# swook/EVE

Measured on AMD Instinct MI355X. Metric: train-step frames/sec, 128x128 eye patches T=30, higher is better.
Workload: dtype bf16; 1 GPU; BASELINE configs[1]: EyeNet training (configs/eye_net.json: ResNet-18-IN + GRU-128, angular + pupil L1 losses, clip 5.0, Adam wd 0.005), 128x128 patches, fwd+bwd+clip+Adam; global_batch=32, batch_per_gpu=32, seq_len=30, parallelism=dp1

## Files before the change

### eve_amd/_lib.py

```python
import ctypes
import os
from ctypes import POINTER, Structure, c_char_p, c_float, c_int, c_longlong, c_uint, c_void_p

from .build import LIB_PATH


class EveLibraryError(RuntimeError):
    pass


class ConvDesc(Structure):
    _fields_ = [(n, c_int) for n in ('dtype', 'N', 'IH', 'IW', 'Cin', 'OH', 'OW', 'Cout',
                                     'KH', 'KW', 'stride', 'pad')]


class DispatchConfig(Structure):
    _fields_ = [(n, c_int) for n in (
        'struct_bytes', 'conv_impl_v1', 'conv_tile_big', 'conv_halo', 'conv_ws64', 'conv_wg8', 'conv_wg8_min_tiles',
        'conv_wg8_s2_min_tiles', 'halo_persist', 'wgrad_target_wgs', 'wgrad_min_rows', 'wgrad_halo', 'wgrad_wg8',
        'wg64_th', 'wg64_nreg', 'wg64_fixed', 'in_split', 'in_min_threads', 'in_stats_one_pass', 'stem_split',
        'in_trunk_kernels', 'stem_fused_wgrad', 'stem_fwd_pairs', 'conv1x1_stream', 'conv3x3_stream', 'in_big_planes', 'cgru_seq_max_b',
        'cgru_scan', 'small_linear', 'tail_loss_node', 'bucket_elems', 'gate_wait_polls')] + [('wgrad_halo_min_m', c_longlong)]

    def as_dict(self):
        return {n: int(getattr(self, n)) for n, _ in self._fields_ if n != 'struct_bytes'}


class WgradProblem(Structure):
    _fields_ = [('dY', c_void_p), ('Y', c_void_p), ('X', c_void_p), ('X2', c_void_p), ('dW', c_void_p), ('db', c_void_p),
                ('M', c_int), ('N', c_int), ('K', c_int), ('K1', c_int), ('K2', c_int), ('act', c_int), ('rows_per_split', c_int),
                ('ldY', c_int), ('ldX', c_int), ('ldW', c_int), ('x_shift_T', c_int), ('reserved', c_int)]


WGRAD_BATCH_MAX = 12

class EyeGateParams(Structure):
    _fields_ = [('max_reproj_px', ctypes.c_double), ('pitch_lo', ctypes.c_double), ('pitch_hi', ctypes.c_double),
                ('yaw_lo', ctypes.c_double * 2), ('yaw_hi', ctypes.c_double * 2), ('close_ratio', ctypes.c_double),
                ('open_ratio', ctypes.c_double), ('baseline_rate', ctypes.c_double), ('baseline_rise', ctypes.c_double),
                ('min_inliers', c_int), ('min_inside', c_int), ('hold_frames', c_int), ('max_closed_frames', c_int)]


P = c_void_p
I = c_int
L = c_longlong
F = c_float

class PackItem(Structure):
    _fields_ = [('w_ohwi', c_void_p), ('dst_ohwi', c_void_p), ('dst_ihwo', c_void_p),
                ('Cout', c_int), ('taps', c_int), ('Cin', c_int), ('src_Cout', c_int), ('src_Cin', c_int)]


class VecTerm(Structure):
    _fields_ = [('pred', c_void_p), ('tgt', c_void_p), ('valid', c_void_p), ('dpred', c_void_p), ('D', c_int), ('kind', c_int)]


class EyeTailWeights(Structure):
    _fields_ = [(n, c_void_p) for n in ('fc_w', 'fc_b', 'c0_w', 'c0_b', 'c2_w', 'c2_b', 'ih_w', 'ih_b', 'hh_w', 'hh_b', 'g0_w', 'g0_b',
                                        'g2_w', 'p0_w', 'p0_b', 'p2_w', 'p2_b')]


class Surface(Structure):
    _fields_ = [('struct_bytes', c_int), ('kind', c_int), ('width', c_int), ('height', c_int), ('frame_stride', c_longlong),
                ('frame_bytes', c_longlong), ('offset', c_longlong * 3), ('pitch', c_int * 3), ('step', c_int * 3),
                ('xshift', c_int), ('yshift', c_int)]


VEC_TERMS_MAX = 32
PACK_BATCH_MAX = 48
ABI_VERSION = 10

SIGNATURES = {
    'eve_conv2d_fwd': [POINTER(ConvDesc), P, P, P, I, P, I, P, P],
    'eve_conv2d_fwd_stats': [POINTER(ConvDesc), P, P, P, I, P, P, F, POINTER(c_int), P],
    'eve_conv2d_dgrad': [POINTER(ConvDesc), P, P, P, P, ctypes.c_ulonglong, P],
    'eve_conv2d_dgrad_acc': [POINTER(ConvDesc), P, P, P, P],
    'eve_conv2d_wgrad': [POINTER(ConvDesc), P, P, P, I, P, P, ctypes.c_ulonglong, P],
    'eve_conv2d_wgrad_bias': [POINTER(ConvDesc), P, P, P, P, P, ctypes.c_ulonglong, P],
    'eve_get_dispatch_config': [POINTER(DispatchConfig)],
    'eve_get_default_dispatch_config': [POINTER(DispatchConfig)],
    'eve_set_dispatch_config': [POINTER(DispatchConfig)],
    'eve_stem_pack_input': [I, I, I, I, I, P, P, P],
    'eve_frames_u8_to_nchw': [L, I, I, I, P, F, F, I, P, P],
    'eve_frames_u8_to_stem': [I, L, I, I, I, P, F, F, P, P],
    'eve_stem7x7s2_fwd': [I, I, I, I, P, P, P, P],
    'eve_stem_fwd_fused': [I, I, I, I, P, P, F, P, P, P, P],
    'eve_stem_wgrad': [I, I, I, I, P, P, P, P],
    'eve_stem_bwd_dx': [I, I, I, I, P, P, P, P, P, P, P, P, P],
    'eve_stem_bwd_wgrad': [I, I, I, I, P, P, P, P, P, P, P, P, P, ctypes.c_ulonglong, P],
    'eve_stem_bwd_wgrad_workspace': [I, I, I],
    'eve_stem_dgrad_pack': [I, I, P, P, P],
    'eve_stem_dgrad': [I, I, I, I, I, P, P, P, P],
    'eve_bias_grad': [I, L, I, P, P, P],
    'eve_cgru_scan_fwd': [I, I, I, P, P, P, P, P, P, P, P, P, P, P, P],
    'eve_cgru_scan_bwd': [I, I, I, P, P, P, P, P, P, P, P, P, P, P, P],
    'eve_vector_terms': [POINTER(VecTerm), I, I, I, P, P],
    'eve_gate_signal': [P, P],
    'eve_gate_wait': [P, c_uint, P, P, P, c_uint, P],
    'eve_crnn_scan_fwd': [I, I, P, P, P, P, P, P, P],
    'eve_crnn_scan_bwd': [I, I, P, P, P, P, P, P, P],
    'eve_clstm_scan_fwd': [I, I, P, P, P, P, P, P, P, P],
    'eve_cgru_scan_fwd_c': [I, I, I, I, P, P, P, P, P, P, P, P, P, P, P, P],
    'eve_cgru_scan_bwd_c': [I, I, I, I, P, P, P, P, P, P, P, P, P, P, P, P],
    'eve_crnn_scan_fwd_c': [I, I, I, P, P, P, P, P, P, P],
    'eve_crnn_scan_bwd_c': [I, I, I, P, P, P, P, P, P, P],
    'eve_clstm_scan_fwd_c': [I, I, I, P, P, P, P, P, P, P, P],
    'eve_clstm_scan_fwd_train_c': [I, I, I, P, P, P, P, P, P, P, P, P, P, P],
    'eve_clstm_scan_bwd_c': [I, I, I, P, P, P, P, P, P, P, P, P, P, P],
    'eve_rnn_scan_fwd': [I, I, I, P, P, P, P, P, P],
    'eve_rnn_scan_bwd': [I, I, I, P, P, P, P, P, P],
    'eve_lstm_scan_fwd': [I, I, I, P, P, P, P, P, P, P, P, P],
    'eve_lstm_scan_bwd': [I, I, I, P, P, P, P, P, P, P, P, P, P, P],
    'eve_pack_weights_batch': [I, I, P, P],
    'eve_eye_losses': [I, I, P, P, P, P, P, P, F, F, P, P, P, P],
    'eve_gaze_to_pog': [L, P, P, P, P, P, P, P, F, F, P, P, P, P, P],
    'eve_gaze_to_pog_bwd': [L, P, P, P, P, P, P],
    'eve_combined_gaze': [L, P, P, P, P, P, P],
    'eve_make_heatmaps': [L, I, I, P, P, F, F, F, P, P],
    'eve_make_heatmaps_bwd': [L, I, I, P, F, F, F, P, P, P],
    'eve_soft_argmax_fwd': [L, I, I, P, F, F, P, P, P],
    'eve_soft_argmax_bwd': [L, I, I, P, P, P, F, F, P, P],
    'eve_linear_fwd': [I, I, I, P, P, P, I, P, P],
    'eve_linear_dgrad': [I, I, I, P, P, I, P, P, P],
    'eve_linear_wgrad': [I, I, I, P, P, I, P, P, P, P],
    'eve_linear_fwd_ex': [I, I, I, P, I, P, P, I, I, P, I, P],
    'eve_linear_dgrad_ex': [I, I, I, P, I, P, I, P, P, I, I, P],
    'eve_tail_head_pose': [I, P, P, P, I, I, P],
    'eve_tail_outputs_fwd': [I, P, P, P, P, P],
    'eve_tail_outputs_bwd': [I, P, P, P, P, P, F, F, P, P, P],
    'eve_linear_wgrad_batch': [POINTER(WgradProblem), I, P],
    'eve_instnorm_stats': [I, I, I, I, P, F, P, P],
    'eve_instnorm_act_fwd': [I, I, I, I, P, P, P, P, P, I, P, P],
    'eve_instnorm_act_bwd': [I, I, I, I, P, P, P, P, P, P, I, P, P, P, P, P],
    'eve_instnorm_act2_fwd': [I, I, I, I, P, P, P, P, P, P, I, P, P, I, I, P, P, P],
    'eve_instnorm_act2_bwd': [I, I, I, I, P, P, I, P, P, P, P, P, P, I, P, P, P, I, P, P, P, P],
    'eve_instnorm_fwd_fused': [I, I, I, I, P, P, P, P, I, F, P, P, P, P],
    'eve_instnorm_bwd_fused': [I, I, I, I, P, P, P, P, P, P, P, I, P, P, P, P, P, P],
    'eve_sum_rows': [I, I, P, P, P],
    'eve_sum_rows_pairs': [I, I, P, P, P, P],
    'eve_act_bwd': [I, L, P, P, I, P, P],
    'eve_add': [I, L, P, P, P, P],
    'eve_maxpool3x3s2_fwd': [I, I, I, I, I, P, P, P, P],
    'eve_maxpool3x3s2_bwd': [I, I, I, I, I, P, P, P, P],
    'eve_in_relu_maxpool_fwd': [I, I, I, I, I, P, P, P, P, P],
    'eve_in_relu_maxpool_bwd': [I, I, I, I, I, P, P, P, P, P, P, P],
    'eve_avgpool_fwd': [I, I, I, I, P, P, P],
    'eve_avgpool_bwd': [I, I, I, I, P, P, P],
    'eve_avgpool_fwd_f32': [I, I, I, I, P, P, P],
    'eve_avgpool_bwd_f32': [I, I, I, I, P, P, P],
    'eve_adaptive_maxpool_fwd': [I, I, I, I, I, I, I, P, P, P, P],
    'eve_adaptive_maxpool_bwd': [I, I, I, I, I, I, I, P, P, P, P, P],
    'eve_bilinear_fwd': [I, I, I, I, I, I, I, P, P, P],
    'eve_bilinear_bwd': [I, I, I, I, I, I, I, P, P, P],
    'eve_nchw_to_nhwc': [I, I, I, I, I, I, P, P, P],
    'eve_nhwc_to_nchw': [I, I, I, I, I, I, P, P, P],
    'eve_cast': [I, I, L, P, P, P],
    'eve_pack_weights': [I, I, I, I, P, P, P, P],
    'eve_gru_scan_fwd': [I, I, I, P, P, P, P, P, P, P, P],
    'eve_gru_scan_bwd': [I, I, I, P, P, P, P, P, P, P, P, P, P],
    'eve_cgru_gates1': [I, L, I, P, P, P, P, P],
    'eve_cgru_gates2': [I, L, I, P, P, P, P, P, P],
    'eve_cgru_gates2_bwd': [I, L, I, P, P, P, P, P, P, P, P],
    'eve_cgru_gates1_bwd': [I, L, I, P, P, P, P, P, P, P],
    'eve_clstm_gates_fwd': [I, L, I, P, P, P, P, P],
    'eve_clstm_gates_bwd': [I, L, I, P, P, P, P, P, P, P],
    'eve_heatmap_head_fwd': [I, L, I, P, P, P],
    'eve_heatmap_head_bwd': [I, L, I, P, P, P, P],
    'eve_heatmap_loss_fwd': [I, I, I, I, P, P, P, P, P, P, P],
    'eve_heatmap_loss_bwd': [I, I, I, P, P, P, P, P, P],
    'eve_sumsq': [L, P, P, P, P],
    'eve_adam_step': [L, P, P, P, P, P, F, F, F, F, F, F, F, I, P, I, P, P, P],
    'eve_eye_tail_stream_fwd': [I, I, P, P, POINTER(EyeTailWeights), P, P, P, P, P, P],
    'eve_stream_state_rows': [I, I, L, L, L, P, P, P, P],
    'eve_eye_tail_stream_fwd_len': [I, I, P, P, POINTER(EyeTailWeights), P, P, P, P, P, P, P],
    'eve_stream_state_rows_at': [I, I, I, L, L, L, L, P, P, P, P],
    'eve_stream_mask_plan': [I, I, P, P, P, P, P, P, P, P, P],
    'eve_stream_permute_rows': [I, I, L, L, L, P, P, P, P],
    'eve_screen_u8_area_to_nchw': [L, I, I, I, P, I, I, P, P],
    'eve_eye_warp_u8_to_nchw': [L, I, I, I, P, P, I, I, P, P],
    'eve_eye_warp_u8_to_stem': [I, L, I, I, I, P, P, I, I, P, P],
    'eve_eye_warp_lens_u8_to_nchw': [L, I, I, I, P, P, P, I, I, P, P],
    'eve_eye_warp_lens_u8_to_stem': [I, L, I, I, I, P, P, P, I, I, P, P],
    'eve_eye_pose_normalize': [L, P, I, I, P, P, P, P, P, P, P],
    'eve_eye_pose_normalize_rt': [L, I, P, I, P, P, P, I, I, P, P, P, P, P, P],
    'eve_face_pose_solve': [L, I, I, I, P, P, P, P, P, P, P, P, P, P],
    'eve_screen_u8_area_bgr_to_nchw': [L, I, I, I, P, I, I, P, P],
    'eve_eye_warp_fmt_to_nchw': [I, I, L, I, I, P, P, P, I, I, P, P],
    'eve_eye_warp_fmt_to_stem': [I, I, I, L, I, I, P, P, P, I, I, P, P],
    'eve_screen_area_fmt_to_nchw': [I, I, L, I, I, P, I, I, P, P],
    'eve_eye_warp_surface_to_nchw': [POINTER(Surface), I, L, P, P, P, I, I, P, P],
    'eve_eye_warp_surface_to_stem': [I, POINTER(Surface), I, L, P, P, P, I, I, P, P],
    'eve_screen_area_surface_to_nchw': [POINTER(Surface), I, L, P, I, I, P, P],
    'eve_overlay_render': [I, I, I, L, I, I, P, P, I, P, P, P, F, F, P, I, I, I, I, P, I, I, I, I, I, I, P, P],
    'eve_face_pose_solve_ex': [L, I, I, I, P, P, P, ctypes.c_double, P, P, P, P, P, P, P, P, P],
    'eve_undistort_points': [L, P, P, L, P, P, P],
    'eve_calib_append': [L, I, I, P, P, P, P, P, P, P, P, P, P, I, P, P, P, P],
    'eve_calib_fit': [L, I, P, P, P, ctypes.c_double, I, P, P, P, P, P, P, P, P],
    'eve_screen_calib_append': [L, I, P, P, P, P, P, P, P, P, ctypes.c_double, ctypes.c_double, I, P, P, P, P],
    'eve_screen_calib_fit': [L, I, P, P, P, I, I, ctypes.c_double, I, ctypes.c_double, P, P, P, P, P, P, P, P, P],
    'eve_screen_calib_apply': [L, I, P, P, P, P, ctypes.c_double, ctypes.c_double, P, P],
    'eve_gaze_events': [L, I, P, P, P, P, P, P, P, P, P] + [ctypes.c_double] * 4 + [I] + [ctypes.c_double] * 3 + [P, I, P, P, P] + [P] * 8,
    'eve_gaze_events_ex': [L, I, P, P, P, P, P, P, P, P, P] + [ctypes.c_double] * 4 + [I] + [ctypes.c_double] * 3 + [P, I, P, P, P] + [P] * 11,
    'eve_gaze_saccades': [L, I] + [P] * 9 + [ctypes.c_double] * 3 + [I] + [P, P, I, P, P, P] + [P] * 3,
    'eve_gaze_pursuits': [L, I] + [P] * 10 + [ctypes.c_double] * 7 + [I] + [P, P, I, P, P, P] + [P] * 7,
    'eve_eye_gate': [L, I, P, P, P, P, P, P, I, P, P, I, I, I, I, POINTER(EyeGateParams), P, I, P, P, P, P, P, P, P, P],
    'eve_gaze_history_plan': [L, I, P, P, P, P, P, P, ctypes.c_double, ctypes.c_double, I, ctypes.c_double, ctypes.c_double, I, I,
                              ctypes.c_double, ctypes.c_double, P, P, P, P],
    'eve_gaze_history_update': [L, I, I, I, P, P, P, ctypes.c_double, ctypes.c_double, P, P, P],
    'eve_gaze_aoi': [L, I, I, P, P, I] + [P] * 8 + [ctypes.c_double] * 2 + [P, P, P, I, P, P, P] + [P] * 4,
    'eve_pupil_track': [L, I] + [P] * 8 + [ctypes.c_double] * 12 + [P, P, P, I, P, P, P] + [P] * 9 + [P],
    'eve_screen_luminance': [POINTER(Surface), I, L, I, P, P, I, I, I, P, I, POINTER(c_int), P, F, F, P, P, P, P, P],
}
EXPORTS = sorted(list(SIGNATURES) + ['eve_abi_version', 'eve_last_error', 'eve_last_kernel'])

_lib = None


def load(path=None):
    global _lib
    if _lib is not None:
        return _lib
    path = path or os.environ.get('EVE_HIP_LIB', LIB_PATH)
    if not os.path.isfile(path):
        raise EveLibraryError(
            'libeve_hip.so not found at %s -- build it with `python -m eve_amd.build` '
            '(hipcc, gfx950).  eve_amd has no CPU fallback for the hot path.' % path)
    lib = ctypes.CDLL(path)
    for name, argtypes in SIGNATURES.items():
        fn = getattr(lib, name)
        fn.argtypes = argtypes
        fn.restype = c_int
    lib.eve_stem_bwd_wgrad_workspace.restype = ctypes.c_ulonglong
    lib.eve_last_kernel.argtypes = []
    lib.eve_last_kernel.restype = ctypes.c_char_p
    lib.eve_abi_version.argtypes = []
    lib.eve_abi_version.restype = c_int
    lib.eve_last_error.argtypes = []
    lib.eve_last_error.restype = c_char_p
    if lib.eve_abi_version() != ABI_VERSION:
        raise EveLibraryError('libeve_hip.so ABI version %d, expected %d (rebuild: python -m eve_amd.build)' % (
            lib.eve_abi_version(), ABI_VERSION))
    _lib = lib
    return lib


def check(status, lib=None):
    if status != 0:
        lib = lib or load()
        raise RuntimeError('libeve_hip: ' + lib.eve_last_error().decode('utf-8', 'replace'))
```

### eve_amd/csrc/api.hip

```cpp
#include <stdio.h>
#include <stdlib.h>
#include <string.h>

#include "common.h"

namespace eve {
static thread_local char g_err[512] = "";
thread_local const char* g_last_kernel = "";
thread_local hipError_t g_launch_error = hipSuccess;
int set_error(hipError_t e, const char* where) {
    snprintf(g_err, sizeof(g_err), "%s: HIP error %d (%s)", where, (int)e, hipGetErrorString(e));
    return 100 + (int)e;
}
int set_error_msg(const char* msg) {
    snprintf(g_err, sizeof(g_err), "%s", msg);
    return 1;
}
}

extern "C" int eve_abi_version(void) { return EVE_ABI_VERSION; }

namespace eve {
static eve_dispatch_config default_dispatch_config() {
    eve_dispatch_config c;
    memset(&c, 0, sizeof(c));
    c.struct_bytes = (int)sizeof(c);
    c.conv_impl_v1 = 0; c.conv_tile_big = 0; c.conv_halo = 1; c.conv_ws64 = 1; c.conv_wg8 = 1;
    c.conv_wg8_min_tiles = 224; c.conv_wg8_s2_min_tiles = 48; c.halo_persist = 1;
    c.wgrad_target_wgs = 0; c.wgrad_min_rows = 1536; c.wgrad_halo = 1; c.wgrad_wg8 = 1;
    c.wg64_th = 0; c.wg64_nreg = 0; c.wg64_fixed = 1;
    c.in_split = 1; c.in_min_threads = 512; c.in_stats_one_pass = 1; c.stem_split = 1; c.in_trunk_kernels = 1; c.stem_fused_wgrad = 1; c.stem_fwd_pairs = 1; c.in_big_planes = 1; c.conv1x1_stream = 1; c.conv3x3_stream = 1;
    c.wgrad_halo_min_m = 1ll << 20;
    c.cgru_seq_max_b = 384;
    c.cgru_scan = 1; c.small_linear = 1; c.tail_loss_node = 1; c.bucket_elems = 4 * 1024 * 1024; c.gate_wait_polls = 1 << 21;
    return c;
}
static void env_int(const char* name, int& field) { if (const char* e = getenv(name)) field = atoi(e); }
static eve_dispatch_config load_dispatch_config() {
    eve_dispatch_config c = default_dispatch_config();
    if (const char* e = getenv("EVE_CONV_IMPL")) c.conv_impl_v1 = (e[0] == 'v' && e[1] == '1') ? 1 : 0;
    if (const char* e = getenv("EVE_CONV_TILE")) c.conv_tile_big = e[0] == '2' ? 1 : 0;
    env_int("EVE_CONV_HALO", c.conv_halo); env_int("EVE_CONV_WS64", c.conv_ws64); env_int("EVE_CONV_WG8", c.conv_wg8);
    env_int("EVE_CONV_WG8_MIN_TILES", c.conv_wg8_min_tiles); env_int("EVE_CONV_WG8_S2_MIN_TILES", c.conv_wg8_s2_min_tiles);
    env_int("EVE_HALO_PERSIST", c.halo_persist); env_int("EVE_WGRAD_TARGET_WGS", c.wgrad_target_wgs);
    env_int("EVE_WGRAD_MIN_ROWS", c.wgrad_min_rows); env_int("EVE_WGRAD_HALO", c.wgrad_halo); env_int("EVE_WGRAD_WG8", c.wgrad_wg8);
    env_int("EVE_WG64_TH", c.wg64_th); env_int("EVE_WG64_NREG", c.wg64_nreg); env_int("EVE_WG64_FIXED", c.wg64_fixed);
    env_int("EVE_IN_SPLIT", c.in_split); env_int("EVE_IN_MIN_THREADS", c.in_min_threads);
    env_int("EVE_IN_STATS_ONE_PASS", c.in_stats_one_pass); env_int("EVE_STEM_SPLIT", c.stem_split);
    env_int("EVE_IN_TRUNK", c.in_trunk_kernels);
    env_int("EVE_STEM_FUSED_WGRAD", c.stem_fused_wgrad);
    env_int("EVE_STEM_FWD_PAIRS", c.stem_fwd_pairs);
    env_int("EVE_IN_BIG_PLANES", c.in_big_planes);
    env_int("EVE_CONV1X1_STREAM", c.conv1x1_stream);
    env_int("EVE_CONV3X3_STREAM", c.conv3x3_stream);
    env_int("EVE_CGRU_SEQ_MAX_B", c.cgru_seq_max_b);
    env_int("EVE_CGRU_SCAN", c.cgru_scan); env_int("EVE_SMALL_LINEAR", c.small_linear); env_int("EVE_TAIL_LOSS_NODE", c.tail_loss_node);
    env_int("EVE_BUCKET_ELEMS", c.bucket_elems); env_int("EVE_GATE_WAIT_POLLS", c.gate_wait_polls);
    if (const char* e = getenv("EVE_WGRAD_HALO_MIN_M")) c.wgrad_halo_min_m = atoll(e);
    if (c.wgrad_min_rows < 64) c.wgrad_min_rows = 64;
    if (c.in_min_threads < 64) c.in_min_threads = 64;
    if (c.bucket_elems < 1) c.bucket_elems = 1;
    if (c.gate_wait_polls < 1) c.gate_wait_polls = 1;
    return c;
}
eve_dispatch_config g_cfg = load_dispatch_config();
}

extern "C" int eve_get_dispatch_config(eve_dispatch_config* out) {
    if (!out) return eve::set_error_msg("get_dispatch_config: null pointer");
    *out = eve::g_cfg;
    return 0;
}
extern "C" int eve_get_default_dispatch_config(eve_dispatch_config* out) {
    if (!out) return eve::set_error_msg("get_default_dispatch_config: null pointer");
    *out = eve::default_dispatch_config();
    return 0;
}
extern "C" int eve_set_dispatch_config(const eve_dispatch_config* cfg) {
    if (!cfg || cfg->struct_bytes != (int)sizeof(eve_dispatch_config)) return eve::set_error_msg("set_dispatch_config: struct size mismatch (ABI)");
    if (cfg->wgrad_min_rows < 64 || cfg->in_min_threads < 64) return eve::set_error_msg("set_dispatch_config: wgrad_min_rows / in_min_threads must be >= 64");
    if (cfg->bucket_elems < 1 || cfg->gate_wait_polls < 1) return eve::set_error_msg("set_dispatch_config: bucket_elems / gate_wait_polls must be >= 1");
    eve::g_cfg = *cfg;
    return 0;
}
extern "C" const char* eve_last_error(void) { return eve::g_err; }
extern "C" const char* eve_last_kernel(void) { return eve::g_last_kernel; }
```

### eve_amd/csrc/conv_igemm.hip

```cpp
#include <limits.h>
#include <stdio.h>
#include <stdlib.h>

#include <initializer_list>
#include <type_traits>
#include "common.h"

namespace eve {

struct GatherParams {
    int N, IH, IW, Cin;
    int OH, OW, Cout;
    int KH, KW;
    int o_mul, k_mul, off, div;
    int K;
    uint32_t M;
    FastDiv fd_ohw, fd_ow, fd_cin, fd_kw, fd_oh;
};

template <typename T>
__device__ __forceinline__ uint4 prologue_vec(uint4 q, const float* __restrict__ ssp, int act) {
    constexpr int VEC = Elem<T>::VEC;
    float f[VEC];
    Elem<T>::unpack(q, f);
// ... 597 lines not shown
            for (int kw = 0; kw < p.KW; ++kw) {
                const int t = kh * p.KW + kw;
                tp.dy[t] = (signed char)(kh * p.k_mul); tp.dx[t] = (signed char)(kw * p.k_mul); tp.wt[t] = (signed char)t;
            }
        tp.osy = tp.osx = 1; tp.oy0 = tp.ox0 = 0; tp.OHf = p.OH; tp.OWf = p.OW;
        launch_dma_one<T>(p, tp, src, w, bias, epi_act, out, (uint32_t)src_bytes, (uint32_t)w_bytes, s);
        return true;
    }
    if (p.o_mul != 1 || p.k_mul != -1 || bias || (epi_act & 0xff) != EVE_ACT_NONE) return false;
    const int sd = p.div;
    bool need_zero = false;
    for (int pass = 0; pass < 2; ++pass) {
        for (int py = 0; py < sd; ++py)
            for (int px = 0; px < sd; ++px) {
                TapPlan tp;
                tp.ntaps = 0;
                for (int kh = 0; kh < p.KH; ++kh)
                    for (int kw = 0; kw < p.KW; ++kw) {
                        const int ny = py + p.off - kh, nx = px + p.off - kw;
                        if (ny % sd != 0 || nx % sd != 0) continue;
                        tp.dy[tp.ntaps] = (signed char)(ny / sd); tp.dx[tp.ntaps] = (signed char)(nx / sd);
                        tp.wt[tp.ntaps] = (signed char)(kh * p.KW + kw);
                        ++tp.ntaps;
                    }
                const int sub_h = (p.OH - py + sd - 1) / sd, sub_w = (p.OW - px + sd - 1) / sd;
                if (sub_h <= 0 || sub_w <= 0) continue;
                if (tp.ntaps == 0) { need_zero = true; continue; }
                if (pass == 0) continue;
                GatherParams q = p;
                q.OH = sub_h; q.OW = sub_w;
                q.o_mul = 1; q.off = 0; q.div = 1;
                q.M = (uint32_t)((long long)p.N * sub_h * sub_w);
                q.fd_ohw = make_fastdiv(sub_h * sub_w); q.fd_ow = make_fastdiv(sub_w);
                tp.osy = tp.osx = sd; tp.oy0 = py; tp.ox0 = px; tp.OHf = p.OH; tp.OWf = p.OW;
                launch_dma_one<T>(q, tp, src, w, bias, epi_act, out, (uint32_t)src_bytes, (uint32_t)w_bytes, s);
            }
        if (pass == 0 && need_zero && !(epi_act & EVE_EPI_ACC))
            (void)hipMemsetAsync(out, 0, (size_t)p.N * p.OH * p.OW * p.Cout * sizeof(T), s);
    }
    return true;
}

template <typename T>
static int launch_igemm(const GatherParams& p, const void* src, const void* w, const float* bias,
                        const float* ss, int pro_act, int epi_act, void* out, hipStream_t s) {
    if (!ss && !use_v1() && launch_igemm_dma<T>(p, src, w, bias, epi_act, out, s)) return 0;
    const bool wide = p.Cout > 64;
    const uint32_t bn = wide ? 128 : 64;
    const uint32_t tiles = ((p.M + 127) / 128) * ((p.Cout + bn - 1) / bn);
    dim3 grid(tiles), block(256);
    const T* a = (const T*)src; const T* b = (const T*)w; T* o = (T*)out;
    if (wide) {
        if (ss) EVE_LAUNCH("igemm_kernel<T, 4, true>", (igemm_kernel<T, 4, true>), grid, block, 0, s, p, a, b, bias, ss, pro_act, epi_act, o);
        else    EVE_LAUNCH("igemm_kernel<T, 4, false>", (igemm_kernel<T, 4, false>), grid, block, 0, s, p, a, b, bias, ss, pro_act, epi_act, o);
    } else {
        if (ss) EVE_LAUNCH("igemm_kernel<T, 2, true>", (igemm_kernel<T, 2, true>), grid, block, 0, s, p, a, b, bias, ss, pro_act, epi_act, o);
        else    EVE_LAUNCH("igemm_kernel<T, 2, false>", (igemm_kernel<T, 2, false>), grid, block, 0, s, p, a, b, bias, ss, pro_act, epi_act, o);
    }
    return 0;
}

static void wgrad_split(const GatherParams& p, uint32_t tk, uint32_t tc, size_t lds_per_wg, uint32_t& splits, uint32_t& rows) {
    const int target_env = g_cfg.wgrad_target_wgs;
    uint32_t per_cu = lds_per_wg ? (uint32_t)((160 * 1024) / lds_per_wg) : 3;
    per_cu = per_cu < 1 ? 1 : (per_cu > 3 ? 3 : per_cu);
    const uint32_t target = target_env > 0 ? (uint32_t)target_env : 256u * per_cu;
    uint32_t want = target / (tk * tc);
    const int min_rows = g_cfg.wgrad_min_rows;
    uint32_t max_splits = (p.M + (uint32_t)min_rows - 1) / (uint32_t)min_rows;
    splits = want < 1 ? 1 : (want > max_splits ? max_splits : want);
    if (splits < 1) splits = 1;
    if (splits > 65535) splits = 65535;
    rows = (p.M + splits - 1) / splits;
    rows = (rows + 63) / 64 * 64;
    splits = (p.M + rows - 1) / rows;
}

template <typename HT>
static bool launch_wgrad_halo(const GatherParams& p, const void* x, const void* dy, float* dw, float* db, hipStream_t s) {
    if (!g_cfg.wgrad_halo) return false;
    const int ks = p.KH;
    if ((ks != 3 && ks != 1) || p.KW != ks || p.o_mul != 1 || p.k_mul != 1 || p.off != -(ks / 2) || p.div != 1 || p.OH != p.IH ||
        p.OW != p.IW)
        return false;
    const int W = p.IW, H = p.IH;
    const long long min_m = g_cfg.wgrad_halo_min_m;
    if (W < 32 || W > 128 || (W & (W - 1)) || p.Cin % 16 || p.Cout % 16 || (long long)p.M < min_m) return false;
    const int MT = p.Cout / 16, CT = p.Cin / 16;
    const bool split = ks == 3 && MT == 4 && CT == 4;
    if (ks == 3 && !split && !((MT == 1 && (CT == 1 || CT == 2 || CT == 4)) || (MT == 2 && (CT == 1 || CT == 2)))) return false;
    if (ks == 1 && !((MT == 2 && CT == 1) || (MT == 1 && CT == 4) || (MT == 1 && CT == 2) || (MT == 4 && CT == 2) || (MT == 2 && CT == 4)))
        return false;
    const unsigned long long xb = (unsigned long long)p.N * H * W * p.Cin * 2, db_ = (unsigned long long)p.M * p.Cout * 2;
    if (xb >= (1ull << 31) || db_ >= (1ull << 31)) return false;
    const size_t red = (size_t)(ks * ks * p.Cin * p.Cout + p.Cout) * 4;
    const unsigned occ = (ks == 3 && MT * CT >= 4) ? 2 : 3;
    int TH = 0; size_t lds = 0;
    int nreg = 0;
    if (split) {
        const int force_th = g_cfg.wg64_th, force_nreg = g_cfg.wg64_nreg;
        for (int th : {8, 4, 2, 1}) {
            if (force_th && th != force_th) continue;
            const size_t need = (size_t)(th + 2) * (W + 2) * 128 + (size_t)th * W * 128;
            for (int nr : {3, 2}) {
                if (force_nreg && nr != force_nreg) continue;
                if (nr * need <= (size_t)160 * 1024) { TH = th; nreg = nr; lds = nr * need > red ? nr * need : red; break; }
            }
            if (TH) break;
        }
    } else
    for (size_t budget : {(size_t)(occ == 3 ? 52 : 78) * 1024, (size_t)78 * 1024}) {
        for (int th : {4, 2, 1}) {
            const size_t need = (size_t)(th + ks - 1) * (W + ks - 1) * p.Cin * 2 + (size_t)th * W * p.Cout * 2;
            if (need <= budget && need >= red) { TH = th; lds = need; break; }
        }
        if (TH) break;
    }
    if (!TH) return false;
    WgradHaloParams h;
    h.N = p.N; h.H = H; h.W = W; h.TH = TH; h.bands = (H + TH - 1) / TH;
    h.total_bands = (uint32_t)p.N * h.bands; h.x_bytes = (uint32_t)xb; h.dy_bytes = (uint32_t)db_;
    h.log2_cpr = 0; h.nreg = nreg;
    while ((32 << h.log2_cpr) < W) ++h.log2_cpr;
    const unsigned per_cu = (unsigned)((160 * 1024) / lds);
    unsigned grid = 256 * (per_cu > occ ? occ : per_cu);
    if (grid > h.total_bands) grid = h.total_bands;
    auto band_tile = [&](auto kernel) { launch(kernel, dim3(grid), dim3(256), lds, s, h, (const HT*)x, (const HT*)dy, dw, db); };
    if (split) {
        const unsigned g64 = h.total_bands < 256u ? h.total_bands : 256u;
        const int fixed64 = g_cfg.wg64_fixed;
        if (fixed64 && W == 32 && TH == 8 && H % 8 == 0)
            EVE_LAUNCH(EVE_HNAME(HT, "wgrad_halo64_kernel<", ", fixed>"), (wgrad_halo64_kernel<HT, true>), dim3(g64), dim3(512), lds, s, h, (const HT*)x, (const HT*)dy, dw, db);
        else
            EVE_LAUNCH(EVE_HNAME(HT, "wgrad_halo64_kernel<", ">"), (wgrad_halo64_kernel<HT, false>), dim3(g64), dim3(512), lds, s, h, (const HT*)x, (const HT*)dy, dw, db);
    } else if (ks == 3) {
        if (MT == 1 && CT == 1) band_tile(EVE_KERNEL_H(HT, wgrad_halo_kernel, 1, 1, 3));
        else if (MT == 1 && CT == 2) band_tile(EVE_KERNEL_H(HT, wgrad_halo_kernel, 1, 2, 3));
        else if (MT == 1 && CT == 4) band_tile(EVE_KERNEL_H(HT, wgrad_halo_kernel, 1, 4, 3));
        else if (MT == 2 && CT == 1) band_tile(EVE_KERNEL_H(HT, wgrad_halo_kernel, 2, 1, 3));
        else band_tile(EVE_KERNEL_H(HT, wgrad_halo_kernel, 2, 2, 3));
    } else {
        if (MT == 2 && CT == 1) band_tile(EVE_KERNEL_H(HT, wgrad_halo_kernel, 2, 1, 1));
        else if (MT == 1 && CT == 4) band_tile(EVE_KERNEL_H(HT, wgrad_halo_kernel, 1, 4, 1));
        else if (MT == 1 && CT == 2) band_tile(EVE_KERNEL_H(HT, wgrad_halo_kernel, 1, 2, 1));
        else if (MT == 4 && CT == 2) band_tile(EVE_KERNEL_H(HT, wgrad_halo_kernel, 4, 2, 1));
        else band_tile(EVE_KERNEL_H(HT, wgrad_halo_kernel, 2, 4, 1));
    }
    return true;
}

#define EVE_WGRAD_TR(T, WCO, WK, P2, MT) EVE_HNAME(T, "wgrad_tr_kernel<", ", " #WCO ", " #WK ", " #P2 ", mt" #MT ">"), ic<WCO>{}, ic<WK>{}, ic<P2>{}, ic<MT>{}

static constexpr uint32_t WGRAD_WG8_T128_MIN_M = 65536;

template <typename T>
static int launch_wgrad(const GatherParams& p, const void* x, const void* dy, const float* ss, int pro_act,
                        float* dw, hipStream_t s, float* db = nullptr, void* workspace = nullptr, unsigned long long workspace_bytes = 0) {
    if constexpr (sizeof(T) == 2) {
    if (!ss && !use_v1() && launch_wgrad_halo<T>(p, x, dy, dw, db, s)) return db ? 1 : 0;
    if (!ss && !use_v1()) {
        const unsigned long long x_bytes = (unsigned long long)p.N * p.IH * p.IW * p.Cin * 2;
        const unsigned long long dy_bytes = (unsigned long long)p.M * p.Cout * 2;
        if (x_bytes < (1ull << 31) && dy_bytes < (1ull << 31)) {
            uint32_t splits, rows;
            const bool pow2 = ((p.OW & (p.OW - 1)) == 0) && ((p.OH & (p.OH - 1)) == 0);
            auto lds_bytes = [](int bco, int bkk, int mode) { return (size_t)((bco == 128 || (bkk == 256 && mode == 2)) ? 3 : 4) * 32 * (bco + bkk) * 2; };
            auto tr_tile = [&](const char* name, auto wco, auto wk, auto p2, auto mt, uint32_t tk, uint32_t tc) {
                constexpr int WCO = decltype(wco)::value, WK = decltype(wk)::value, P2 = decltype(p2)::value, MT = decltype(mt)::value;
                auto go = [&](auto kernel) {
                    launch(kernel, dim3(tk * tc * splits), dim3(64 * WCO * WK), lds_bytes(64 * WCO, 64 * WK, P2), s, p, (const T*)x, (const T*)dy, dw,
                           rows, (uint32_t)x_bytes, (uint32_t)dy_bytes, db);
                };
                if (db) go(Named<wgrad_tr_kernel<T, WCO, WK, P2, true, MT>>{name});
                else    go(Named<wgrad_tr_kernel<T, WCO, WK, P2, false, MT>>{name});
            };
            const bool pow2w = (p.OW & (p.OW - 1)) == 0;
            const int mode = pow2 ? 1 : ((pow2w && p.OH * p.OW >= 32) ? 2 : 0);
            const int wg8w = g_cfg.wgrad_wg8;
            if (wg8w && !db && mode == 1 && p.Cout % 256 == 0 && p.K % 256 == 0) {
                const uint32_t tk = p.K / 256, tc = p.Cout / 256;
                wgrad_split(p, tk, tc, (size_t)128 * 1024, splits, rows);
                const unsigned long long n = (unsigned long long)p.Cout * p.K;
                const bool slab = splits > 1 && workspace && (unsigned long long)splits * n * 4 <= workspace_bytes && ((uintptr_t)dw & 15) == 0 &&
                                  ((uintptr_t)workspace & 15) == 0;
                if (slab) {
                    EVE_LAUNCH(EVE_HNAME(T, "wgrad_wg8_kernel<", ", true>"), (wgrad_wg8_kernel<T, true>), dim3(tk * tc * splits), dim3(512), (size_t)128 * 1024, s, p,
                               (const T*)x, (const T*)dy, (float*)workspace, rows, (uint32_t)x_bytes, (uint32_t)dy_bytes);
                    const long long n4 = (long long)(n / 4);
                    long long blocks = (n4 + 255) / 256;
                    if (blocks > 2048) blocks = 2048;
                    hipLaunchKernelGGL(wgrad_slab_reduce_kernel, dim3((unsigned)blocks), dim3(256), 0, s, (const float*)workspace, dw, n4, (int)splits);
                } else {
                    EVE_LAUNCH(EVE_HNAME(T, "wgrad_wg8_kernel<", ", false>"), (wgrad_wg8_kernel<T, false>), dim3(tk * tc * splits), dim3(512), (size_t)128 * 1024, s, p,
                               (const T*)x, (const T*)dy, dw, rows, (uint32_t)x_bytes, (uint32_t)dy_bytes);
                }
            } else if ((wg8w == 1 || wg8w == 2) && !db && mode == 1 && p.KH == 3 && p.KW == 3 && p.Cin == 128 && p.Cout % 128 == 0 &&
                       (wg8w == 2 || p.M >= WGRAD_WG8_T128_MIN_M)) {
                const uint32_t tk = 3, tc = p.Cout / 128;
                wgrad_split(p, tk, tc, (size_t)128 * 1024, splits, rows);
                const unsigned long long n = (unsigned long long)p.Cout * p.K;
                const bool slab = splits > 1 && workspace && (unsigned long long)splits * n * 4 <= workspace_bytes && ((uintptr_t)dw & 15) == 0 &&
                                  ((uintptr_t)workspace & 15) == 0;
                if (slab) {
                    EVE_LAUNCH(EVE_HNAME(T, "wgrad_wg8_t128_kernel<", ", true>"), (wgrad_wg8_t128_kernel<T, true>), dim3(tk * tc * splits), dim3(512), (size_t)128 * 1024,
                               s, p, (const T*)x, (const T*)dy, (float*)workspace, rows, (uint32_t)x_bytes, (uint32_t)dy_bytes);
                    const long long n4 = (long long)(n / 4);
                    hipLaunchKernelGGL(wgrad_slab_reduce_wide_kernel, dim3((unsigned)((n4 + 31) / 32)), dim3(256), 0, s, (const float*)workspace, dw, n4,
                                       (int)splits);
                } else {
                    EVE_LAUNCH(EVE_HNAME(T, "wgrad_wg8_t128_kernel<", ", false>"), (wgrad_wg8_t128_kernel<T, false>), dim3(tk * tc * splits), dim3(512), (size_t)128 * 1024,
                               s, p, (const T*)x, (const T*)dy, dw, rows, (uint32_t)x_bytes, (uint32_t)dy_bytes);
                }
            } else if (p.Cout > 64) {
                const uint32_t tk = (p.K + 127) / 128, tc = (p.Cout + 127) / 128;
                wgrad_split(p, tk, tc, lds_bytes(128, 128, mode), splits, rows);
                if (mode == 1)      tr_tile(EVE_WGRAD_TR(T, 2, 2, 1, 4), tk, tc);
                else if (mode == 2) tr_tile(EVE_WGRAD_TR(T, 2, 2, 2, 4), tk, tc);
                else                tr_tile(EVE_WGRAD_TR(T, 2, 2, 0, 4), tk, tc);
            } else if (mode == 1 && p.K % 192 == 0 && p.K <= 1152) {
                const uint32_t tk = p.K / 192;
                wgrad_split(p, tk, 1, lds_bytes(64, 192, mode), splits, rows);
                tr_tile(EVE_WGRAD_TR(T, 1, 3, 1, 4), tk, 1);
            } else {
                const uint32_t tk = (p.K + 255) / 256, tc = 1;
                wgrad_split(p, tk, tc, lds_bytes(64, 256, mode), splits, rows);
                if (mode == 1)      tr_tile(EVE_WGRAD_TR(T, 1, 4, 1, 4), tk, tc);
                else if (mode == 2) {
                    if (p.Cout <= 16)      tr_tile(EVE_WGRAD_TR(T, 1, 4, 2, 1), tk, tc);
                    else if (p.Cout <= 32) tr_tile(EVE_WGRAD_TR(T, 1, 4, 2, 2), tk, tc);
                    else                   tr_tile(EVE_WGRAD_TR(T, 1, 4, 2, 4), tk, tc);
                }
                else                tr_tile(EVE_WGRAD_TR(T, 1, 4, 0, 4), tk, tc);
            }
            return db ? 1 : 0;
        }
    }
    }
    const bool wide = p.Cout > 64;
    const uint32_t bco = wide ? 128 : 64;
    const uint32_t tk = (p.K + 127) / 128, tc = (p.Cout + bco - 1) / bco;
    uint32_t want = (1024 + tk * tc - 1) / (tk * tc);
    uint32_t max_splits = (p.M + 255) / 256;
    uint32_t splits = want < 1 ? 1 : (want > max_splits ? max_splits : want);
    if (splits < 1) splits = 1;
    if (splits > 65535) splits = 65535;
    uint32_t rows = (p.M + splits - 1) / splits;
    rows = (rows + 63) / 64 * 64;
    splits = (p.M + rows - 1) / rows;
    dim3 grid(tk, tc, splits), block(256);
    const T* a = (const T*)x; const T* b = (const T*)dy;
    if (wide) {
        if (ss) EVE_LAUNCH("wgrad_kernel<T, 4, true>", (wgrad_kernel<T, 4, true>), grid, block, 0, s, p, a, b, ss, pro_act, dw, rows);
        else    EVE_LAUNCH("wgrad_kernel<T, 4, false>", (wgrad_kernel<T, 4, false>), grid, block, 0, s, p, a, b, ss, pro_act, dw, rows);
    } else {
        if (ss) EVE_LAUNCH("wgrad_kernel<T, 2, true>", (wgrad_kernel<T, 2, true>), grid, block, 0, s, p, a, b, ss, pro_act, dw, rows);
        else    EVE_LAUNCH("wgrad_kernel<T, 2, false>", (wgrad_kernel<T, 2, false>), grid, block, 0, s, p, a, b, ss, pro_act, dw, rows);
    }
    return 0;
}

template <typename HT>
static bool launch_s2_fwd_wg8(const eve_conv_desc* d, const void* x, const void* w, const float* bias, int epi_act, void* y, hipStream_t s) {
    const int on = g_cfg.conv_wg8, min_tiles = g_cfg.conv_wg8_s2_min_tiles;
    const int W = d->OW;
    if (!on || d->KH != 3 || d->KW != 3 || d->stride != 2 || d->pad != 1 || d->OH != W || d->IH != 2 * W || d->IW != 2 * W ||
        !(W == 16 || W == 8 || W == 4) || d->Cin % 64 || (epi_act & ~0xff) ||
        !((epi_act & 0xff) == EVE_ACT_NONE || (epi_act & 0xff) == EVE_ACT_RELU))
        return false;
    const int cout_t = W == 16 ? 128 : 256;
    if (d->Cout % cout_t) return false;
    const unsigned long long xb = (unsigned long long)d->N * 4 * W * W * d->Cin * 2, wb = (unsigned long long)d->Cout * 9 * d->Cin * 2;
    if (xb >= (1ull << 31) || wb >= (1ull << 31)) return false;
    const int ti = W == 16 ? 2 : (W == 8 ? 4 : 16);
    const uint32_t tiles = (uint32_t)((d->N + ti - 1) / ti) * (uint32_t)(d->Cout / cout_t);
    if ((int)tiles < min_tiles) return false;
    Wg8Params g;
    g.N = d->N; g.Cin = d->Cin; g.Cout = d->Cout; g.flip = 0; g.K = 9 * d->Cin; g.x_bytes = (uint32_t)xb; g.w_bytes = (uint32_t)wb;
    g.tiles_n = (uint32_t)(d->Cout / cout_t); g.s2_py = 0;
    auto s2_tile = [&](auto kernel, auto geom) {
        launch(kernel, dim3(tiles), dim3(512), decltype(geom)::LDS, s, g, (const HT*)x, (const HT*)w, bias, epi_act, (HT*)y);
    };
    if (W == 16) s2_tile(EVE_KERNEL_H(HT, conv3x3s2_wg8_kernel, 4, 2, 16), Wg8S2Geom<4, 2, 16>{});
    else if (W == 8) s2_tile(EVE_KERNEL_H(HT, conv3x3s2_wg8_kernel, 2, 4, 8), Wg8S2Geom<2, 4, 8>{});
    else s2_tile(EVE_KERNEL_H(HT, conv3x3s2_wg8_kernel, 2, 4, 4), Wg8S2Geom<2, 4, 4>{});
    return true;
}

template <typename H>
__global__ __launch_bounds__(256) void s2_dgrad_pack_kernel(const H* __restrict__ w_ihwo, H* __restrict__ w0, H* __restrict__ w1,
                                                            int Cdx, int Cout) {
    const int kv = Cout / 8;
    const long long n0 = (long long)2 * Cdx * 2 * kv, n1 = (long long)2 * Cdx * 4 * kv;
    for (long long i = (long long)blockIdx.x * 256 + threadIdx.x; i < n0 + n1; i += (long long)gridDim.x * 256) {
        const int py = i >= n0 ? 1 : 0, nt = py ? 4 : 2;
        const long long r = py ? i - n0 : i;
        const int v = (int)(r % kv), t = (int)((r / kv) % nt), row = (int)(r / ((long long)kv * nt));
        const int px = row >= Cdx ? 1 : 0, ci = row - px * Cdx;
        const int dy = py ? t >> 1 : 0, dx = t & 1;
        const int kh = py + 1 - 2 * dy, kw = px + 1 - 2 * dx;
        uint4 q = make_uint4(0u, 0u, 0u, 0u);
        if (kh >= 0 && kw >= 0)
            q = reinterpret_cast<const uint4*>(w_ihwo + (((size_t)ci * 3 + kh) * 3 + kw) * Cout)[v];
        reinterpret_cast<uint4*>(py ? w1 : w0)[r] = q;
    }
}

#define EVE_S2_DGRAD(H, WM, WN, W, NT) eve::Named<conv3x3_wg8_kernel<H, WM, WN, W, NT>>{EVE_HNAME(H, "conv3x3_wg8_kernel<", ", " #WM ", " #WN ", " #W ", s2dgrad" #NT ">")}, Wg8Geom<WM, WN, W>{}, ic<NT>{}

template <typename HT>
static bool launch_s2_dgrad_wg8(const eve_conv_desc* d, const void* dy, const void* w_ihwo, void* dx, void* workspace,
                                unsigned long long workspace_bytes, hipStream_t s) {
    const int on = g_cfg.conv_wg8, min_tiles = g_cfg.conv_wg8_s2_min_tiles;
    const int W = d->OW, Cdx = d->Cin, Co = d->Cout;
    if (!on || d->KH != 3 || d->KW != 3 || d->stride != 2 || d->pad != 1 || d->OH != W || d->IH != 2 * W || d->IW != 2 * W ||
        !(W == 16 || W == 8 || W == 4) || Co % 64 || !workspace || ((uintptr_t)workspace & 255))
        return false;
    const int cout_t = W == 16 ? 128 : 256;
    if ((2 * Cdx) % cout_t) return false;
    const unsigned long long wbytes = (unsigned long long)2 * Cdx * 6 * Co * 2;
    const unsigned long long xb = (unsigned long long)d->N * W * W * Co * 2, ob = (unsigned long long)d->N * 4 * W * W * Cdx * 2;
    if (wbytes > workspace_bytes || xb >= (1ull << 31) || ob >= (1ull << 31) || wbytes >= (1ull << 31)) return false;
    const int ti = W == 16 ? 2 : (W == 8 ? 4 : 16);
    const uint32_t tiles = (uint32_t)((d->N + ti - 1) / ti) * (uint32_t)(2 * Cdx / cout_t);
    if ((int)tiles < min_tiles) return false;
    HT* w0 = (HT*)workspace;
    HT* w1 = w0 + (size_t)2 * Cdx * 2 * Co;
    const long long nvec = (long long)2 * Cdx * 6 * (Co / 8);
    hipLaunchKernelGGL(s2_dgrad_pack_kernel<HT>, dim3((unsigned)((nvec + 255) / 256 > 1024 ? 1024 : (nvec + 255) / 256)), dim3(256), 0, s,
                       (const HT*)w_ihwo, w0, w1, Cdx, Co);
    Wg8Params g;
    g.N = d->N; g.Cin = Co; g.Cout = 2 * Cdx; g.flip = 0; g.x_bytes = (uint32_t)xb; g.tiles_n = (uint32_t)(2 * Cdx / cout_t);
    auto row_parity = [&](auto kernel, auto geom, auto nt, const HT* wp, int py) {
        constexpr int NT = decltype(nt)::value;
        g.K = NT * Co; g.w_bytes = (uint32_t)((unsigned long long)2 * Cdx * NT * Co * 2); g.s2_py = py;
        launch(kernel, dim3(tiles), dim3(512), decltype(geom)::LDS, s, g, (const HT*)dy, wp, (const float*)nullptr, (int)EVE_ACT_NONE, (HT*)dx);
    };
    if (W == 16) { row_parity(EVE_S2_DGRAD(HT, 4, 2, 16, 2), w0, 0); row_parity(EVE_S2_DGRAD(HT, 4, 2, 16, 4), w1, 1); }
    else if (W == 8) { row_parity(EVE_S2_DGRAD(HT, 2, 4, 8, 2), w0, 0); row_parity(EVE_S2_DGRAD(HT, 2, 4, 8, 4), w1, 1); }
    else { row_parity(EVE_S2_DGRAD(HT, 2, 4, 4, 2), w0, 0); row_parity(EVE_S2_DGRAD(HT, 2, 4, 4, 4), w1, 1); }
    return true;
}

static int conv_entry(const char* who, const eve_conv_desc* d, const char* cout_msg, bool operands, int max_cout_vecs = INT_MAX) {
    const int vec = (d && d->dtype != EVE_DT_F32) ? 8 : 4;
    if (int e = check_desc(d, vec)) return e;
    char msg[128];
    if (cout_msg && (d->Cout % vec || d->Cout / vec > max_cout_vecs)) { snprintf(msg, sizeof(msg), "%s: %s", who, cout_msg); return set_error_msg(msg); }
    if (!operands) { snprintf(msg, sizeof(msg), "%s: null pointer", who); return set_error_msg(msg); }
    return 0;
}

struct ConvCall {
    const char* who;
    const eve_conv_desc* d;
    bool dgrad;
    const void* in; const void* w; const float* bias; int epi_act; void* out;
    const float* in_scale_shift; int pro_act;
    void* workspace; unsigned long long workspace_bytes;
    hipStream_t s;
    int cin() const { return dgrad ? d->Cout : d->Cin; }
    int cout() const { return dgrad ? d->Cin : d->Cout; }
};
typedef bool (*ConvRung)(const ConvCall&);

static bool rung_1x1_stream(const ConvCall& c) {
    const eve_conv_desc* d = c.d;
    if (!(d->KH == 1 && d->KW == 1 && d->stride == 1 && d->pad == 0)) return false;
    const long long M = (long long)d->N * d->OH * d->OW;
    bool done = false;
    EVE_DISPATCH_H16(d->dtype, done = launch_conv1x1_stream<H>(M, c.cin(), c.cout(), c.in, c.w, c.bias, c.epi_act, c.out, c.s));
    return done;
}
static bool rung_1x1_s2_stream(const ConvCall& c) {
    const eve_conv_desc* d = c.d;
    if (!(!c.bias && c.epi_act == (c.dgrad ? (int)EVE_EPI_ACC : (int)EVE_ACT_NONE) && d->KH == 1 && d->stride == 2)) return false;
    bool done = false;
    EVE_DISPATCH_H16(d->dtype, done = launch_conv1x1_s2_stream<H>(d, c.dgrad, c.in, c.w, c.out, c.s));
    return done;
}
static bool rung_3x3_stream(const ConvCall& c) {
    const eve_conv_desc* d = c.d;
    if (!(d->KH == 3 && d->KW == 3 && d->stride == 1 && d->pad == 1)) return false;
    bool done = false;
    EVE_DISPATCH_H16(d->dtype, done = launch_conv3x3_stream<H>(d->N, d->IH, d->IW, c.cin(), c.cout(), c.dgrad ? 1 : 0, c.in, c.w, c.bias, c.epi_act,
                                                               c.out, c.s));
    return done;
}
static bool rung_s2_wg8(const ConvCall& c) {
    bool done = false;
    if (c.dgrad) EVE_DISPATCH_H16(c.d->dtype, done = launch_s2_dgrad_wg8<H>(c.d, c.in, c.w, c.out, c.workspace, c.workspace_bytes, c.s));
    else         EVE_DISPATCH_H16(c.d->dtype, done = launch_s2_fwd_wg8<H>(c.d, c.in, c.w, c.bias, c.epi_act, c.out, c.s));
    return done;
}
static int conv_ladder(const ConvCall& c, std::initializer_list<ConvRung> rungs) {
    bool done = false;
    if (!c.in_scale_shift && c.d->dtype != EVE_DT_F32)
        for (ConvRung rung : rungs)
            if ((done = rung(c))) break;
    if (!done) {
        const GatherParams p = c.dgrad ? dgrad_params(c.d) : fwd_params(c.d);
        EVE_DISPATCH_T(c.d->dtype, launch_igemm<T>(p, c.in, c.w, c.bias, c.in_scale_shift, c.pro_act, c.epi_act, c.out, c.s));
    }
    const hipError_t e = take_launch_error();
    return e == hipSuccess ? 0 : set_error(e, c.who);
}

}

using namespace eve;

extern "C" int eve_conv2d_fwd(const eve_conv_desc* d, const void* x, const void* w_ohwi, const float* bias,
                              int epi_act, const float* in_scale_shift, int pro_act, void* y,
                              eve_stream_t stream) {
    if (int e = conv_entry("conv2d_fwd", d, nullptr, x && w_ohwi && y)) return e;
    const ConvCall c = {__func__, d, false, x, w_ohwi, bias, epi_act, y, in_scale_shift, pro_act, nullptr, 0, (hipStream_t)stream};
    return conv_ladder(c, {rung_1x1_stream, rung_1x1_s2_stream, rung_3x3_stream, rung_s2_wg8});
}

extern "C" int eve_conv2d_fwd_stats(const eve_conv_desc* d, const void* x, const void* w_ohwi, const float* bias, int epi_act,
                                    void* y, float* mean_rstd, float eps, int* stats_written, eve_stream_t stream) {
    if (!stats_written || !mean_rstd) return set_error_msg("conv2d_fwd_stats: null pointer");
    *stats_written = 0;
    if (int e = conv_entry("conv2d_fwd_stats", d, nullptr, x && w_ohwi && y)) return e;
    if (d->KH == 3 && d->KW == 3 && d->stride == 1 && d->pad == 1 && d->dtype != EVE_DT_F32 && !(epi_act & EVE_EPI_ACC)) {
        bool done = false;
        EVE_DISPATCH_H16(d->dtype, done = launch_conv3x3_stream<H>(d->N, d->IH, d->IW, d->Cin, d->Cout, 0, x, w_ohwi, bias, epi_act, y,
                                                                   (hipStream_t)stream, mean_rstd, eps));
        if (done) { *stats_written = 1; EVE_CHECK_LAUNCH(); return 0; }
    }
    return eve_conv2d_fwd(d, x, w_ohwi, bias, epi_act, nullptr, 0, y, stream);
}

extern "C" int eve_conv2d_dgrad(const eve_conv_desc* d, const void* dy, const void* w_ihwo, void* dx,
                                void* workspace, unsigned long long workspace_bytes, eve_stream_t stream) {
    if (int e = conv_entry("conv2d_dgrad", d, "Cout must be a multiple of the 16-byte vector", dy && w_ihwo && dx)) return e;
    const ConvCall c = {__func__, d, true, dy, w_ihwo, nullptr, 0, dx, nullptr, 0, workspace, workspace_bytes, (hipStream_t)stream};
    return conv_ladder(c, {rung_1x1_stream, rung_3x3_stream, rung_s2_wg8});
}

extern "C" int eve_conv2d_dgrad_acc(const eve_conv_desc* d, const void* dy, const void* w_ihwo, void* dx,
                                    eve_stream_t stream) {
    if (int e = conv_entry("conv2d_dgrad_acc", d, "Cout must be a multiple of the 16-byte vector", dy && w_ihwo && dx)) return e;
    const ConvCall c = {__func__, d, true, dy, w_ihwo, nullptr, EVE_EPI_ACC, dx, nullptr, 0, nullptr, 0, (hipStream_t)stream};
    return conv_ladder(c, {rung_1x1_stream, rung_1x1_s2_stream, rung_3x3_stream});
}

extern "C" int eve_conv2d_wgrad(const eve_conv_desc* d, const void* x, const void* dy,
                                const float* in_scale_shift, int pro_act, float* dw_ohwi,
                                void* workspace, unsigned long long workspace_bytes, eve_stream_t stream) {
    if (int e = conv_entry("conv2d_wgrad", d, "Cout must be a multiple of the 16-byte vector", x && dy && dw_ohwi)) return e;
    GatherParams p = fwd_params(d);
    hipStream_t s = (hipStream_t)stream;
    if (d->dtype == EVE_DT_BF16) launch_wgrad<bf16_t>(p, x, dy, in_scale_shift, pro_act, dw_ohwi, s, nullptr, workspace, workspace_bytes);
    else if (d->dtype == EVE_DT_F16) launch_wgrad<f16_t>(p, x, dy, in_scale_shift, pro_act, dw_ohwi, s, nullptr, workspace, workspace_bytes);
    else                         launch_wgrad<float>(p, x, dy, in_scale_shift, pro_act, dw_ohwi, s);
    EVE_CHECK_LAUNCH();
    return 0;
}

extern "C" int eve_stem_wgrad(int dtype, int N, int IH, int IW, const void* x_padded, const void* dconv, float* dw, eve_stream_t stream) {
    if ((dtype != EVE_DT_BF16 && dtype != EVE_DT_F16) || N <= 0 || IH <= 0 || IW <= 0 || (IH & 1) || (IW & 1) || !x_padded || !dconv || !dw)
        return set_error_msg("stem_wgrad: bad arguments");
    GatherParams p;
    p.N = N; p.IH = IH + 6; p.IW = IW + 8; p.Cin = 4;
    p.OH = IH / 2; p.OW = IW / 2; p.Cout = 64; p.KH = 7; p.KW = 8;
    p.o_mul = 2; p.k_mul = 1; p.off = 0; p.div = 1;
    p.K = 7 * 8 * 4;
    p.M = (uint32_t)((long long)N * p.OH * p.OW);
    p.fd_ohw = make_fastdiv(p.OH * p.OW); p.fd_ow = make_fastdiv(p.OW);
    p.fd_cin = make_fastdiv(4); p.fd_kw = make_fastdiv(8); p.fd_oh = make_fastdiv(p.OH);
    const char* x1 = (const char*)x_padded + 8;
    if ((unsigned long long)N * p.IH * p.IW * 8 >= (1ull << 31)) return set_error_msg("stem_wgrad: packed input must stay below 2 GiB");
    const unsigned long long per_img = (unsigned long long)p.OH * p.OW * 64 * 2;
    int chunk = (int)(((1ull << 31) - 1) / per_img);
    if (chunk < 1) return set_error_msg("stem_wgrad: one image's gradient exceeds 2 GiB");
    const int nchunks = (N + chunk - 1) / chunk;
    chunk = (N + nchunks - 1) / nchunks;
    for (int n0 = 0; n0 < N; n0 += chunk) {
        const int n = N - n0 < chunk ? N - n0 : chunk;
        p.N = n;
        p.M = (uint32_t)((long long)n * p.OH * p.OW);
        const char* xc = x1 + (size_t)n0 * p.IH * p.IW * 8;
        const char* dc = (const char*)dconv + (size_t)n0 * per_img;
        EVE_DISPATCH_H16(dtype, launch_wgrad<H>(p, xc, dc, nullptr, 0, dw, (hipStream_t)stream));
    }
    EVE_CHECK_LAUNCH();
    return 0;
}

static void launch_bias_grad(int dtype, long long M, int C, const void* dy, float* db, hipStream_t s) {
    long long blocks = (M + 255) / 256;
    if (blocks > 2048) blocks = 2048;
    const long long rows = (M + blocks - 1) / blocks;
    blocks = (M + rows - 1) / rows;
    EVE_DISPATCH_T(dtype, hipLaunchKernelGGL(bias_grad_kernel<T>, dim3((unsigned)blocks), dim3(256), 0, s, (const T*)dy, db, M, C, rows));
}

extern "C" int eve_bias_grad(int dtype, long long M, int C, const void* dy, float* db, eve_stream_t stream) {
    const int vec = dtype != EVE_DT_F32 ? 8 : 4;
    if (M <= 0 || C <= 0 || C % vec || C / vec > 256) return set_error_msg("bias_grad: bad shape");
    if (!dy || !db) return set_error_msg("bias_grad: null pointer");
    launch_bias_grad(dtype, M, C, dy, db, (hipStream_t)stream);
    EVE_CHECK_LAUNCH();
    return 0;
}

extern "C" int eve_conv2d_wgrad_bias(const eve_conv_desc* d, const void* x, const void* dy, float* dw_ohwi, float* db,
                                     void* workspace, unsigned long long workspace_bytes, eve_stream_t stream) {
    if (int e = conv_entry("conv2d_wgrad_bias", d, "bad Cout", x && dy && dw_ohwi && db, 256)) return e;
    GatherParams p = fwd_params(d);
    hipStream_t s = (hipStream_t)stream;
    int fused = 0;
    if (d->dtype == EVE_DT_BF16) fused = launch_wgrad<bf16_t>(p, x, dy, nullptr, 0, dw_ohwi, s, db, workspace, workspace_bytes);
    else if (d->dtype == EVE_DT_F16) fused = launch_wgrad<f16_t>(p, x, dy, nullptr, 0, dw_ohwi, s, db, workspace, workspace_bytes);
    else                         launch_wgrad<float>(p, x, dy, nullptr, 0, dw_ohwi, s);
    if (!fused) launch_bias_grad(d->dtype, (long long)p.M, d->Cout, dy, db, s);
    EVE_CHECK_LAUNCH();
    return 0;
}
```

### eve_amd/csrc/linear_small.hip

```cpp
#include "common.h"

namespace eve {

constexpr int LM_T = 32;
constexpr int LM_GW = 2;
constexpr int LM_G = 4;

struct LmFrag { float w[2][4]; float x[2][4]; };

__device__ __forceinline__ void lm_mfma(f32x4_t (&acc)[2][2], const LmFrag& f) {
#pragma unroll
    for (int s = 0; s < 4; ++s)
#pragma unroll
        for (int a = 0; a < 2; ++a)
#pragma unroll
            for (int b = 0; b < 2; ++b) acc[a][b] = __builtin_amdgcn_mfma_f32_16x16x4f32(f.w[a][s], f.x[b][s], acc[a][b], 0, 0, 0);
}

__device__ __forceinline__ bool lm_reduce(f32x4_t (&acc)[2][2], float (*red)[16][64], const int wave, const int lane) {
    if (wave) {
#pragma unroll
        for (int a = 0; a < 2; ++a)
#pragma unroll
            for (int b = 0; b < 2; ++b)
#pragma unroll
                for (int v = 0; v < 4; ++v) red[wave - 1][(a * 2 + b) * 4 + v][lane] = acc[a][b][v];
    }
    __syncthreads();
    if (wave) return false;
#pragma unroll
    for (int w = 0; w < 3; ++w)
#pragma unroll
        for (int a = 0; a < 2; ++a)
#pragma unroll
            for (int b = 0; b < 2; ++b)
#pragma unroll
                for (int v = 0; v < 4; ++v) acc[a][b][v] += red[w][(a * 2 + b) * 4 + v][lane];
    return true;
}

struct LmActGrad { float p0, n0, n1, q; };
__device__ __forceinline__ LmActGrad lm_act_grad(const int act) {
    switch (act) {
        case EVE_ACT_RELU:    return {1.f, 0.f, 0.f, 0.f};
        case EVE_ACT_LEAKY:   return {1.f, 0.01f, 0.f, 0.f};
        case EVE_ACT_SELU:    return {EVE_SELU_SCALE, EVE_SELU_SCALE * EVE_SELU_ALPHA, 1.f, 0.f};
        case EVE_ACT_TANH:    return {1.f, 1.f, 0.f, -1.f};
        case EVE_ACT_SIGMOID: return {0.f, 0.f, 0.f, -1.f};
        default:              return {1.f, 1.f, 0.f, 0.f};
    }
}
__device__ __forceinline__ float lm_apply_grad(const float g, const float y, const LmActGrad& c, const bool sigmoid) {
    const bool pos = y > 0.f;
    float d = fmaf(pos ? 0.f : c.n1, y, pos ? c.p0 : c.n0);
    d = fmaf(c.q * y, y, d);
    if (sigmoid) d += y;
    return g * d;
}

__device__ __forceinline__ void lm_act16(float (&v)[2][2][4], const int act) {
#define LM_ALL(expr)                                   \
    _Pragma("unroll") for (int a = 0; a < 2; ++a)      \
    _Pragma("unroll") for (int b = 0; b < 2; ++b)      \
    _Pragma("unroll") for (int r = 0; r < 4; ++r) { const float z = v[a][b][r]; v[a][b][r] = (expr); }
    switch (act) {
        case EVE_ACT_RELU:    LM_ALL(z > 0.f ? z : 0.f) break;
        case EVE_ACT_LEAKY:   LM_ALL(z > 0.f ? z : 0.01f * z) break;
        case EVE_ACT_SELU:    LM_ALL(EVE_SELU_SCALE * (z > 0.f ? z : EVE_SELU_ALPHA * (__expf(z) - 1.f))) break;
        case EVE_ACT_TANH:    LM_ALL(tanhf(z)) break;
        case EVE_ACT_SIGMOID: LM_ALL(1.f / (1.f + __expf(-z))) break;
        default: break;
    }
#undef LM_ALL
}

template <bool VEC, bool HASY, int G>
__global__ __launch_bounds__(256) void linear_mm_kernel(const float* __restrict__ A, const float* __restrict__ Y, const int pro_act,
                                                        const float* __restrict__ B, const float* __restrict__ bias,
                                                        const int epi_act, float* __restrict__ C, const int M, const int R,
                                                        const int Nc, const int lda, const int ldc, const int n_bias,
                                                        const int accumulate) {
    __shared__ float red[3][16][64];
    const int tid = threadIdx.x, wave = tid >> 6, lane = tid & 63, i = lane & 15, kk = lane >> 4;
    const int m0 = blockIdx.x * LM_T, c0 = blockIdx.y * LM_T;
    const LmActGrad ag = lm_act_grad(pro_act);
    const bool sig = pro_act == EVE_ACT_SIGMOID;
    const float* bcol[2];
    const float* arow[2];
    const float* yrow[2];
    bool nok[2], mok[2];
#pragma unroll
    for (int t = 0; t < 2; ++t) {
        const int n = c0 + t * 16 + i, m = m0 + t * 16 + i;
        nok[t] = n < Nc; mok[t] = m < M;
        bcol[t] = B + min(n, Nc - 1);
        arow[t] = A + (size_t)min(m, M - 1) * lda;
        yrow[t] = HASY ? Y + (size_t)min(m, M - 1) * lda : nullptr;
    }
    struct Raw { LmFrag f; float y[2][4]; };
    auto fetch = [&](const int kb, Raw& r) {
        const int k = kb * 16 + 4 * kk;
#pragma unroll
        for (int t = 0; t < 2; ++t)
#pragma unroll
            for (int s = 0; s < 4; ++s) r.f.w[t][s] = bcol[t][(size_t)min(k + s, R - 1) * Nc];
#pragma unroll
        for (int t = 0; t < 2; ++t) {
            if (VEC) {
                const int kc = min(k, R - 4);
                const float4 v = *reinterpret_cast<const float4*>(arow[t] + kc);
                r.f.x[t][0] = v.x; r.f.x[t][1] = v.y; r.f.x[t][2] = v.z; r.f.x[t][3] = v.w;
                if (HASY) {
                    const float4 y = *reinterpret_cast<const float4*>(yrow[t] + kc);
                    r.y[t][0] = y.x; r.y[t][1] = y.y; r.y[t][2] = y.z; r.y[t][3] = y.w;
                }
            } else {
#pragma unroll
                for (int s = 0; s < 4; ++s) {
                    const int kc = min(k + s, R - 1);
                    r.f.x[t][s] = arow[t][kc];
                    if (HASY) r.y[t][s] = yrow[t][kc];
                }
            }
        }
    };
    auto finish = [&](const int kb, Raw& r) {
        const int k = kb * 16 + 4 * kk;
#pragma unroll
        for (int t = 0; t < 2; ++t)
#pragma unroll
            for (int s = 0; s < 4; ++s) {
                const bool kok = k + s < R;
                r.f.w[t][s] = (nok[t] && kok) ? r.f.w[t][s] : 0.f;
                float v = r.f.x[t][s];
                if (HASY) v = lm_apply_grad(v, r.y[t][s], ag, sig);
                r.f.x[t][s] = (mok[t] && kok) ? v : 0.f;
            }
    };
    f32x4_t acc[2][2];
#pragma unroll
    for (int a = 0; a < 2; ++a)
#pragma unroll
        for (int b = 0; b < 2; ++b) acc[a][b] = f32x4_t{0.f, 0.f, 0.f, 0.f};
    float bv[2][4];
#pragma unroll
    for (int a = 0; a < 2; ++a)
#pragma unroll
        for (int r = 0; r < 4; ++r) {
            const int n = c0 + a * 16 + 4 * kk + r;
            const float w = (bias && n_bias > 0) ? bias[min(n, n_bias - 1)] : 0.f;
            bv[a][r] = n < n_bias ? w : 0.f;
        }
    const int nkb = (R + 15) >> 4;
    Raw cur[G], nxt[G];
#pragma unroll
    for (int g = 0; g < G; ++g) fetch(wave + 4 * g, cur[g]);
    for (int kb = wave; kb < nkb; kb += 4 * G) {
        const bool more = kb + 4 * G < nkb;
        if (more) {
#pragma unroll
            for (int g = 0; g < G; ++g) fetch(kb + 4 * (G + g), nxt[g]);
        }
#pragma unroll
        for (int g = 0; g < G; ++g)
            if (kb + 4 * g < nkb) {
                finish(kb + 4 * g, cur[g]);
                lm_mfma(acc, cur[g].f);
            }
        if (more) {
#pragma unroll
            for (int g = 0; g < G; ++g) cur[g] = nxt[g];
        }
    }
    if (!lm_reduce(acc, red, wave, lane)) return;
    const bool vec_c = VEC && !(ldc & 3) && !(Nc & 3) && !((uintptr_t)C & 15);
    float v[2][2][4], prev[2][2][4];
    float* cptr[2][2];
#pragma unroll
    for (int a = 0; a < 2; ++a)
#pragma unroll
        for (int b = 0; b < 2; ++b) {
            const int m = m0 + b * 16 + i, n = c0 + a * 16 + 4 * kk;
            cptr[a][b] = C + (size_t)min(m, M - 1) * ldc + n;
            if (accumulate) {
                if (vec_c) {
                    const float4 p = *reinterpret_cast<const float4*>(C + (size_t)min(m, M - 1) * ldc + min(n, Nc - 4));
                    prev[a][b][0] = p.x; prev[a][b][1] = p.y; prev[a][b][2] = p.z; prev[a][b][3] = p.w;
                } else {
#pragma unroll
                    for (int r = 0; r < 4; ++r) prev[a][b][r] = C[(size_t)min(m, M - 1) * ldc + min(n + r, Nc - 1)];
                }
            }
#pragma unroll
            for (int r = 0; r < 4; ++r) v[a][b][r] = acc[a][b][r] + bv[a][r];
        }
    lm_act16(v, epi_act);
#pragma unroll
    for (int a = 0; a < 2; ++a)
#pragma unroll
        for (int b = 0; b < 2; ++b) {
            const int m = m0 + b * 16 + i, n = c0 + a * 16 + 4 * kk;
            if (accumulate) {
#pragma unroll
                for (int r = 0; r < 4; ++r) v[a][b][r] += prev[a][b][r];
            }
            if (m >= M || n >= Nc) continue;
            if (vec_c) {
                *reinterpret_cast<float4*>(cptr[a][b]) = make_float4(v[a][b][0], v[a][b][1], v[a][b][2], v[a][b][3]);
            } else {
#pragma unroll
                for (int r = 0; r < 4; ++r)
                    if (n + r < Nc) cptr[a][b][r] = v[a][b][r];
            }
        }
}

static inline bool lm_vec_ok(const void* a, const void* y, int lda, int R) {
    return !(lda & 3) && !(R & 3) && !((uintptr_t)a & 15) && !((uintptr_t)y & 15);
}
#define LM_LAUNCH(M_, Nc_, R_, ...)                                                                                                  \
    do {                                                                                                                         \
        const dim3 grid_(((M_) + LM_T - 1) / LM_T, ((Nc_) + LM_T - 1) / LM_T);                                                   \
        const int big_ = R_ > 160;                                                                                                          \
        if (vec_ && hasy_ && big_) EVE_LAUNCH("linear_mm_kernel", (linear_mm_kernel<true, true, 4>), grid_, dim3(256), 0, (hipStream_t)stream, __VA_ARGS__);   \
        else if (vec_ && hasy_) EVE_LAUNCH("linear_mm_kernel", (linear_mm_kernel<true, true, 2>), grid_, dim3(256), 0, (hipStream_t)stream, __VA_ARGS__);      \
        else if (vec_ && big_) EVE_LAUNCH("linear_mm_kernel", (linear_mm_kernel<true, false, 4>), grid_, dim3(256), 0, (hipStream_t)stream, __VA_ARGS__);      \
        else if (vec_) EVE_LAUNCH("linear_mm_kernel", (linear_mm_kernel<true, false, 2>), grid_, dim3(256), 0, (hipStream_t)stream, __VA_ARGS__);              \
// ... 279 lines not shown
```

### eve_amd/kernels.py

```python
import ctypes

import torch

from . import _lib
from ._lib import ConvDesc

ACT_NONE, ACT_RELU, ACT_LEAKY, ACT_SELU, ACT_TANH, ACT_SIGMOID = range(6)
EPI_ACCUMULATE = 0x100
DT_F32, DT_BF16, DT_F16 = 0, 1, 2
HALF_DTYPES = (torch.bfloat16, torch.float16)
SCAN_WIDTHS = (32, 64, 128)


def dt_code(dtype):
    if dtype == torch.float32:
        return DT_F32
    if dtype == torch.bfloat16:
        return DT_BF16
    if dtype == torch.float16:
        return DT_F16
    raise TypeError('eve_amd kernels support float32, bfloat16 and float16, got %s' % dtype)


PIXEL_FORMATS = {'bgr': 0, 'bgra': 1, 'nv12': 2, 'i420': 3, 'yuyv': 4}
# ... 1305 lines not shown
                tensors.append(t)
        if not all(t.is_contiguous() for t in tensors):
            raise RuntimeError('eve_amd: non-contiguous tensor handed to a kernel')
        for name, t, on in (('reproj_rms', reproj_rms, spec.max_reproj_px is not None), ('inliers', inliers, spec.min_inliers is not None),
                            ('warp', warp, spec.min_coverage is not None), ('h', h, spec.head_angles), ('contours', contours, spec.blink is not None)):
            if (t is not None) != bool(on):
                raise ValueError('eye_gate: %s goes with its criterion in the spec, and only with it' % name)
        IW = IH = OW = OH = 0
        if warp is not None:
            if frame_size is None or patch_size is None:
                raise ValueError('eye_gate: warp needs frame_size (IW, IH) and patch_size (OW, OH)')
            (IW, IH), (OW, OH) = (int(v) for v in frame_size), (int(v) for v in patch_size)
        inf = float('inf')
        rng = lambda r: (-inf, inf) if r is None else r
        P = EyeGateParams()
        P.max_reproj_px = inf if spec.max_reproj_px is None else spec.max_reproj_px
        P.pitch_lo, P.pitch_hi = rng(spec.head_pitch)
        for e, r in enumerate((spec.head_yaw_left, spec.head_yaw_right)):
            P.yaw_lo[e], P.yaw_hi[e] = rng(r)
        P.min_inliers = 0 if spec.min_inliers is None else spec.min_inliers
        P.min_inside = 1 if spec.min_coverage is None else spec.min_inside
        bl = spec.blink
        P.close_ratio, P.open_ratio = (0.0, 1.0) if bl is None else (bl.close_ratio, bl.open_ratio)
        P.baseline_rate, P.baseline_rise = (0.0, 0.0) if bl is None else (bl.baseline_rate, bl.baseline_rise)
        P.hold_frames, P.max_closed_frames = (0, 1) if bl is None else (bl.hold_frames, bl.max_closed_frames)
        dev = state.device
        out = {'usable': torch.empty((B, T, 2), dtype=torch.uint8, device=dev), 'reason': torch.empty((B, T, 2), dtype=torch.uint8, device=dev),
               'openness': torch.empty((B, T, 2), dtype=torch.float32, device=dev), 'blink': torch.empty((B, T, 2), dtype=torch.uint8, device=dev)}
        self._ck(self.lib.eve_eye_gate(
            B, T, self._p(pose_valid), self._p(reproj_rms), self._p(inliers), self._p(warp), self._p(h), self._p(contours), C, self._p(lengths),
            self._p(reset), IW, IH, OW, OH, ctypes.byref(P), self._p(state), store.shape[1], self._p(store), self._p(count), self._p(dropped),
            self._p(out['usable']), self._p(out['reason']), self._p(out['openness']), self._p(out['blink']), self._stream()))
        return out

    def _flat32(self, t, shape, what):
        t = t.contiguous()
        assert t.dtype == torch.float32 and tuple(t.shape) == tuple(shape), (what, t.dtype, tuple(t.shape), tuple(shape))
        self._p(t)
        return t

    def gaze_to_pog(self, g, origin, R, inv_cam, ppm, screen, head_R=None, kappa=None):
        N = g.shape[0]
        g = self._flat32(g, (N, 2), 'g'); origin = self._flat32(origin, (N, 3), 'origin')
        R = self._flat32(R, (N, 3, 3), 'R'); inv_cam = self._flat32(inv_cam, (N, 4, 4), 'inv_cam')
        ppm = self._flat32(ppm, (N, 2), 'ppm')
        if kappa is not None:
            head_R = self._flat32(head_R, (N, 3, 3), 'head_R'); kappa = self._flat32(kappa, (N, 2), 'kappa')
        new = lambda *s: torch.empty(s, dtype=torch.float32, device=g.device)
        g_out, mm, px, jac = new(N, 2), new(N, 2), new(N, 2), new(N, 6, 2)
        self._ck(self.lib.eve_gaze_to_pog(N, self._p(g), self._p(origin), self._p(R), self._p(inv_cam), self._p(ppm),
                                          self._p(head_R if kappa is not None else None), self._p(kappa), float(screen[0]),
                                          float(screen[1]), self._p(g_out), self._p(mm), self._p(px), self._p(jac), self._stream()))
        return g_out, mm, px, jac

    def gaze_to_pog_bwd(self, jac, dg_out, dmm, dpx):
        N = jac.shape[0]
        f = lambda t: None if t is None else self._flat32(t, (N, 2), 'grad')
        dg_out, dmm, dpx = f(dg_out), f(dmm), f(dpx)
        dg = torch.empty((N, 2), dtype=torch.float32, device=jac.device)
        self._ck(self.lib.eve_gaze_to_pog_bwd(N, self._p(jac), self._p(dg_out), self._p(dmm), self._p(dpx), self._p(dg), self._stream()))
        return dg

    def combined_gaze(self, origin, pog_mm, R, cam):
        N = origin.shape[0]
        origin = self._flat32(origin, (N, 3), 'origin'); pog_mm = self._flat32(pog_mm, (N, 2), 'pog_mm')
        R = self._flat32(R, (N, 3, 3), 'R'); cam = self._flat32(cam, (N, 4, 4), 'cam')
        g = torch.empty((N, 2), dtype=torch.float32, device=origin.device)
        self._ck(self.lib.eve_combined_gaze(N, self._p(origin), self._p(pog_mm), self._p(R), self._p(cam), self._p(g), self._stream()))
        return g

    def make_heatmaps(self, centres_px, sigma, hw, screen, validity=None):
        N = centres_px.shape[0]
        c = self._flat32(centres_px, (N, 2), 'centres')
        v = None
        if validity is not None:
            v = validity.contiguous()
            v = v.view(torch.uint8) if v.dtype == torch.bool else v.to(torch.uint8)
            assert tuple(v.shape) == (N,)
        out = torch.empty((N, 1, hw[0], hw[1]), dtype=torch.float32, device=c.device)
        for i in range(0, N, 65535):
            n = min(65535, N - i)
            self._ck(self.lib.eve_make_heatmaps(n, hw[0], hw[1], self._p(c[i:i + n]), self._p(None if v is None else v[i:i + n]),
                                                float(sigma), float(screen[0]), float(screen[1]), self._p(out[i:i + n]), self._stream()))
        return out

    def make_heatmaps_bwd(self, centres_px, sigma, screen, dout):
        N, _, H, W = dout.shape
        c = self._flat32(centres_px, (N, 2), 'centres')
        dout = self._flat32(dout, (N, 1, H, W), 'dout')
        dc = torch.empty((N, 2), dtype=torch.float32, device=c.device)
        self._ck(self.lib.eve_make_heatmaps_bwd(N, H, W, self._p(c), float(sigma), float(screen[0]), float(screen[1]), self._p(dout),
                                                self._p(dc), self._stream()))
        return dc

    def soft_argmax_fwd(self, heat, screen):
        N, _, H, W = heat.shape
        heat = self._flat32(heat, (N, 1, H, W), 'heat')
        px = torch.empty((N, 2), dtype=torch.float32, device=heat.device)
        stats = torch.empty((N, 4), dtype=torch.float32, device=heat.device)
        self._ck(self.lib.eve_soft_argmax_fwd(N, H, W, self._p(heat), float(screen[0]), float(screen[1]), self._p(px), self._p(stats),
                                              self._stream()))
        return px, stats

    def soft_argmax_bwd(self, heat, stats, dpog, screen):
        N, _, H, W = heat.shape
        dpog = self._flat32(dpog, (N, 2), 'dpog')
        dh = torch.empty_like(heat)
        for i in range(0, N, 65535):
            n = min(65535, N - i)
            self._ck(self.lib.eve_soft_argmax_bwd(n, H, W, self._p(heat[i:i + n]), self._p(stats[i:i + n]), self._p(dpog[i:i + n]),
                                                  float(screen[0]), float(screen[1]), self._p(dh[i:i + n]), self._stream()))
        return dh

    def heatmap_head_fwd(self, logits):
        N, H, W, Cp = logits.shape
        out = torch.empty((N, 1, H, W), dtype=torch.float32, device=logits.device)
        self._ck(self.lib.eve_heatmap_head_fwd(dt_code(logits.dtype), N * H * W, Cp, self._p(logits), self._p(out),
                                               self._stream()))
        return out

    def heatmap_head_bwd(self, dy, y, dtype, cpad):
        N, _, H, W = y.shape
        dy = dy.contiguous().float()
        dl = torch.empty((N, H, W, cpad), dtype=dtype, device=y.device)
        self._ck(self.lib.eve_heatmap_head_bwd(dt_code(dtype), N * H * W, cpad, self._p(dy), self._p(y), self._p(dl),
                                               self._stream()))
        return dl

    def heatmap_loss_fwd(self, kind, pred, gt, validity):
        B, T = pred.shape[:2]
        HW = pred[0, 0].numel()
        pred, gt = pred.contiguous(), gt.contiguous()
        assert pred.dtype == torch.float32 and gt.dtype == torch.float32 and gt.shape == pred.shape
        v = validity.contiguous()
        v = v.view(torch.uint8) if v.dtype == torch.bool else v.to(torch.uint8)
        assert tuple(v.shape) == (B, T)
        per_map = torch.empty((B * T,), dtype=torch.float32, device=pred.device)
        w = torch.empty((B * T,), dtype=torch.float32, device=pred.device)
        loss = torch.empty((1,), dtype=torch.float32, device=pred.device)
        self._ck(self.lib.eve_heatmap_loss_fwd(kind, B, T, HW, self._p(pred), self._p(gt), self._p(v), self._p(per_map),
                                               self._p(loss), self._p(w), self._stream()))
        return loss.view(()), w

    def heatmap_loss_bwd(self, kind, pred, gt, w, upstream):
        B, T = pred.shape[:2]
        HW = pred[0, 0].numel()
        pred, gt = pred.contiguous(), gt.contiguous()
        up = upstream.detach().float().reshape(1).contiguous()
        dp = torch.empty_like(pred)
        self._ck(self.lib.eve_heatmap_loss_bwd(kind, B * T, HW, self._p(pred), self._p(gt), self._p(w), self._p(up),
                                               self._p(dp), self._stream()))
        return dp

    def eye_losses(self, g_pred, g_tgt, g_val, p_pred, p_tgt, p_val, coeff_ang, coeff_l1):
        B, T = p_pred[0].shape
        dev = p_pred[0].device

        def pair(ts, dtype, shape):
            out = []
            for t in ts:
                t = t.contiguous()
                if dtype == torch.uint8:
                    t = t.view(torch.uint8) if t.dtype == torch.bool else t.to(torch.uint8)
                assert t.dtype == dtype and tuple(t.shape) == shape and t.is_cuda, (t.dtype, t.shape)
                out.append(t)
            return out, (ctypes.c_void_p * 2)(*[t.data_ptr() for t in out])

        keep = []
        ptrs = []
        for ts, dt, shp in ((g_pred, torch.float32, (B, T, 2)), (g_tgt, torch.float32, (B, T, 2)), (g_val, torch.uint8, (B, T)),
                            (p_pred, torch.float32, (B, T)), (p_tgt, torch.float32, (B, T)), (p_val, torch.uint8, (B, T))):
            k_, a = pair(ts, dt, shp)
            keep.append(k_)
            ptrs.append(a)
        terms = torch.zeros((5,), dtype=torch.float32, device=dev)
        dg = [torch.empty((B, T, 2), dtype=torch.float32, device=dev) for _ in range(2)]
        dp = [torch.empty((B, T), dtype=torch.float32, device=dev) for _ in range(2)]
        dg_a = (ctypes.c_void_p * 2)(*[t.data_ptr() for t in dg])
        dp_a = (ctypes.c_void_p * 2)(*[t.data_ptr() for t in dp])
        self._ck(self.lib.eve_eye_losses(B, T, ptrs[0], ptrs[1], ptrs[2], ptrs[3], ptrs[4], ptrs[5], float(coeff_ang),
                                         float(coeff_l1), self._p(terms), dg_a, dp_a, self._stream()))
        return terms, dg, dp

    def linear_fwd(self, x, w_in_out, bias, act):
        M, K = x.shape
        N = w_in_out.shape[1]
        assert x.dtype == torch.float32 and w_in_out.dtype == torch.float32 and w_in_out.shape[0] == K
        assert x.is_contiguous() and w_in_out.is_contiguous()
        y = torch.empty((M, N), dtype=torch.float32, device=x.device)
        self._ck(self.lib.eve_linear_fwd(M, K, N, self._p(x), self._p(w_in_out), self._p(self._f32(bias, 'bias')), act,
                                         self._p(y), self._stream()))
        return y

    def linear_fwd_ex(self, x, k_cols, w_in_out, bias, act, y, n_cols=None):
        M = x.shape[0]
        K, N = w_in_out.shape
        assert k_cols == K and (n_cols is None or n_cols == N)
        for t in (x, w_in_out, y, bias):
            assert t is None or (t.dtype == torch.float32 and t.is_contiguous() and t.is_cuda)
        assert x.shape[1] >= K and y.shape[1] >= N and y.shape[0] == M
        self._ck(self.lib.eve_linear_fwd_ex(M, K, N, self._p(x), x.shape[1], self._p(w_in_out), self._p(bias),
                                            bias.numel() if bias is not None else 0, act, self._p(y), y.shape[1], self._stream()))
        return y

    def linear_dgrad_ex(self, dy, n_cols, y, act, w_out_in, dx, accumulate=False):
        M = dy.shape[0]
        N, K = w_out_in.shape
        assert n_cols == N and dy.shape[1] >= N and tuple(dx.shape) == (M, K) and (y is None or y.shape == dy.shape)
        for t in (dy, y, w_out_in, dx):
            assert t is None or (t.dtype == torch.float32 and t.is_contiguous() and t.is_cuda)
        self._ck(self.lib.eve_linear_dgrad_ex(M, K, N, self._p(dy), dy.shape[1], self._p(y), act, self._p(w_out_in), self._p(dx), K,
                                              int(bool(accumulate)), self._stream()))
        return dx

    def tail_head_pose(self, h_left, h_right, cat, col):
        BT = h_left.numel() // 2
        for t in (h_left, h_right, cat):
            assert t.dtype == torch.float32 and t.is_contiguous() and t.is_cuda
        assert h_right.numel() == 2 * BT and cat.shape[0] == 2 * BT and cat.shape[1] >= col + 4
        self._ck(self.lib.eve_tail_head_pose(BT, self._p(h_left), self._p(h_right), self._p(cat), cat.shape[1], col, self._stream()))

    def tail_outputs_fwd(self, g2, p2):
        M = g2.shape[0]
        assert tuple(g2.shape) == (M, 4) and tuple(p2.shape) == (M, 4) and g2.is_contiguous() and p2.is_contiguous()
        gaze = torch.empty((M, 2), dtype=torch.float32, device=g2.device)
        pupil = torch.empty((M,), dtype=torch.float32, device=g2.device)
        self._ck(self.lib.eve_tail_outputs_fwd(M, self._p(g2), self._p(p2), self._p(gaze), self._p(pupil), self._stream()))
        return gaze, pupil

    def tail_outputs_bwd(self, dg, dp, g_full, coeff_ang, coeff_l1):
        BT = dp[0].numel()
        for t in (dg[0], dg[1], dp[0], dp[1]):
            assert t.dtype == torch.float32 and t.is_contiguous()
        assert g_full is None or (g_full.dtype == torch.float32 and g_full.numel() == 1 and g_full.is_cuda)
        d_g2 = torch.empty((2 * BT, 4), dtype=torch.float32, device=dp[0].device)
        d_p2 = torch.empty((2 * BT, 4), dtype=torch.float32, device=dp[0].device)
        self._ck(self.lib.eve_tail_outputs_bwd(BT, self._p(dg[0]), self._p(dg[1]), self._p(dp[0]), self._p(dp[1]), self._p(g_full),
                                               float(coeff_ang), float(coeff_l1), self._p(d_g2), self._p(d_p2), self._stream()))
        return d_g2, d_p2

    def linear_dgrad(self, dy, y, act, w_out_in):
        M, N = dy.shape
        K = w_out_in.shape[1]
        assert dy.dtype == torch.float32 and dy.is_contiguous() and tuple(w_out_in.shape) == (N, K)
        dx = torch.empty((M, K), dtype=torch.float32, device=dy.device)
        self._ck(self.lib.eve_linear_dgrad(M, K, N, self._p(dy), self._p(y), act, self._p(w_out_in), self._p(dx),
                                           self._stream()))
        return dx

    def linear_wgrad(self, dy, y, act, x, dw_out_in, db):
        M, N = dy.shape
        K = x.shape[1]
        assert tuple(dw_out_in.shape) == (N, K) and dw_out_in.dtype == torch.float32 and dw_out_in.is_contiguous()
        assert x.is_contiguous() and dy.is_contiguous() and (db is None or (db.numel() == N and db.is_contiguous()))
        self._ck(self.lib.eve_linear_wgrad(M, K, N, self._p(dy), self._p(y), act, self._p(x), self._p(dw_out_in),
                                           self._p(db), self._stream()))

    def bias_grad(self, dy, db):
        C = dy.shape[-1]
        M = dy.numel() // C
        assert db.dtype == torch.float32 and db.numel() == C
        self._ck(self.lib.eve_bias_grad(dt_code(dy.dtype), M, C, self._p(dy), self._p(db), self._stream()))
        return db

    def instnorm_stats(self, x, eps=1e-5):
        N, H, W, C = x.shape
        mr = torch.empty((N, C, 2), dtype=torch.float32, device=x.device)
        self._timed('in_stats', 0.0, lambda: self._ck(self.lib.eve_instnorm_stats(
            dt_code(x.dtype), N, H * W, C, self._p(x), eps, self._p(mr), self._stream())), (x,))
        return mr

    def instnorm_act_fwd(self, x, mr, gamma, beta, res, act):
        N, H, W, C = x.shape
        y = torch.empty_like(x)
        self._timed('in_fwd', 0.0, lambda: self._ck(self.lib.eve_instnorm_act_fwd(
            dt_code(x.dtype), N, H * W, C, self._p(x), self._p(mr), self._p(self._f32(gamma, 'gamma')),
            self._p(self._f32(beta, 'beta')), self._p(res), act, self._p(y), self._stream())), (x, res, y))
        return y

    def instnorm_act_bwd(self, dy, y, x, mr, gamma, act, want_dres, beta=None, dx_add=None):
        N, H, W, C = x.shape
        dx = torch.empty_like(x)
        dres = torch.empty_like(x) if want_dres else None
        sums = torch.empty((N, C, 2), dtype=torch.float32, device=x.device)
        self._timed('in_bwd', 0.0, lambda: self._ck(self.lib.eve_instnorm_act_bwd(
            dt_code(x.dtype), N, H * W, C, self._p(dy), self._p(y), self._p(x), self._p(mr),
            self._p(self._f32(gamma, 'gamma')), self._p(self._f32(beta, 'beta')), act, self._p(dx), self._p(dres),
            self._p(sums), self._p(dx_add), self._stream())), (dy, x, y, dy, x, y, dx, dres, dx_add))
        return dx, dres, sums

    def instnorm_act2_fwd(self, xs, mrs, gamma_a, beta_a, gamma_b, beta_b, act):
        x, x2 = xs[0], (xs[1] if len(xs) > 1 else None)
        N, H, W, C = x.shape
        C2 = x2.shape[-1] if x2 is not None else 0
        y_a = torch.empty((N, H, W, C + C2), dtype=x.dtype, device=x.device)
        y_b = torch.empty_like(y_a) if gamma_b is not None else None
        self._timed('in_fwd', 0.0, lambda: self._ck(self.lib.eve_instnorm_act2_fwd(
            dt_code(x.dtype), N, H * W, C, self._p(x), self._p(mrs[0]), self._p(self._f32(gamma_a, 'gamma')),
            self._p(self._f32(beta_a, 'beta')), self._p(self._f32(gamma_b, 'gamma')), self._p(self._f32(beta_b, 'beta')), act,
            self._p(y_a), self._p(y_b), C + C2, C2, self._p(x2), self._p(mrs[1] if x2 is not None else None), self._stream())),
            (x, x2, y_a, y_b))
        return y_a, y_b

    def instnorm_act2_bwd(self, dy_a, dy_b, xs, mrs, gamma_a, beta_a, gamma_b, beta_b, act):
        x, x2 = xs[0], (xs[1] if len(xs) > 1 else None)
        N, H, W, C = x.shape
        C2 = x2.shape[-1] if x2 is not None else 0
        assert dy_a.shape[-1] == C + C2
        dx = torch.empty_like(x)
        dx2 = torch.empty_like(x2) if x2 is not None else None
        sums_a = torch.empty((N, C + C2, 2), dtype=torch.float32, device=x.device)
        sums_b = torch.empty_like(sums_a) if dy_b is not None else None
        self._timed('in_bwd', 0.0, lambda: self._ck(self.lib.eve_instnorm_act2_bwd(
            dt_code(x.dtype), N, H * W, C, self._p(dy_a), self._p(dy_b), C + C2, self._p(x), self._p(mrs[0]),
            self._p(self._f32(gamma_a, 'gamma')), self._p(self._f32(beta_a, 'beta')), self._p(self._f32(gamma_b, 'gamma')),
            self._p(self._f32(beta_b, 'beta')), act, self._p(dx), self._p(sums_a), self._p(sums_b), C2, self._p(x2),
            self._p(mrs[1] if x2 is not None else None), self._p(dx2), self._stream())),
            (dy_a, dy_b, x, x2, dy_a, dy_b, x, x2, dx, dx2))
        return ([dx] if x2 is None else [dx, dx2]), sums_a, sums_b

    def instnorm_fwd_fused(self, x, gamma, beta, res, act, eps=1e-5, want_mask=False):
        N, H, W, C = x.shape
        y = torch.empty_like(x)
        mr = torch.empty((N, C, 2), dtype=torch.float32, device=x.device)
        mask = torch.empty((x.numel() * x.element_size() // 16,), dtype=torch.uint8, device=x.device) if want_mask else None
        st = self._timed('in_fwd', 0.0, lambda: self.lib.eve_instnorm_fwd_fused(
            dt_code(x.dtype), N, H * W, C, self._p(x), self._p(self._f32(gamma, 'gamma')), self._p(self._f32(beta, 'beta')),
            self._p(res), act, eps, self._p(y), self._p(mr), self._p(mask), self._stream()), (x, res, y, mask))
        if st == -1:
            if self.prof:
                self.prof.pop()
            return None
        self._ck(st)
        return (y, mr, mask) if want_mask else (y, mr)

    def instnorm_bwd_fused(self, dy, y, x, mr, gamma, act, want_dres, dy2=None, mask=None, beta=None, dx_add=None):
        N, H, W, C = x.shape
        dx = torch.empty_like(x)
        dres = torch.empty_like(x) if want_dres else None
        sums = torch.empty((N, C, 2), dtype=torch.float32, device=x.device)
        st = self._timed('in_bwd', 0.0, lambda: self.lib.eve_instnorm_bwd_fused(
            dt_code(x.dtype), N, H * W, C, self._p(dy), self._p(dy2), self._p(None if mask is not None else y), self._p(x), self._p(mr),
            self._p(self._f32(gamma, 'gamma')), self._p(self._f32(beta, 'beta')), act, self._p(dx), self._p(dres), self._p(sums), self._p(mask),
            self._p(dx_add), self._stream()), (dy, dy2, y if mask is None else mask, x, dx, dres, dx_add))
        if st == -1:
            if self.prof:
                self.prof.pop()
            return None
        self._ck(st)
        return dx, dres, sums

    def sum_rows(self, t):
        assert t.dtype == torch.float32 and t.is_contiguous()
        out = torch.empty(t.shape[1:], dtype=torch.float32, device=t.device)
        self._ck(self.lib.eve_sum_rows(t.shape[0], out.numel(), self._p(t), self._p(out), self._stream()))
        return out

    def sum_rows_pairs(self, sums, out0, out1):
        N, C, two = sums.shape
        assert two == 2 and sums.dtype == torch.float32 and sums.is_contiguous()
        for o in (out0, out1):
            assert o.dtype == torch.float32 and o.is_contiguous() and o.numel() == C
        self._ck(self.lib.eve_sum_rows_pairs(N, C, self._p(sums), self._p(out0), self._p(out1), self._stream()))

    def act_bwd(self, dy, y, act):
        dx = torch.empty_like(dy)
        self._ck(self.lib.eve_act_bwd(dt_code(dy.dtype), dy.numel(), self._p(dy), self._p(y), act,
                                      self._p(dx), self._stream()))
        return dx

    def add(self, a, b):
        out = torch.empty_like(a)
        self._ck(self.lib.eve_add(dt_code(a.dtype), a.numel(), self._p(a), self._p(b), self._p(out),
                                  self._stream()))
        return out

    def maxpool3x3s2_fwd(self, x):
        N, IH, IW, C = x.shape
        OH, OW = (IH - 1) // 2 + 1, (IW - 1) // 2 + 1
        y = torch.empty((N, OH, OW, C), dtype=x.dtype, device=x.device)
        idx = torch.empty((N, OH, OW, C), dtype=torch.uint8, device=x.device)
        self._ck(self.lib.eve_maxpool3x3s2_fwd(dt_code(x.dtype), N, IH, IW, C, self._p(x), self._p(y),
                                               self._p(idx), self._stream()))
        return y, idx

    def maxpool3x3s2_bwd(self, dy, idx, in_hw):
        N, OH, OW, C = dy.shape
        IH, IW = in_hw
        dx = torch.empty((N, IH, IW, C), dtype=dy.dtype, device=dy.device)
        self._ck(self.lib.eve_maxpool3x3s2_bwd(dt_code(dy.dtype), N, IH, IW, C, self._p(dy), self._p(idx),
                                               self._p(dx), self._stream()))
        return dx
# ... 514 lines not shown
```

### eve_amd/ops.py

```python

import torch

from . import kernels as K
from .kernels import (ACT_LEAKY, ACT_NONE, ACT_RELU, ACT_SELU, ACT_SIGMOID, ACT_TANH,
                      HALF_DTYPES, default_kernels, dispatch_flag)


class _LazyGroup(object):
    __slots__ = ('F', 'ohwi', 'transpose', 'w')

    def __init__(self, F, ohwi, transpose):
        self.F, self.ohwi, self.transpose, self.w = F, ohwi, transpose, None

    def weights(self):
        if self.w is None:
            self.w = pixel_group_weights(self.ohwi, self.F, self.transpose)
        return self.w

    def __getitem__(self, i):
        return self.F if i == 0 else self.weights()

    def __iter__(self):
        yield self.F
        yield self.weights()
# ... 309 lines not shown


class StemDgradPack(object):
    __slots__ = ('weight', 'dtype', 'w')

    def __init__(self, weight, dtype):
        self.weight, self.dtype, self.w = weight, dtype, None

    def get(self):
        if self.w is None:
            self.w = default_kernels().stem_dgrad_pack(self.weight.detach().float(), self.dtype)
        return self.w

    def patch_grads(self, dconv, rows):
        dx = default_kernels().stem_dgrad(dconv.contiguous(), self.get(), self.weight.shape[1])
        out, r = [], 0
        for n in rows:
            out.append(dx[r:r + n])
            r += n
        return out


class StemPatchGradFn(torch.autograd.Function):

    @staticmethod
    def forward(ctx, y, dgrad_pack, *patches):
        dgrad_pack.get()
        ctx.dgrad_pack, ctx.rows = dgrad_pack, tuple(p.shape[0] for p in patches)
        return y.view_as(y)

    @staticmethod
    def backward(ctx, dy):
        grads = ctx.dgrad_pack.patch_grads(dy, ctx.rows)
        return (dy, None) + tuple(g if need else None for g, need in zip(grads, ctx.needs_input_grad[2:]))


def conv2d(x, weight, bias, pack, stride=1, pad=0, act=ACT_NONE, acc=None, want_stats=False):
    if want_stats:
        return Conv2dFn.apply(x, weight, bias, pack, stride, pad, act, acc, True)
    return Conv2dFn.apply(x, weight, bias, pack, stride, pad, act, acc)


class LinearFn(torch.autograd.Function):

    @staticmethod
    def forward(ctx, x, weight, bias, pack, act):
        k = default_kernels()
        cout_p, _, _, cin_p = pack.ohwi.shape
        b = None
        if bias is not None:
            b = bias.detach().float()
            if b.numel() != cout_p:
                b = torch.nn.functional.pad(b, (0, cout_p - b.numel()))
            b = b.contiguous()
        y = k.linear_fwd(x.contiguous(), pack.ihwo.view(cin_p, cout_p), b, act)
        ctx.pack, ctx.act, ctx.has_bias = pack, act, bias is not None
        ctx.wshape = tuple(weight.shape)
        ctx.w_direct = weight if _direct_grad_ok(weight) else None
        ctx.b_direct = bias if (bias is not None and _direct_grad_ok(bias)) else None
        _note_use(ctx.w_direct, ctx.needs_input_grad[1])
        _note_use(ctx.b_direct, ctx.needs_input_grad[2])
        ctx.save_for_backward(x, y if act != ACT_NONE else None)
        return y

    @staticmethod
    def backward(ctx, dy):
        k = default_kernels()
        x, y = ctx.saved_tensors
        pack, act = ctx.pack, ctx.act
        cout_p, _, _, cin_p = pack.ohwi.shape
        O, I = pack.shape_oihw[0], pack.shape_oihw[1]
        dy = dy.contiguous()
        dx = dw = db = None
        if ctx.needs_input_grad[0]:
            dx = k.linear_dgrad(dy, y, act, pack.ohwi.view(cout_p, cin_p))
        want_w, want_b = ctx.needs_input_grad[1], ctx.has_bias and ctx.needs_input_grad[2]
        if want_w or want_b:
            wp, bp = ctx.w_direct, ctx.b_direct
            w_dir = wp is not None and (cout_p, cin_p) == (O, I)
            b_dir = want_b and bp is not None and cout_p == O
            dwbuf = wp.grad.view(O, I) if w_dir else torch.zeros((cout_p, cin_p), dtype=torch.float32, device=x.device)
            dbbuf = None
            if want_b:
                dbbuf = bp.grad if b_dir else torch.zeros((cout_p,), dtype=torch.float32, device=x.device)
            k.linear_wgrad(dy, y, act, x.contiguous(), dwbuf, dbbuf)
            if w_dir:
                _notify_grad_ready(wp)
            elif want_w:
                dw = dwbuf[:O, :I].reshape(ctx.wshape)
            if b_dir:
                _notify_grad_ready(bp)
            elif want_b:
                db = dbbuf[:O]
        return dx, dw, db, None, None


def _pad_bias(bias, n):
    if bias is None:
        return None
    b = bias.detach().float()
    if b.numel() != n:
        b = torch.nn.functional.pad(b, (0, n - b.numel()))
    return b.contiguous()


class _TailGrads(object):

    def __init__(self, device):
        self.device, self.items = device, []

    def target(self, weight, bias, pack, want_w, want_b):
        cout_p, _, _, cin_p = pack.ohwi.shape
        O, I = pack.shape_oihw[0], pack.shape_oihw[1]
        w_dir = want_w and _direct_grad_ok(weight) and (cout_p, cin_p) == (O, I)
        b_dir = want_b and bias is not None and _direct_grad_ok(bias) and cout_p == O
        dw = weight.grad.view(O, I) if w_dir else torch.zeros((cout_p, cin_p), dtype=torch.float32, device=self.device)
        db = None
        if want_b and bias is not None:
            db = bias.grad if b_dir else torch.zeros((cout_p,), dtype=torch.float32, device=self.device)
        self.items.append((weight, bias, pack, want_w, want_b, w_dir, b_dir, dw, db))
        return dw, db

    def results(self):
        out = []
        for weight, bias, pack, want_w, want_b, w_dir, b_dir, dw, db in self.items:
            O, I = pack.shape_oihw[0], pack.shape_oihw[1]
            gw = gb = None
            if w_dir:
                _notify_grad_ready(weight)
            elif want_w:
                gw = dw[:O, :I].reshape(tuple(weight.shape))
            if b_dir:
                _notify_grad_ready(bias)
            elif want_b and bias is not None:
                gb = db[:O]
            out.append((gw, gb))
        return out


class EyeTailLossFn(torch.autograd.Function):

    @staticmethod
    def forward(ctx, feats, h_left, h_right, targets, c_ang, c_l1, net, packs, B, T):
        k = default_kernels()
        cnn, cell = net.cnn_layers, net.rnn_cells[0]
        p_fc, p0, p2, p_ih, p_hh, pg0, pg2, pp0, pp2 = packs
        M, dev = feats.shape[0], feats.device
        BT = B * T
        assert M == 2 * BT and feats.dtype == torch.float32
        f32 = lambda t: t.detach()
        new = lambda n: torch.empty((M, n), dtype=torch.float32, device=dev)
        feats = feats.contiguous()
        cin0 = p0.ohwi.shape[3]
        c0 = new(cin0)
        k.linear_fwd_ex(feats, 512, p_fc.ihwo.view(512, 128), f32(cnn.fc.bias), ACT_NONE, c0)
        k.tail_head_pose(h_left.detach().float().contiguous(), h_right.detach().float().contiguous(), c0, 128)
        a1 = k.linear_fwd(c0, p0.ihwo.view(cin0, 128), f32(net.fc_common[0].bias), ACT_SELU)
        a2 = k.linear_fwd(a1, p2.ihwo.view(128, 128), f32(net.fc_common[2].bias), ACT_NONE)
        gi = k.linear_fwd(a2, p_ih.ihwo.view(128, 384), f32(cell.bias_ih), ACT_NONE)
        hs, gates, hn_pre = k.gru_scan_fwd(gi.view(2 * B, T, 384), p_hh.ihwo.view(128, 384), f32(cell.bias_hh), None)
        hs2 = hs.view(M, 128)
        g1 = k.linear_fwd(hs2, pg0.ihwo.view(128, 128), f32(net.fc_to_gaze[0].bias), ACT_SELU)
        g2 = k.linear_fwd_ex(g1, 128, pg2.ihwo.view(128, 4), None, ACT_TANH, new(4))
        p1 = k.linear_fwd(hs2, pp0.ihwo.view(128, 128), f32(net.fc_to_pupil[0].bias), ACT_SELU)
        p2_ = k.linear_fwd_ex(p1, 128, pp2.ihwo.view(128, 4), f32(net.fc_to_pupil[2].bias), ACT_RELU, new(4))
        gaze, pupil = k.tail_outputs_fwd(g2, p2_)
        tg_l, tg_r, vg_l, vg_r, tp_l, tp_r, vp_l, vp_r = targets
        terms, dg, dp = k.eye_losses((gaze[:BT].view(B, T, 2), gaze[BT:].view(B, T, 2)), (tg_l, tg_r), (vg_l, vg_r),
                                     (pupil[:BT].view(B, T), pupil[BT:].view(B, T)), (tp_l, tp_r), (vp_l, vp_r), c_ang, c_l1)
        ctx.net, ctx.packs, ctx.coeffs, ctx.BT = net, packs, (c_ang, c_l1), (B, T)
        ctx.params = EyeTailLossFn.tail_parameters(net)
        for p_ in ctx.params:
            _note_use(p_, True)
        ctx.set_materialize_grads(False)
        ctx.save_for_backward(feats, c0, a1, a2, hs, gates, hn_pre, g1, g2, p1, p2_, dg[0], dg[1], dp[0], dp[1])
        ctx.mark_non_differentiable(gaze, pupil, hs)
        return tuple(terms.unbind(0)) + (gaze, pupil, hs)

    @staticmethod
    def tail_parameters(net):
        cnn, cell = net.cnn_layers, net.rnn_cells[0]
        return [cnn.fc.weight, cnn.fc.bias, net.fc_common[0].weight, net.fc_common[0].bias, net.fc_common[2].weight,
                net.fc_common[2].bias, cell.weight_ih, cell.bias_ih, cell.weight_hh, cell.bias_hh, net.fc_to_gaze[0].weight,
                net.fc_to_gaze[0].bias, net.fc_to_gaze[2].weight, net.fc_to_pupil[0].weight, net.fc_to_pupil[0].bias,
                net.fc_to_pupil[2].weight, net.fc_to_pupil[2].bias]

    @staticmethod
    def backward(ctx, g_ang_l, g_l1_l, g_ang_r, g_l1_r, g_full, *unused):
        if any(g is not None for g in (g_ang_l, g_l1_l, g_ang_r, g_l1_r)):
            raise NotImplementedError('EyeTailLossFn propagates d(full_loss) only: use losses.eyenet_loss_terms for the separate terms')
        if g_full is None:
            return (None,) * 10
        k = default_kernels()
        feats, c0, a1, a2, hs, gates, hn_pre, g1, g2, p1, p2_, dg_l, dg_r, dp_l, dp_r = ctx.saved_tensors
        p_fc, p0, p2, p_ih, p_hh, pg0, pg2, pp0, pp2 = ctx.packs
        (w_fc, b_fc, w0, b0, w2, b2, w_ih, b_ih, w_hh, b_hh, wg0, bg0, wg2, wp0, bp0, wp2, bp2) = ctx.params
        B, T = ctx.BT
        M, dev = feats.shape[0], feats.device
        cin0 = p0.ohwi.shape[3]
        hs2 = hs.view(M, 128)
        g_full = g_full.detach().float().contiguous()
        d_g2, d_p2 = k.tail_outputs_bwd((dg_l, dg_r), (dp_l, dp_r), g_full, ctx.coeffs[0], ctx.coeffs[1])
        d_g1 = k.linear_dgrad(d_g2, g2, ACT_TANH, pg2.ohwi.view(4, 128))
        d_hs = k.linear_dgrad(d_g1, g1, ACT_SELU, pg0.ohwi.view(128, 128))
        d_p1 = k.linear_dgrad(d_p2, p2_, ACT_RELU, pp2.ohwi.view(4, 128))
        k.linear_dgrad_ex(d_p1, 128, p1, ACT_SELU, pp0.ohwi.view(128, 128), d_hs, accumulate=True)
        dgi, dgh, _ = k.gru_scan_bwd(d_hs.view(2 * B, T, 128), p_hh.ohwi.view(384, 128), None, hs, gates, hn_pre, False)
        dgi2, dgh2 = dgi.view(M, 384), dgh.view(M, 384)
        d_a2 = k.linear_dgrad(dgi2, None, ACT_NONE, p_ih.ohwi.view(384, 128))
        d_a1 = k.linear_dgrad(d_a2, None, ACT_NONE, p2.ohwi.view(128, 128))
        d_c0 = k.linear_dgrad(d_a1, a1, ACT_SELU, p0.ohwi.view(128, cin0))
        d_feats = None
        if ctx.needs_input_grad[0]:
            d_feats = torch.empty((M, 512), dtype=torch.float32, device=dev)
            k.linear_dgrad_ex(d_c0, 128, None, ACT_NONE, p_fc.ohwi.view(128, 512), d_feats)
        gw = lambda p_: p_.grad.view(p_.shape[0], -1) if p_.dim() == 2 else p_.grad
        k.linear_wgrad_batch([
            dict(dY=d_c0, X=feats, dW=gw(w_fc), db=gw(b_fc)),
            dict(dY=d_a1, Y=a1, act=ACT_SELU, X=c0, K1=w0.shape[1], dW=gw(w0), db=gw(b0)),
            dict(dY=d_a2, X=a1, dW=gw(w2), db=gw(b2)),
            dict(dY=dgi2, X=a2, dW=gw(w_ih), db=gw(b_ih)),
            dict(dY=dgh2, X=hs2, x_shift_T=T, dW=gw(w_hh), db=gw(b_hh)),
            dict(dY=d_g1, Y=g1, act=ACT_SELU, X=hs2, dW=gw(wg0), db=gw(bg0)),
            dict(dY=d_g2, Y=g2, act=ACT_TANH, X=g1, dW=gw(wg2)),
            dict(dY=d_p1, Y=p1, act=ACT_SELU, X=hs2, dW=gw(wp0), db=gw(bp0)),
            dict(dY=d_p2, Y=p2_, act=ACT_RELU, X=p1, dW=gw(wp2), db=gw(bp2))])
        for p_ in ctx.params:
            _notify_grad_ready(p_)
        return (d_feats,) + (None,) * 9


def linear(x2d, weight, bias, pack, act=ACT_NONE):
    M, C = x2d.shape
    if x2d.dtype == torch.float32 and pack.ohwi.dtype == torch.float32 and pack.ihwo is not None \
            and dispatch_flag(default_kernels(), 'small_linear', 1):
        return LinearFn.apply(x2d, weight, bias, pack, act)
    y = Conv2dFn.apply(x2d.view(M, 1, 1, C), weight, bias, pack, 1, 0, act)
    return y.view(M, y.shape[-1])


def _wgrad_pixel_pairs(k, x, dy, ks, stride, pad, dwp, db):
    N, H, W, ci = x.shape
    co = dy.shape[3]
    wg = W // 2
    if (x.dtype not in HALF_DTYPES or stride != 1 or pad != (ks - 1) // 2 or ks not in (1, 3) or min(ci, co) != 8 or max(ci, co) > 32 or
            W % 2 or wg < 32 or wg > 128 or (wg & (wg - 1)) or N * H * wg < (1 << 20) or tuple(dy.shape[:3]) != (N, H, W) or
            not hasattr(k, 'dispatch_config')):
        return False
    dwg = torch.zeros((2 * co, ks, ks, 2 * ci), dtype=torch.float32, device=x.device)
    dbg = torch.zeros((2 * co,), dtype=torch.float32, device=x.device) if db is not None else None
    k.conv2d_wgrad(x.view(N, H, wg, 2 * ci), dy.view(N, H, wg, 2 * co), ks, ks, 1, pad, dwg, db=dbg)
    idx = _pixel_group_index(co, ci, ks, 2, False, x.device)
    flat = torch.zeros((co * ks * ks * ci + 1,), dtype=torch.float32, device=x.device)
    flat.index_add_(0, idx.reshape(-1), dwg.reshape(-1))
    dwp += flat[:-1].view(co, ks, ks, ci)
    if db is not None:
        db += dbg.view(2, co).sum(0)
    return True


def _wgrad_into(k, x, dy, weight, pack, stride, pad, db=None):
    cout_p, KH, KW, cin_p = pack.ohwi.shape
    O, I = pack.shape_oihw[0], pack.shape_oihw[1]
    if _direct_grad_ok(weight) and (cout_p, cin_p) == (O, I):
        k.conv2d_wgrad(x, dy, KH, KW, stride, pad, weight.grad.permute(0, 2, 3, 1), algo=pack.algo, db=db)
        _notify_grad_ready(weight)
        return None
    dwp = torch.zeros((cout_p, KH, KW, cin_p), dtype=torch.float32, device=x.device)
    k.conv2d_wgrad(x, dy, KH, KW, stride, pad, dwp, algo=pack.algo, db=db)
    return dwp[:O, :, :, :I].permute(0, 3, 1, 2)


def _in_fwd(k, x, res, act, eps, want_mask=False):
    fused = k.instnorm_fwd_fused(x, None, None, res, act, eps, want_mask=True) if want_mask else \
        k.instnorm_fwd_fused(x, None, None, res, act, eps)
    if fused is not None:
        return fused
    mr = k.instnorm_stats(x, eps)
    y = k.instnorm_act_fwd(x, mr, None, None, res, act)
    return (y, mr, None) if want_mask else (y, mr)


def _in_bwd(k, dy, y, x, mr, act, want_dres, dy2=None):
    mask = y if (y is not None and y.dtype == torch.uint8) else None
    out = k.instnorm_bwd_fused(dy, None if mask is not None else y, x, mr, None, act, want_dres, dy2=dy2, mask=mask) \
        if mask is not None else k.instnorm_bwd_fused(dy, y, x, mr, None, act, want_dres, dy2=dy2)
    if out is None:
        assert mask is None, 'a sign mask exists only where the fused kernel fits'
        if dy2 is not None:
            dy = k.add(dy, dy2)
        out = k.instnorm_act_bwd(dy, y, x, mr, None, act, want_dres)
    return out[0], out[1]


def _block_forward(k, x, packs, stride, eps):
    p1, p2, pd = packs
    a = k.conv2d_fwd(x, p1.ohwi, None, stride, 1, ACT_NONE, algo=p1.algo)
    an, mr1 = _in_fwd(k, a, None, ACT_RELU, eps)
    b = k.conv2d_fwd(an, p2.ohwi, None, 1, 1, ACT_NONE, algo=p2.algo)
    if pd is not None:
        d = k.conv2d_fwd(x, pd.ohwi, None, stride, 0, ACT_NONE, algo=pd.algo)
        idn, mrd = _in_fwd(k, d, None, ACT_NONE, eps)
    else:
        d = mrd = None
        idn = x
    y, mr2, ymask = _in_fwd(k, b, idn, ACT_RELU, eps, want_mask=True)
    return y, (x, a, mr1, an, b, mr2, ymask if ymask is not None else y, d, mrd)


def _block_backward(k, dy, dy2, saved, weights, packs, stride, need_w):
    x, a, mr1, an, b, mr2, y, d, mrd = saved
    p1, p2, pd = packs
    w1, w2, wd = weights
    hw = (x.shape[1], x.shape[2])
    db, g = _in_bwd(k, dy, y, b, mr2, ACT_RELU, True, dy2=dy2)
    dw2 = _wgrad_into(k, an, db, w2, p2, 1, 1) if need_w[1] else None
    dan = k.conv2d_dgrad(db, p2.ihwo, (an.shape[1], an.shape[2]), 1, 1, algo=p2.algo)
    da, _ = _in_bwd(k, dan, None, a, mr1, ACT_RELU, False)
    dw1 = _wgrad_into(k, x, da, w1, p1, stride, 1) if need_w[0] else None
    dwd = None
    dx1 = k.conv2d_dgrad(da, p1.ihwo, hw, stride, 1, algo=p1.algo)
    if pd is not None:
        dd, _ = _in_bwd(k, g, None, d, mrd, ACT_NONE, False)
        dwd = _wgrad_into(k, x, dd, wd, pd, stride, 0) if need_w[2] else None
        dx1 = k.conv2d_dgrad(dd, pd.ihwo, hw, stride, 0, algo=pd.algo, accumulate_into=dx1)
        g = None
    return (dx1, None, dw1, dw2, dwd) if g is None else (g, dx1, dw1, dw2, dwd)


class ResNetTrunkFn(torch.autograd.Function):

    @staticmethod
    def forward(ctx, x, x8, x_padded, spec, eps, *weights):
        k = default_kernels()
        stem_pack, blocks = spec[:2]
        saved = []
        if stem_pack is not None:
            y, idx, mr = k.stem_fwd_fused(x_padded, stem_pack.ohwi, eps)
            saved += [x_padded, y, idx, mr]
        else:
            y = x
        for packs, stride in blocks:
            y, sv = _block_forward(k, y, packs, stride, eps)
            saved += list(sv)
        ctx.spec, ctx.weights = spec, weights
        ctx.patch_rows = tuple(t.shape[0] for t in (x, x8) if t is not None) if stem_pack is not None else ()
        for i, w in enumerate(weights):
            if _direct_grad_ok(w):
                _note_use(w, ctx.needs_input_grad[5 + i])
        ctx.save_for_backward(*saved)
        return y

    @staticmethod
    def backward(ctx, dy):
        k = default_kernels()
        stem_pack, blocks = ctx.spec[:2]
        saved = list(ctx.saved_tensors)
        weights = list(ctx.weights)
        need_w = list(ctx.needs_input_grad[5:])
        grads = [None] * len(weights)
        wpos = len(weights)
        spos = len(saved)
        d_a, d_b = dy.contiguous(), None
        for packs, stride in reversed(blocks):
            nw = 3 if packs[2] is not None else 2
            wpos -= nw
            spos -= 9
            ws = tuple(weights[wpos:wpos + nw]) + ((None,) if nw == 2 else ())
# ... 526 lines not shown
```

### include/eve_hip.h

```cpp
#ifndef EVE_HIP_H_
#define EVE_HIP_H_

#include <stddef.h>
#include <stdint.h>

#ifdef __cplusplus
extern "C" {
#endif

#define EVE_ABI_VERSION 10

typedef void* eve_stream_t;

enum { EVE_DT_F32 = 0, EVE_DT_BF16 = 1, EVE_DT_F16 = 2 };
enum {
    EVE_ACT_NONE = 0,
    EVE_ACT_RELU = 1,
    EVE_ACT_LEAKY = 2,
    EVE_ACT_SELU = 3,
    EVE_ACT_TANH = 4,
    EVE_ACT_SIGMOID = 5
};

int eve_abi_version(void);
const char* eve_last_kernel(void);
const char* eve_last_error(void);
typedef struct eve_dispatch_config {
    int struct_bytes;
    int conv_impl_v1;
    int conv_tile_big;
    int conv_halo;
    int conv_ws64;
    int conv_wg8;
    int conv_wg8_min_tiles;
    int conv_wg8_s2_min_tiles;
    int halo_persist;
    int wgrad_target_wgs;
    int wgrad_min_rows;
    int wgrad_halo;
    int wgrad_wg8;
    int wg64_th, wg64_nreg;
    int wg64_fixed;
    int in_split;
    int in_min_threads;
    int in_stats_one_pass;
    int stem_split;
    int in_trunk_kernels;
    int stem_fused_wgrad;
    int stem_fwd_pairs;
    int conv1x1_stream;
    int conv3x3_stream;
    int in_big_planes;
    int cgru_seq_max_b;
    int cgru_scan;
    int small_linear;
    int tail_loss_node;
    int bucket_elems;
    int gate_wait_polls;
    long long wgrad_halo_min_m;
} eve_dispatch_config;
int eve_get_dispatch_config(eve_dispatch_config* out);
int eve_get_default_dispatch_config(eve_dispatch_config* out);
int eve_set_dispatch_config(const eve_dispatch_config* cfg);

typedef struct eve_conv_desc {
    int dtype;
    int N, IH, IW, Cin;
    int OH, OW, Cout;
    int KH, KW, stride, pad;
} eve_conv_desc;

#define EVE_EPI_ACCUMULATE 0x100
int eve_conv2d_fwd(const eve_conv_desc* d, const void* x, const void* w_ohwi, const float* bias,
                   int epi_act, const float* in_scale_shift, int pro_act, void* y,
                   eve_stream_t stream);
int eve_conv2d_fwd_stats(const eve_conv_desc* d, const void* x, const void* w_ohwi, const float* bias, int epi_act, void* y,
                         float* mean_rstd, float eps, int* stats_written, eve_stream_t stream);
int eve_conv2d_dgrad(const eve_conv_desc* d, const void* dy, const void* w_ihwo, void* dx,
                     void* workspace, unsigned long long workspace_bytes, eve_stream_t stream);
int eve_conv2d_dgrad_acc(const eve_conv_desc* d, const void* dy, const void* w_ihwo, void* dx,
                     eve_stream_t stream);
int eve_conv2d_wgrad(const eve_conv_desc* d, const void* x, const void* dy,
                     const float* in_scale_shift, int pro_act, float* dw_ohwi,
                     void* workspace, unsigned long long workspace_bytes, eve_stream_t stream);
int eve_conv2d_wgrad_bias(const eve_conv_desc* d, const void* x, const void* dy, float* dw_ohwi, float* db,
                          void* workspace, unsigned long long workspace_bytes, eve_stream_t stream);
int eve_stem_pack_input(int dtype , int N, int C, int IH, int IW, const float* src_nchw, void* x_padded,
                        eve_stream_t stream);
int eve_stem7x7s2_fwd(int dtype, int N, int IH, int IW, const void* x_padded, const void* w_ohwi8, void* y,
                      eve_stream_t stream);
int eve_frames_u8_to_nchw(long long N, int H, int W, int C, const uint8_t* src_nhwc, float scale, float shift,
                          int has_shift, float* dst_nchw, eve_stream_t stream);
int eve_frames_u8_to_stem(int dtype, long long N, int C, int IH, int IW, const uint8_t* src_nhwc, float scale, float shift,
                          void* x_padded, eve_stream_t stream);
int eve_stem_fwd_fused(int dtype, int N, int IH, int IW, const void* x_padded, const void* w_ohwi8, float eps,
                       void* y_pool, uint8_t* idx, float* mean_rstd, eve_stream_t stream);
int eve_stem_bwd_wgrad(int dtype, int N, int IH, int IW, const void* x_padded, const void* w_ohwi8, const float* mean_rstd,
                       const void* dy_pool, const void* dy_pool2, const void* y_pool, const uint8_t* idx, float* dw,
                       void* workspace, unsigned long long workspace_bytes, eve_stream_t stream);
unsigned long long eve_stem_bwd_wgrad_workspace(int dtype, int N, int IH);
int eve_stem_wgrad(int dtype, int N, int IH, int IW, const void* x_padded, const void* dconv, float* dw, eve_stream_t stream);
int eve_stem_bwd_dx(int dtype, int N, int IH, int IW, const void* x_padded, const void* w_ohwi8, const float* mean_rstd,
                    const void* dy_pool, const void* dy_pool2 , const void* y_pool, const uint8_t* idx, void* dx, eve_stream_t stream);
int eve_stem_dgrad_pack(int dtype, int C, const float* w_oihw, void* w_packed, eve_stream_t stream);
int eve_stem_dgrad(int dtype, int N, int IH, int IW, int C, const void* dconv, const void* w_packed, float* dx_nchw,
                   eve_stream_t stream);
int eve_linear_fwd(int M, int K, int N, const float* x, const float* w_in_out, const float* bias, int act,
                   float* y, eve_stream_t stream);
int eve_linear_dgrad(int M, int K, int N, const float* dy, const float* y, int act, const float* w_out_in,
                     float* dx, eve_stream_t stream);
int eve_linear_wgrad(int M, int K, int N, const float* dy, const float* y, int act, const float* x,
                     float* dw_out_in, float* db, eve_stream_t stream);
int eve_linear_fwd_ex(int M, int K, int N, const float* x, int ldx, const float* w_in_out, const float* bias, int n_bias,
                      int act, float* y, int ldy, eve_stream_t stream);
int eve_linear_dgrad_ex(int M, int K, int N, const float* dy, int lddy, const float* y, int act, const float* w_out_in,
                        float* dx, int lddx, int accumulate, eve_stream_t stream);
int eve_tail_head_pose(int BT, const float* h_left, const float* h_right, float* cat, int ld, int col, eve_stream_t stream);
int eve_tail_outputs_fwd(int M, const float* g2, const float* p2, float* gaze, float* pupil, eve_stream_t stream);
int eve_tail_outputs_bwd(int BT, const float* dg_l, const float* dg_r, const float* dp_l, const float* dp_r, const float* g_full,
                         float coeff_ang, float coeff_l1, float* d_g2, float* d_p2, eve_stream_t stream);
int eve_eye_losses(int B, int T, const float* const* g_pred, const float* const* g_tgt, const uint8_t* const* g_val,
                   const float* const* p_pred, const float* const* p_tgt, const uint8_t* const* p_val,
                   float coeff_ang, float coeff_l1, float* terms, float* const* dg, float* const* dp,
                   eve_stream_t stream);
#define EVE_VEC_TERMS_MAX 32
typedef struct eve_vec_term { const float* pred; const float* tgt; const unsigned char* valid; float* dpred; int D; int kind; } eve_vec_term;
int eve_vector_terms(const eve_vec_term* terms, int n, int B, int T, float* out, eve_stream_t stream);
int eve_gaze_to_pog(long long N, const float* g, const float* origin, const float* R, const float* inv_cam,
                    const float* ppm, const float* head_R, const float* kappa, float screen_w, float screen_h,
                    float* g_out, float* pog_mm, float* pog_px, float* jac, eve_stream_t stream);
int eve_gaze_to_pog_bwd(long long N, const float* jac, const float* dg_out, const float* dmm, const float* dpx,
                        float* dg, eve_stream_t stream);
int eve_combined_gaze(long long N, const float* origin, const float* pog_mm, const float* R, const float* cam,
                      float* g, eve_stream_t stream);
int eve_make_heatmaps(long long N, int H, int W, const float* centres_px, const uint8_t* validity, float sigma,
                      float screen_w, float screen_h, float* out, eve_stream_t stream);
int eve_make_heatmaps_bwd(long long N, int H, int W, const float* centres_px, float sigma, float screen_w, float screen_h,
                          const float* dout, float* dcentres, eve_stream_t stream);
int eve_soft_argmax_fwd(long long N, int H, int W, const float* heat, float screen_w, float screen_h, float* pog_px,
                        float* stats, eve_stream_t stream);
int eve_soft_argmax_bwd(long long N, int H, int W, const float* heat, const float* stats, const float* dpog,
                        float screen_w, float screen_h, float* dheat, eve_stream_t stream);
int eve_bias_grad(int dtype, long long M, int C, const void* dy, float* db, eve_stream_t stream);

int eve_instnorm_stats(int dtype, int N, int HW, int C, const void* x, float eps, float* mean_rstd,
                       eve_stream_t stream);
int eve_instnorm_act_fwd(int dtype, int N, int HW, int C, const void* x, const float* mean_rstd,
                         const float* gamma, const float* beta, const void* res, int act, void* y,
                         eve_stream_t stream);
int eve_instnorm_act_bwd(int dtype, int N, int HW, int C, const void* dy, const void* y,
                         const void* x, const float* mean_rstd, const float* gamma, const float* beta, int act,
                         void* dx, void* dres, float* sums, const void* dx_add, eve_stream_t stream);

int eve_instnorm_act2_fwd(int dtype, int N, int HW, int C, const void* x, const float* mean_rstd,
                          const float* gamma_a, const float* beta_a, const float* gamma_b, const float* beta_b,
                          int act, void* y_a, void* y_b, int ldy, int C2, const void* x2, const float* mean_rstd2,
                          eve_stream_t stream);
int eve_instnorm_act2_bwd(int dtype, int N, int HW, int C, const void* dy_a, const void* dy_b, int lddy,
                          const void* x, const float* mean_rstd, const float* gamma_a, const float* beta_a,
                          const float* gamma_b, const float* beta_b, int act, void* dx, float* sums_a,
                          float* sums_b, int C2, const void* x2, const float* mean_rstd2, void* dx2, eve_stream_t stream);

int eve_instnorm_fwd_fused(int dtype, int N, int HW, int C, const void* x, const float* gamma,
                           const float* beta, const void* res, int act, float eps, void* y,
                           float* mean_rstd, unsigned char* sign_mask, eve_stream_t stream);
int eve_instnorm_bwd_fused(int dtype, int N, int HW, int C, const void* dy, const void* dy2, const void* y,
                           const void* x, const float* mean_rstd, const float* gamma, const float* beta, int act,
                           void* dx, void* dres, float* sums, const unsigned char* sign_mask, const void* dx_add, eve_stream_t stream);

int eve_sum_rows(int rows, int cols, const float* in, float* out, eve_stream_t stream);
int eve_sum_rows_pairs(int rows, int C, const float* in, float* out0, float* out1, eve_stream_t stream);

int eve_act_bwd(int dtype, long long n, const void* dy, const void* y, int act, void* dx,
                eve_stream_t stream);
int eve_add(int dtype, long long n, const void* a, const void* b, void* out, eve_stream_t stream);

int eve_maxpool3x3s2_fwd(int dtype, int N, int IH, int IW, int C, const void* x, void* y,
                         uint8_t* idx, eve_stream_t stream);
int eve_maxpool3x3s2_bwd(int dtype, int N, int IH, int IW, int C, const void* dy,
                         const uint8_t* idx, void* dx, eve_stream_t stream);
int eve_in_relu_maxpool_fwd(int dtype, int N, int IH, int IW, int C, const void* x,
                            const float* mean_rstd, void* y, uint8_t* idx, eve_stream_t stream);
int eve_in_relu_maxpool_bwd(int dtype, int N, int IH, int IW, int C, const void* dy_pool,
                            const void* y_pool, const uint8_t* idx, const void* x,
                            const float* mean_rstd, void* dx, eve_stream_t stream);
int eve_avgpool_fwd(int dtype, int N, int HW, int C, const void* x, void* y, eve_stream_t stream);
int eve_avgpool_bwd(int dtype, int N, int HW, int C, const void* dy, void* dx, eve_stream_t stream);
int eve_avgpool_fwd_f32(int dtype, int N, int HW, int C, const void* x, float* y, eve_stream_t stream);
int eve_avgpool_bwd_f32(int dtype, int N, int HW, int C, const float* dy, void* dx, eve_stream_t stream);
int eve_adaptive_maxpool_fwd(int dtype, int N, int IH, int IW, int OH, int OW, int C, const void* x,
                             void* y, int32_t* idx, eve_stream_t stream);
int eve_adaptive_maxpool_bwd(int dtype, int N, int IH, int IW, int OH, int OW, int C,
                             const void* dy, const int32_t* idx, const void* add, void* dx, eve_stream_t stream);
int eve_bilinear_fwd(int dtype, int N, int IH, int IW, int OH, int OW, int C, const void* x, void* y,
                     eve_stream_t stream);
int eve_bilinear_bwd(int dtype, int N, int IH, int IW, int OH, int OW, int C, const void* dy,
                     void* dx, eve_stream_t stream);

int eve_nchw_to_nhwc(int dtype_dst, int N, int C, int H, int W, int Cpad, const float* src_nchw,
                     void* dst_nhwc, eve_stream_t stream);
int eve_nhwc_to_nchw(int dtype_src, int N, int C, int H, int W, int Cpad, const void* src_nhwc,
                     float* dst_nchw, eve_stream_t stream);
int eve_cast(int dtype_src, int dtype_dst, long long n, const void* src, void* dst,
             eve_stream_t stream);
int eve_pack_weights(int dtype_dst, int Cout, int taps, int Cin, const float* w_ohwi, void* dst_ohwi,
                     void* dst_ihwo, eve_stream_t stream);
#define EVE_PACK_BATCH_MAX 48
typedef struct eve_pack_item {
    const float* w_ohwi; void* dst_ohwi; void* dst_ihwo;
    int Cout, taps, Cin;
    int src_Cout, src_Cin;
} eve_pack_item;
int eve_pack_weights_batch(int dtype_dst, int count, const eve_pack_item* items , eve_stream_t stream);

int eve_gru_scan_fwd(int S, int T, int H, const float* gi, const float* whh_t, const float* bhh,
                     const float* h0, float* hs, float* gates, float* hn_pre, eve_stream_t stream);
int eve_gru_scan_bwd(int S, int T, int H, const float* dhs, const float* whh, const float* h0,
                     const float* hs, const float* gates, const float* hn_pre, float* dgi, float* dgh,
                     float* dh0, eve_stream_t stream);
int eve_rnn_scan_fwd(int S, int T, int H, const float* gi, const float* whh_t, const float* bhh, const float* h0,
                     float* hs, eve_stream_t stream);
int eve_rnn_scan_bwd(int S, int T, int H, const float* dhs, const float* whh, const float* hs, float* dpre,
                     float* dh0, eve_stream_t stream);
int eve_lstm_scan_fwd(int S, int T, int H, const float* gi, const float* whh_t, const float* bhh, const float* h0,
                      const float* c0, float* hs, float* cs, float* gates, eve_stream_t stream);
int eve_lstm_scan_bwd(int S, int T, int H, const float* dhs, const float* dcs, const float* whh, const float* c0,
                      const float* hs, const float* cs, const float* gates, float* dpre, float* dh0, float* dc0,
                      eve_stream_t stream);

int eve_cgru_scan_fwd(int dtype, int B, int T, const void* xs, const void* h0, const void* w1, const float* b1, const void* w2,
                      const float* b2, void* hs, void* hs_tm, void* ru, void* rh, void* og, eve_stream_t stream);
int eve_cgru_scan_bwd(int dtype, int B, int T, const void* dhs_tm, const void* ru, const void* og, const void* hs_tm, const void* h0,
                      const void* w1t, const void* w2t, void* dg1_all, void* dg2_all, void* dxs_tm, void* dh0,
                      eve_stream_t stream);
int eve_crnn_scan_fwd(int B, int T, const float* xs, const float* h0, const float* w, const float* bias, float* hs,
                      float* hs_tm, eve_stream_t stream);
int eve_crnn_scan_bwd(int B, int T, const float* dhs_tm, const float* hs_tm, const float* wt, float* dpre_all, float* dxs_tm,
                      float* dh0, eve_stream_t stream);
int eve_clstm_scan_fwd(int B, int T, const float* xs, const float* h0, const float* c0, const float* w, const float* bias,
                       float* hs, float* cs, eve_stream_t stream);
int eve_cgru_scan_fwd_c(int dtype, int B, int T, int C, const void* xs, const void* h0, const void* w1, const float* b1,
                        const void* w2, const float* b2, void* hs, void* hs_tm, void* ru, void* rh, void* og, eve_stream_t stream);
int eve_cgru_scan_bwd_c(int dtype, int B, int T, int C, const void* dhs_tm, const void* ru, const void* og, const void* hs_tm,
                        const void* h0, const void* w1t, const void* w2t, void* dg1_all, void* dg2_all, void* dxs_tm, void* dh0,
                        eve_stream_t stream);
int eve_crnn_scan_fwd_c(int B, int T, int C, const float* xs, const float* h0, const float* w, const float* bias, float* hs,
                        float* hs_tm, eve_stream_t stream);
int eve_crnn_scan_bwd_c(int B, int T, int C, const float* dhs_tm, const float* hs_tm, const float* wt, float* dpre_all,
                        float* dxs_tm, float* dh0, eve_stream_t stream);
int eve_clstm_scan_fwd_c(int B, int T, int C, const float* xs, const float* h0, const float* c0, const float* w, const float* bias,
                         float* hs, float* cs, eve_stream_t stream);
int eve_clstm_scan_fwd_train_c(int B, int T, int C, const float* xs, const float* h0, const float* c0, const float* w,
                               const float* bias, float* hs, float* cs, float* gates_tm, float* cs_tm, float* hs_tm,
                               eve_stream_t stream);
int eve_clstm_scan_bwd_c(int B, int T, int C, const float* dhs_tm, const float* dcs_tm, const float* gates_tm, const float* cs_tm,
                         const float* c0, const float* wt, float* dpre_all, float* dxs_tm, float* dh0, float* dc0,
                         eve_stream_t stream);
int eve_cgru_gates1(int dtype, long long P, int C, const void* g1, const void* h, void* ru, void* rh,
                    eve_stream_t stream);
int eve_cgru_gates2(int dtype, long long P, int C, const void* g2, const void* ru, const void* h,
                    void* o, void* hnew, eve_stream_t stream);
int eve_cgru_gates2_bwd(int dtype, long long P, int C, const void* dhnew, const void* ru,
                        const void* h, const void* o, void* dg2, void* dru, void* dh,
                        eve_stream_t stream);
int eve_cgru_gates1_bwd(int dtype, long long P, int C, const void* drh, const void* dru,
                        const void* ru, const void* h, void* dg1, void* dh, eve_stream_t stream);

int eve_clstm_gates_fwd(int dtype, long long P, int C, const void* gates, const void* c_prev, void* h,
                        void* c, eve_stream_t stream);
int eve_clstm_gates_bwd(int dtype, long long P, int C, const void* dh, const void* dc_in, const void* gates,
                        const void* c_prev, void* dgates, void* dc_prev, eve_stream_t stream);

int eve_heatmap_head_fwd(int dtype, long long pixels, int Cpad, const void* logits, float* out, eve_stream_t stream);
int eve_heatmap_head_bwd(int dtype, long long pixels, int Cpad, const float* dy, const float* y, void* dlogits,
                         eve_stream_t stream);
int eve_heatmap_loss_fwd(int kind, int B, int T, int HW, const float* pred, const float* gt, const uint8_t* validity,
                         float* per_map, float* loss, float* w, eve_stream_t stream);
int eve_heatmap_loss_bwd(int kind, int BT, int HW, const float* pred, const float* gt, const float* w,
                         const float* upstream, float* dpred, eve_stream_t stream);

#define EVE_WGRAD_BATCH_MAX 12
typedef struct eve_wgrad_problem {
    const float* dY;
    const float* Y;
    const float* X;
    const float* X2;
    float* dW;
    float* db;
    int M, N, K, K1, K2, act, rows_per_split ;
    int ldY;
    int ldX, ldW;
    int x_shift_T;
    int reserved;
} eve_wgrad_problem;
typedef struct eve_wgrad_batch { int n; int first_block[EVE_WGRAD_BATCH_MAX]; eve_wgrad_problem p[EVE_WGRAD_BATCH_MAX]; } eve_wgrad_batch;
int eve_linear_wgrad_batch(const eve_wgrad_problem* problems, int n, eve_stream_t stream);

int eve_gate_signal(unsigned* flag, eve_stream_t stream);
int eve_gate_wait(const unsigned* flag, unsigned value, const unsigned* value_ref, unsigned* timeouts, float* poison,
                  unsigned max_polls, eve_stream_t stream);

#define EVE_SUMSQ_WORKSPACE 1024
int eve_sumsq(long long n, const float* g, float* out, float* workspace, eve_stream_t stream);
typedef struct eve_adam_guard {
    int step;
    int skipped_total;
    int skipped_run;
    int good_run;
    float loss_scale;
    float applied;
    float clip;
    float bc1, bc2_sqrt;
    int skipped_gate;
    float reserved[2];
} eve_adam_guard;
int eve_adam_step(long long n, float* p, const float* g, float* m, float* v, const float* sumsq,
                  float max_norm, float gscale, float lr, float beta1, float beta2, float eps,
                  float weight_decay, int step, eve_adam_guard* guard, int check_finite, const float* lr_dev,
                  const float* poison, eve_stream_t stream);

typedef struct eve_eye_tail_weights {
    const float* fc_w;  const float* fc_b;
    const float* c0_w;  const float* c0_b;
    const float* c2_w;  const float* c2_b;
    const float* ih_w;  const float* ih_b;
    const float* hh_w;  const float* hh_b;
    const float* g0_w;  const float* g0_b;
    const float* g2_w;
    const float* p0_w;  const float* p0_b;
    const float* p2_w;  const float* p2_b;
} eve_eye_tail_weights;
int eve_eye_tail_stream_fwd(int S, int T, const float* feats, const float* head_pose, const eve_eye_tail_weights* weights,
                            float* h, const int* reset, float* gaze, float* pupil, float* hs, eve_stream_t stream);
int eve_stream_state_rows(int dtype, int S, long long row_elems, long long src_stride, long long dst_stride, const void* src,
                          void* dst, const int* reset, eve_stream_t stream);
int eve_eye_tail_stream_fwd_len(int S, int T, const float* feats, const float* head_pose, const eve_eye_tail_weights* weights,
                                float* h, const int* reset, const int* lengths, float* gaze, float* pupil, float* hs,
                                eve_stream_t stream);
int eve_stream_state_rows_at(int dtype, int S, int T, long long row_elems, long long frame_stride, long long src_stride,
                             long long dst_stride, const void* src, void* dst, const int* lengths, eve_stream_t stream);
int eve_stream_mask_plan(int B, int T, const uint8_t* mask, const uint8_t* pose_valid, const int* lengths, int* count, int* perm,
                         int* inv, uint8_t* eye_valid, uint8_t* valid, eve_stream_t stream);
int eve_stream_permute_rows(int S, int T, long long row_bytes, long long frame_stride_bytes, long long seq_stride_bytes,
                            const void* src, void* dst, const int* index, eve_stream_t stream);
int eve_screen_u8_area_to_nchw(long long N, int IH, int IW, int C, const uint8_t* src_nhwc, int OH, int OW, float* dst_nchw,
                               eve_stream_t stream);
int eve_screen_u8_area_bgr_to_nchw(long long N, int IH, int IW, int C, const uint8_t* src_nhwc, int OH, int OW, float* dst_nchw,
                                   eve_stream_t stream);
int eve_eye_warp_u8_to_nchw(long long N, int IH, int IW, int C, const uint8_t* frames_nhwc, const float* warps, int OH, int OW,
                            float* dst_nchw, eve_stream_t stream);
int eve_eye_warp_u8_to_stem(int dtype , long long N, int IH, int IW, int C, const uint8_t* frames_nhwc,
                            const float* warps, int OH, int OW, void* x_padded, eve_stream_t stream);
int eve_eye_warp_lens_u8_to_nchw(long long N, int IH, int IW, int C, const uint8_t* frames_nhwc, const float* warps, const float* lens,
                                 int OH, int OW, float* dst_nchw, eve_stream_t stream);
int eve_eye_warp_lens_u8_to_stem(int dtype , long long N, int IH, int IW, int C, const uint8_t* frames_nhwc,
                                 const float* warps, const float* lens, int OH, int OW, void* x_padded, eve_stream_t stream);
enum { EVE_PIX_BGR = 0, EVE_PIX_BGRA = 1, EVE_PIX_NV12 = 2, EVE_PIX_I420 = 3, EVE_PIX_YUYV = 4 };
enum { EVE_YUV_BT601 = 0, EVE_YUV_BT709 = 1, EVE_YUV_JFIF = 2 };
int eve_eye_warp_fmt_to_nchw(int format, int matrix, long long N, int IH, int IW, const uint8_t* frames, const float* warps,
                             const float* lens , int OH, int OW, float* dst_nchw, eve_stream_t stream);
int eve_eye_warp_fmt_to_stem(int dtype , int format, int matrix, long long N, int IH, int IW,
                             const uint8_t* frames, const float* warps, const float* lens , int OH, int OW,
                             void* x_padded, eve_stream_t stream);
int eve_screen_area_fmt_to_nchw(int format, int matrix, long long N, int IH, int IW, const uint8_t* src, int OH, int OW,
                                float* dst_nchw, eve_stream_t stream);
enum { EVE_SURF_RGB = 0, EVE_SURF_YUV = 1 };
typedef struct eve_surface {
    int struct_bytes;
    int kind;
    int width, height;
    long long frame_stride;
    long long frame_bytes;
    long long offset[3];
    int pitch[3];
    int step[3];
    int xshift, yshift;
} eve_surface;
int eve_eye_warp_surface_to_nchw(const eve_surface* surface, int matrix, long long N, const uint8_t* frames, const float* warps,
                                 const float* lens , int OH, int OW, float* dst_nchw, eve_stream_t stream);
int eve_eye_warp_surface_to_stem(int dtype , const eve_surface* surface, int matrix, long long N,
                                 const uint8_t* frames, const float* warps, const float* lens , int OH, int OW,
                                 void* x_padded, eve_stream_t stream);
int eve_screen_area_surface_to_nchw(const eve_surface* surface, int matrix, long long N, const uint8_t* src, int OH, int OW,
                                    float* dst_nchw, eve_stream_t stream);
enum { EVE_PIX_RGB = 5, EVE_PIX_RGBA = 6 };
int eve_overlay_render(int in_format, int out_format, int matrix, long long N, int IH, int IW, const uint8_t* src, uint8_t* dst,
                       int M, const float* centres, const uint8_t* marker_valid, const int* marker_table, float sx, float sy,
                       const float* heat , int HH, int HW, int heat_rgb, int amax,
                       const uint8_t* inset , int ih, int iw, int ix0, int iy0, int zoom, int mirror,
                       const uint8_t* frame_valid , eve_stream_t stream);
int eve_eye_pose_normalize(long long N, const float* pose, int OH, int OW, float* head_R, float* o, float* R, float* warp, float* h,
                           uint8_t* valid, eve_stream_t stream);
int eve_eye_pose_normalize_rt(long long N, int frames_per_row, const float* rows, int row_stride, const float* head_R, const float* head_t,
                              const uint8_t* valid_in , int OH, int OW, float* o, float* R, float* warp, float* h,
                              uint8_t* valid, eve_stream_t stream);
int eve_face_pose_solve(long long S, int T, int L, int landmark_cols, const float* landmarks, const float* rig,
                        const int* lengths , double* state , const int* reset ,
                        float* head_R, float* head_t, float* reproj_rms, uint8_t* valid, eve_stream_t stream);
int eve_undistort_points(long long N, const float* points, const float* lens, long long lens_stride, double* xy, uint8_t* ok,
                         eve_stream_t stream);
int eve_face_pose_solve_ex(long long S, int T, int L, int landmark_cols, const float* landmarks, const float* rig,
                           const float* lens , double huber_px, const int* lengths ,
                           double* state , const int* reset , float* head_R, float* head_t,
                           float* reproj_rms, uint8_t* valid, uint8_t* inliers, eve_stream_t stream);

int eve_calib_append(long long B, int T, int E, const float* g, const float* head_R, const float* origin, const float* R,
                     const float* inv_cam, const float* ppm, const float* target, const uint8_t* valid ,
                     const int* lengths , const uint8_t* eye_valid , int C, double* samples, int* count,
                     int* dropped, eve_stream_t stream);
int eve_calib_fit(long long S, int C, const double* samples, const int* count , const uint8_t* select ,
                  double huber_mm, int min_samples, double* kappa, double* rms_mm, int* used, int* inliers, uint8_t* ok,
                  float* kappa_store , uint8_t* ok_store , eve_stream_t stream);

int eve_screen_calib_append(long long B, int T, const float* pog, const float* origin, const float* inv_cam, const float* ppm,
                            const float* target, const uint8_t* valid , const int* lengths ,
                            const uint8_t* frame_valid , double W, double H, int C, double* samples, int* count,
                            int* dropped, eve_stream_t stream);
int eve_screen_calib_fit(long long S, int C, const double* samples, const int* count ,
                         const uint8_t* select , int mode, int kind, double huber_mm, int min_samples, double max_shift_mm,
                         double* coef, double* report, int* used, int* inliers, int* solves, uint8_t* ok,
                         double* coef_store , uint8_t* kind_store , eve_stream_t stream);
int eve_screen_calib_apply(long long B, int T, const float* px_in, const float* ppm, const double* coef, const uint8_t* kind, double W,
                           double H, float* px_out, eve_stream_t stream);

int eve_gaze_events(long long B, int T, const float* pog, const float* origin, const float* inv_cam, const float* ppm,
                    const double* frame_time , const uint8_t* valid , const int* lengths ,
                    const int* reset , const int* flush , double fps, double min_cutoff_hz, double beta,
                    double d_cutoff_hz, int velocity_from_raw, double saccade_deg_s, double min_fixation_s, double max_gap_s, double* state,
                    int F, double* store, int* count, int* dropped, float* filtered, float* velocity, uint8_t* event, int* fixation_id,
                    float* fixation_px, float* fixation_ms, uint8_t* fixating, eve_stream_t stream);

int eve_gaze_events_ex(long long B, int T, const float* pog, const float* origin, const float* inv_cam, const float* ppm,
                       const double* frame_time , const uint8_t* valid , const int* lengths ,
                       const int* reset , const int* flush , double fps, double min_cutoff_hz, double beta,
                       double d_cutoff_hz, int velocity_from_raw, double saccade_deg_s, double min_fixation_s, double max_gap_s, double* state,
                       int F, double* store, int* count, int* dropped, float* filtered, float* velocity, uint8_t* event, int* fixation_id,
                       float* fixation_px, float* fixation_ms, uint8_t* fixating, uint8_t* sample ,
                       double* sample_time , double* gaze_vector , eve_stream_t stream);

int eve_gaze_saccades(long long B, int T, const uint8_t* sample, const double* sample_time, const double* gaze_vector, const float* point,
                      const uint8_t* event, const float* velocity, const int* fixation_id, const int* lengths ,
                      const int* reset , double min_amplitude_deg, double min_duration_s, double max_duration_s,
                      int max_missing, double* state, double* table, int S, double* store, int* count, int* dropped, int* saccade_id,
                      float* saccade_ms, eve_stream_t stream);

int eve_gaze_pursuits(long long B, int T, const uint8_t* sample, const double* sample_time, const double* gaze_vector, const float* point,
                      const uint8_t* event, const float* velocity, const int* fixation_id, const float* target ,
                      const int* lengths , const int* reset , double window_s, double min_window_s,
                      double pursuit_deg_s, double min_straightness, double settle_s, double min_duration_s, double min_amplitude_deg,
                      int max_missing, double* state, double* table, int S, double* store, int* count, int* dropped, uint8_t* gaze_class,
                      int* pursuit_id, float* pursuit_ms, float* gaze_velocity_windowed, float* gaze_straightness, float* pursuit_gain,
                      eve_stream_t stream);

typedef struct eve_eye_gate_params {
    double max_reproj_px;
    double pitch_lo, pitch_hi, yaw_lo[2], yaw_hi[2];
    double close_ratio, open_ratio, baseline_rate, baseline_rise;
    int min_inliers;
    int min_inside;
    int hold_frames, max_closed_frames;
} eve_eye_gate_params;
int eve_eye_gate(long long B, int T, const uint8_t* pose_valid , const float* reproj_rms ,
                 const uint8_t* inliers , const float* warp , const float* h ,
                 const float* contours , int C, const int* lengths , const int* reset ,
                 int IW, int IH, int OW, int OH, const eve_eye_gate_params* params, double* state, int capacity, double* blinks, int* count,
                 int* dropped, uint8_t* usable, uint8_t* reason, float* openness, uint8_t* blink, eve_stream_t stream);

int eve_gaze_history_plan(long long B, int T, const float* pog , const double* frame_time ,
                          const uint8_t* valid , const uint8_t* valid_key ,
                          const int* lengths , const int* reset , double fps, double ln_decay,
                          int weight_seconds, double max_gap_s, double gain, int MW, int MH, double screen_w, double screen_h, double* state,
                          double* coef, int* clear, eve_stream_t stream);
int eve_gaze_history_update(long long B, int T, int MH, int MW, const double* coef, const int* clear, const float* heat ,
                            double alpha, double floor, float* map, float* frames , eve_stream_t stream);

int eve_gaze_aoi(long long B, int T, int A, const float* pog, const float* shapes, int shapes_per_frame,
                 const double* frame_time , const uint8_t* valid , const uint8_t* valid_key ,
                 const int* fixation_id , const uint8_t* fixating , const int* lengths ,
                 const int* reset , const int* flush , double fps, double max_gap_s, double* state,
                 double* table, int* trans, int visit_capacity, double* visits, int* count, int* dropped, int* id, long long* mask,
                 float* visit_ms, eve_stream_t stream);

int eve_pupil_track(long long B, int T, const float* size, const uint8_t* eye_valid ,
                    const double* frame_time , const int* lengths , const int* reset ,
                    const int* flush , const float* luminance ,
                    const uint8_t* baseline_mark , double fps, double min_mm, double max_mm, double max_speed_mm_s,
// ... 19 lines not shown
```

Measured before the change: 90100 frames/s.

## Fuse EyeNet tail MLP chains into per-row-block kernels for forward and backward

Adds fused kernels that compute the pre-GRU linear chain (fc, c0, c2, ih projection) and the gaze/pupil heads, plus their backward passes, in a few launches. Each block processes 16 rows end to end with MFMA, replacing a sequence of separate small linear, activation and output kernels. The goal is to remove launch overhead and intermediate global traffic in the latency-bound tail. It also adds a slab-reduce helper and entry point, and moves shared linear helpers into a header. The fused path is on by default, gated by weight shapes, and keeps the old path as a fallback; the trade-off is low occupancy on small row counts.

```diff
diff --git a/eve_amd/_lib.py b/eve_amd/_lib.py
--- a/eve_amd/_lib.py
+++ b/eve_amd/_lib.py
@@ -20,7 +20,7 @@
         'conv_wg8_s2_min_tiles', 'halo_persist', 'wgrad_target_wgs', 'wgrad_min_rows', 'wgrad_halo', 'wgrad_wg8',
         'wg64_th', 'wg64_nreg', 'wg64_fixed', 'in_split', 'in_min_threads', 'in_stats_one_pass', 'stem_split',
         'in_trunk_kernels', 'stem_fused_wgrad', 'stem_fwd_pairs', 'conv1x1_stream', 'conv3x3_stream', 'in_big_planes', 'cgru_seq_max_b',
-        'cgru_scan', 'small_linear', 'tail_loss_node', 'bucket_elems', 'gate_wait_polls')] + [('wgrad_halo_min_m', c_longlong)]
+        'cgru_scan', 'small_linear', 'tail_loss_node', 'bucket_elems', 'gate_wait_polls', 'tail_fused')] + [('wgrad_halo_min_m', c_longlong)]
 
     def as_dict(self):
         return {n: int(getattr(self, n)) for n, _ in self._fields_ if n != 'struct_bytes'}
@@ -77,6 +77,7 @@
     'eve_conv2d_dgrad_acc': [POINTER(ConvDesc), P, P, P, P],
     'eve_conv2d_wgrad': [POINTER(ConvDesc), P, P, P, I, P, P, ctypes.c_ulonglong, P],
     'eve_conv2d_wgrad_bias': [POINTER(ConvDesc), P, P, P, P, P, ctypes.c_ulonglong, P],
+    'eve_wgrad_slab_reduce': [P, P, L, I, I, P],
     'eve_get_dispatch_config': [POINTER(DispatchConfig)],
     'eve_get_default_dispatch_config': [POINTER(DispatchConfig)],
     'eve_set_dispatch_config': [POINTER(DispatchConfig)],
@@ -171,6 +172,10 @@
     'eve_sumsq': [L, P, P, P, P],
     'eve_adam_step': [L, P, P, P, P, P, F, F, F, F, F, F, F, I, P, I, P, P, P],
     'eve_eye_tail_stream_fwd': [I, I, P, P, POINTER(EyeTailWeights), P, P, P, P, P, P],
+    'eve_eye_tail_pre_fwd': [I, P, P, P, POINTER(EyeTailWeights), P, I, P, P, P, P],
+    'eve_eye_tail_heads_fwd': [I, P, POINTER(EyeTailWeights), P, P, P, P, P, P, P, P],
+    'eve_eye_tail_heads_bwd': [I, P, P, P, P, P, F, F, P, P, P, P, POINTER(EyeTailWeights), P, P, P, P, P, P],
+    'eve_eye_tail_pre_bwd': [I, P, P, POINTER(EyeTailWeights), P, P, P, I, P, P],
     'eve_stream_state_rows': [I, I, L, L, L, P, P, P, P],
     'eve_eye_tail_stream_fwd_len': [I, I, P, P, POINTER(EyeTailWeights), P, P, P, P, P, P, P],
     'eve_stream_state_rows_at': [I, I, I, L, L, L, L, P, P, P, P],
diff --git a/eve_amd/csrc/api.hip b/eve_amd/csrc/api.hip
--- a/eve_amd/csrc/api.hip
+++ b/eve_amd/csrc/api.hip
@@ -33,6 +33,7 @@
     c.wgrad_halo_min_m = 1ll << 20;
     c.cgru_seq_max_b = 384;
     c.cgru_scan = 1; c.small_linear = 1; c.tail_loss_node = 1; c.bucket_elems = 4 * 1024 * 1024; c.gate_wait_polls = 1 << 21;
+    c.tail_fused = 1;
     return c;
 }
 static void env_int(const char* name, int& field) { if (const char* e = getenv(name)) field = atoi(e); }
@@ -56,6 +57,7 @@
     env_int("EVE_CGRU_SEQ_MAX_B", c.cgru_seq_max_b);
     env_int("EVE_CGRU_SCAN", c.cgru_scan); env_int("EVE_SMALL_LINEAR", c.small_linear); env_int("EVE_TAIL_LOSS_NODE", c.tail_loss_node);
     env_int("EVE_BUCKET_ELEMS", c.bucket_elems); env_int("EVE_GATE_WAIT_POLLS", c.gate_wait_polls);
+    env_int("EVE_TAIL_FUSED", c.tail_fused);
     if (const char* e = getenv("EVE_WGRAD_HALO_MIN_M")) c.wgrad_halo_min_m = atoll(e);
     if (c.wgrad_min_rows < 64) c.wgrad_min_rows = 64;
     if (c.in_min_threads < 64) c.in_min_threads = 64;
diff --git a/eve_amd/csrc/conv_igemm.hip b/eve_amd/csrc/conv_igemm.hip
--- a/eve_amd/csrc/conv_igemm.hip
+++ b/eve_amd/csrc/conv_igemm.hip
@@ -773,6 +773,16 @@
 #define EVE_WGRAD_TR(T, WCO, WK, P2, MT) EVE_HNAME(T, "wgrad_tr_kernel<", ", " #WCO ", " #WK ", " #P2 ", mt" #MT ">"), ic<WCO>{}, ic<WK>{}, ic<P2>{}, ic<MT>{}
 
 static constexpr uint32_t WGRAD_WG8_T128_MIN_M = 65536;
+
+static void launch_slab_reduce(const float* slabs, float* dw, long long n4, int splits, bool wide, hipStream_t s) {
+    if (wide && (n4 + 31) / 32 <= 0x7fffffffll) {
+        hipLaunchKernelGGL(wgrad_slab_reduce_wide_kernel, dim3((unsigned)((n4 + 31) / 32)), dim3(256), 0, s, slabs, dw, n4, splits);
+    } else {
+        long long blocks = (n4 + 255) / 256;
+        if (blocks > 2048) blocks = 2048;
+        hipLaunchKernelGGL(wgrad_slab_reduce_kernel, dim3((unsigned)blocks), dim3(256), 0, s, slabs, dw, n4, splits);
+    }
+}
 
 template <typename T>
 static int launch_wgrad(const GatherParams& p, const void* x, const void* dy, const float* ss, int pro_act,
@@ -807,10 +817,7 @@
                 if (slab) {
                     EVE_LAUNCH(EVE_HNAME(T, "wgrad_wg8_kernel<", ", true>"), (wgrad_wg8_kernel<T, true>), dim3(tk * tc * splits), dim3(512), (size_t)128 * 1024, s, p,
                                (const T*)x, (const T*)dy, (float*)workspace, rows, (uint32_t)x_bytes, (uint32_t)dy_bytes);
-                    const long long n4 = (long long)(n / 4);
-                    long long blocks = (n4 + 255) / 256;
-                    if (blocks > 2048) blocks = 2048;
-                    hipLaunchKernelGGL(wgrad_slab_reduce_kernel, dim3((unsigned)blocks), dim3(256), 0, s, (const float*)workspace, dw, n4, (int)splits);
+                    launch_slab_reduce((const float*)workspace, dw, (long long)(n / 4), (int)splits, false, s);
                 } else {
                     EVE_LAUNCH(EVE_HNAME(T, "wgrad_wg8_kernel<", ", false>"), (wgrad_wg8_kernel<T, false>), dim3(tk * tc * splits), dim3(512), (size_t)128 * 1024, s, p,
                                (const T*)x, (const T*)dy, dw, rows, (uint32_t)x_bytes, (uint32_t)dy_bytes);
@@ -825,9 +832,7 @@
                 if (slab) {
                     EVE_LAUNCH(EVE_HNAME(T, "wgrad_wg8_t128_kernel<", ", true>"), (wgrad_wg8_t128_kernel<T, true>), dim3(tk * tc * splits), dim3(512), (size_t)128 * 1024,
                                s, p, (const T*)x, (const T*)dy, (float*)workspace, rows, (uint32_t)x_bytes, (uint32_t)dy_bytes);
-                    const long long n4 = (long long)(n / 4);
-                    hipLaunchKernelGGL(wgrad_slab_reduce_wide_kernel, dim3((unsigned)((n4 + 31) / 32)), dim3(256), 0, s, (const float*)workspace, dw, n4,
-                                       (int)splits);
+                    launch_slab_reduce((const float*)workspace, dw, (long long)(n / 4), (int)splits, true, s);
                 } else {
                     EVE_LAUNCH(EVE_HNAME(T, "wgrad_wg8_t128_kernel<", ", false>"), (wgrad_wg8_t128_kernel<T, false>), dim3(tk * tc * splits), dim3(512), (size_t)128 * 1024,
                                s, p, (const T*)x, (const T*)dy, dw, rows, (uint32_t)x_bytes, (uint32_t)dy_bytes);
@@ -1079,6 +1084,14 @@
     return 0;
 }
 
+extern "C" int eve_wgrad_slab_reduce(const float* slabs, float* dw, long long n, int splits, int wide, eve_stream_t stream) {
+    if (!slabs || !dw || n <= 0 || (n & 3) || splits <= 0 || ((uintptr_t)slabs & 15) || ((uintptr_t)dw & 15))
+        return set_error_msg("wgrad_slab_reduce: bad arguments (n a positive multiple of 4, 16-byte aligned pointers)");
+    launch_slab_reduce(slabs, dw, n / 4, splits, wide != 0, (hipStream_t)stream);
+    if (hipError_t e = hipGetLastError(); e != hipSuccess) return set_error(e, __func__);
+    return 0;
+}
+
 extern "C" int eve_stem_wgrad(int dtype, int N, int IH, int IW, const void* x_padded, const void* dconv, float* dw, eve_stream_t stream) {
     if ((dtype != EVE_DT_BF16 && dtype != EVE_DT_F16) || N <= 0 || IH <= 0 || IW <= 0 || (IH & 1) || (IW & 1) || !x_padded || !dconv || !dw)
         return set_error_msg("stem_wgrad: bad arguments");
diff --git a/eve_amd/csrc/linear_small.h b/eve_amd/csrc/linear_small.h
--- /dev/null
+++ b/eve_amd/csrc/linear_small.h
@@ -0,0 +1,79 @@
+#pragma once
+#include "common.h"
+
+namespace eve {
+
+constexpr int LM_T = 32;
+constexpr int LM_GW = 2;
+constexpr int LM_G = 4;
+
+struct LmFrag { float w[2][4]; float x[2][4]; };
+
+__device__ __forceinline__ void lm_mfma(f32x4_t (&acc)[2][2], const LmFrag& f) {
+#pragma unroll
+    for (int s = 0; s < 4; ++s)
+#pragma unroll
+        for (int a = 0; a < 2; ++a)
+#pragma unroll
+            for (int b = 0; b < 2; ++b) acc[a][b] = __builtin_amdgcn_mfma_f32_16x16x4f32(f.w[a][s], f.x[b][s], acc[a][b], 0, 0, 0);
+}
+
+__device__ __forceinline__ bool lm_reduce(f32x4_t (&acc)[2][2], float (*red)[16][64], const int wave, const int lane) {
+    if (wave) {
+#pragma unroll
+        for (int a = 0; a < 2; ++a)
+#pragma unroll
+            for (int b = 0; b < 2; ++b)
+#pragma unroll
+                for (int v = 0; v < 4; ++v) red[wave - 1][(a * 2 + b) * 4 + v][lane] = acc[a][b][v];
+    }
+    __syncthreads();
+    if (wave) return false;
+#pragma unroll
+    for (int w = 0; w < 3; ++w)
+#pragma unroll
+        for (int a = 0; a < 2; ++a)
+#pragma unroll
+            for (int b = 0; b < 2; ++b)
+#pragma unroll
+                for (int v = 0; v < 4; ++v) acc[a][b][v] += red[w][(a * 2 + b) * 4 + v][lane];
+    return true;
+}
+
+struct LmActGrad { float p0, n0, n1, q; };
+__device__ __forceinline__ LmActGrad lm_act_grad(const int act) {
+    switch (act) {
+        case EVE_ACT_RELU:    return {1.f, 0.f, 0.f, 0.f};
+        case EVE_ACT_LEAKY:   return {1.f, 0.01f, 0.f, 0.f};
+        case EVE_ACT_SELU:    return {EVE_SELU_SCALE, EVE_SELU_SCALE * EVE_SELU_ALPHA, 1.f, 0.f};
+        case EVE_ACT_TANH:    return {1.f, 1.f, 0.f, -1.f};
+        case EVE_ACT_SIGMOID: return {0.f, 0.f, 0.f, -1.f};
+        default:              return {1.f, 1.f, 0.f, 0.f};
+    }
+}
+__device__ __forceinline__ float lm_apply_grad(const float g, const float y, const LmActGrad& c, const bool sigmoid) {
+    const bool pos = y > 0.f;
+    float d = fmaf(pos ? 0.f : c.n1, y, pos ? c.p0 : c.n0);
+    d = fmaf(c.q * y, y, d);
+    if (sigmoid) d += y;
+    return g * d;
+}
+
+template <int N>
+__device__ __forceinline__ void lm_act_n(float (&v)[N], const int act) {
+#define LM_ALL(expr) _Pragma("unroll") for (int r = 0; r < N; ++r) { const float z = v[r]; v[r] = (expr); }
+    switch (act) {
+        case EVE_ACT_RELU:    LM_ALL(z > 0.f ? z : 0.f) break;
+        case EVE_ACT_LEAKY:   LM_ALL(z > 0.f ? z : 0.01f * z) break;
+        case EVE_ACT_SELU:    LM_ALL(EVE_SELU_SCALE * (z > 0.f ? z : EVE_SELU_ALPHA * (__expf(z) - 1.f))) break;
+        case EVE_ACT_TANH:    LM_ALL(tanhf(z)) break;
+        case EVE_ACT_SIGMOID: LM_ALL(1.f / (1.f + __expf(-z))) break;
+        default: break;
+    }
+#undef LM_ALL
+}
+__device__ __forceinline__ void lm_act16(float (&v)[2][2][4], const int act) { lm_act_n(reinterpret_cast<float (&)[16]>(v), act); }
+
+constexpr float LM_HALF_PI = 1.5707963267948966f;
+
+}
diff --git a/eve_amd/csrc/linear_small.hip b/eve_amd/csrc/linear_small.hip
--- a/eve_amd/csrc/linear_small.hip
+++ b/eve_amd/csrc/linear_small.hip
@@ -1,78 +1,7 @@
-#include "common.h"
+#include "linear_small.h"
 
 namespace eve {
 
-constexpr int LM_T = 32;
-constexpr int LM_GW = 2;
-constexpr int LM_G = 4;
-
-struct LmFrag { float w[2][4]; float x[2][4]; };
-
-__device__ __forceinline__ void lm_mfma(f32x4_t (&acc)[2][2], const LmFrag& f) {
-#pragma unroll
-    for (int s = 0; s < 4; ++s)
-#pragma unroll
-        for (int a = 0; a < 2; ++a)
-#pragma unroll
-            for (int b = 0; b < 2; ++b) acc[a][b] = __builtin_amdgcn_mfma_f32_16x16x4f32(f.w[a][s], f.x[b][s], acc[a][b], 0, 0, 0);
-}
-
-__device__ __forceinline__ bool lm_reduce(f32x4_t (&acc)[2][2], float (*red)[16][64], const int wave, const int lane) {
-    if (wave) {
-#pragma unroll
-        for (int a = 0; a < 2; ++a)
-#pragma unroll
-            for (int b = 0; b < 2; ++b)
-#pragma unroll
-                for (int v = 0; v < 4; ++v) red[wave - 1][(a * 2 + b) * 4 + v][lane] = acc[a][b][v];
-    }
-    __syncthreads();
-    if (wave) return false;
-#pragma unroll
-    for (int w = 0; w < 3; ++w)
-#pragma unroll
-        for (int a = 0; a < 2; ++a)
-#pragma unroll
-            for (int b = 0; b < 2; ++b)
-#pragma unroll
-                for (int v = 0; v < 4; ++v) acc[a][b][v] += red[w][(a * 2 + b) * 4 + v][lane];
-    return true;
-}
-
-struct LmActGrad { float p0, n0, n1, q; };
-__device__ __forceinline__ LmActGrad lm_act_grad(const int act) {
-    switch (act) {
-        case EVE_ACT_RELU:    return {1.f, 0.f, 0.f, 0.f};
-        case EVE_ACT_LEAKY:   return {1.f, 0.01f, 0.f, 0.f};
-        case EVE_ACT_SELU:    return {EVE_SELU_SCALE, EVE_SELU_SCALE * EVE_SELU_ALPHA, 1.f, 0.f};
-        case EVE_ACT_TANH:    return {1.f, 1.f, 0.f, -1.f};
-        case EVE_ACT_SIGMOID: return {0.f, 0.f, 0.f, -1.f};
-        default:              return {1.f, 1.f, 0.f, 0.f};
-    }
-}
-__device__ __forceinline__ float lm_apply_grad(const float g, const float y, const LmActGrad& c, const bool sigmoid) {
-    const bool pos = y > 0.f;
-    float d = fmaf(pos ? 0.f : c.n1, y, pos ? c.p0 : c.n0);
-    d = fmaf(c.q * y, y, d);
-    if (sigmoid) d += y;
-    return g * d;
-}
-
-__device__ __forceinline__ void lm_act16(float (&v)[2][2][4], const int act) {
-#define LM_ALL(expr)                                   \
-    _Pragma("unroll") for (int a = 0; a < 2; ++a)      \
-    _Pragma("unroll") for (int b = 0; b < 2; ++b)      \
-    _Pragma("unroll") for (int r = 0; r < 4; ++r) { const float z = v[a][b][r]; v[a][b][r] = (expr); }
-    switch (act) {
-        case EVE_ACT_RELU:    LM_ALL(z > 0.f ? z : 0.f) break;
-        case EVE_ACT_LEAKY:   LM_ALL(z > 0.f ? z : 0.01f * z) break;
-        case EVE_ACT_SELU:    LM_ALL(EVE_SELU_SCALE * (z > 0.f ? z : EVE_SELU_ALPHA * (__expf(z) - 1.f))) break;
-        case EVE_ACT_TANH:    LM_ALL(tanhf(z)) break;
-        case EVE_ACT_SIGMOID: LM_ALL(1.f / (1.f + __expf(-z))) break;
-        default: break;
-    }
-#undef LM_ALL
-}
 
 template <bool VEC, bool HASY, int G>
 __global__ __launch_bounds__(256) void linear_mm_kernel(const float* __restrict__ A, const float* __restrict__ Y, const int pro_act,
diff --git a/eve_amd/csrc/tail_fused.hip b/eve_amd/csrc/tail_fused.hip
--- /dev/null
+++ b/eve_amd/csrc/tail_fused.hip
@@ -0,0 +1,352 @@
+#include "linear_small.h"
+
+namespace eve {
+
+constexpr int TF_ROWS = 16;
+
+struct TfWeights {
+    const float *fc_w, *fc_b, *c0_w, *c0_b, *c2_w, *c2_b, *ih_w, *ih_b, *g0_w, *g0_b, *g2_w, *p0_w, *p0_b, *p2_w, *p2_b;
+};
+
+template <typename Epi>
+__device__ __forceinline__ void tf_layer(const float* xs, const int ldx, const int K, const float* __restrict__ W, const int N,
+                                         const float* __restrict__ bias, const int n_bias, const int act, const int first,
+                                         const int stride, const int lane, Epi&& epi) {
+    const int i = lane & 15, kk = lane >> 4;
+    const int ntiles = (N + 15) >> 4, nkb = (K + 15) >> 4, ngroups = (nkb + 3) >> 2;
+    const float* xrow = xs + i * ldx + 4 * kk;
+    for (int t0 = first; t0 < ntiles; t0 += 2 * stride) {
+        const bool has1 = t0 + stride < ntiles;
+        const int tt[2] = {t0, has1 ? t0 + stride : t0};
+        const float* wcol[2];
+        bool nok[2];
+#pragma unroll
+        for (int a = 0; a < 2; ++a) {
+            const int n = 16 * tt[a] + i;
+            nok[a] = n < N;
+            wcol[a] = W + min(n, N - 1);
+        }
+        struct Group { float w[4][2][4]; };
+        auto fetch = [&](const int g, Group& r) {
+#pragma unroll
+            for (int j = 0; j < 4; ++j) {
+                const int k = (4 * g + j) * 16 + 4 * kk;
+#pragma unroll
+                for (int a = 0; a < 2; ++a)
+#pragma unroll
+                    for (int s = 0; s < 4; ++s) r.w[j][a][s] = wcol[a][(size_t)min(k + s, K - 1) * N];
+            }
+        };
+        f32x4_t part[2][4];
+#pragma unroll
+        for (int a = 0; a < 2; ++a)
+#pragma unroll
+            for (int j = 0; j < 4; ++j) part[a][j] = f32x4_t{0.f, 0.f, 0.f, 0.f};
+        Group cur, nxt;
+        fetch(0, cur);
+        for (int g = 0; g < ngroups; ++g) {
+            const bool more = g + 1 < ngroups;
+            if (more) fetch(g + 1, nxt);
+#pragma unroll
+            for (int j = 0; j < 4; ++j) {
+                const int kb = 4 * g + j;
+                if (kb >= nkb) continue;
+                const int k = kb * 16 + 4 * kk;
+                const float4 xv = *reinterpret_cast<const float4*>(xrow + kb * 16);
+                const float x4[4] = {xv.x, xv.y, xv.z, xv.w};
+#pragma unroll
+                for (int s = 0; s < 4; ++s) {
+                    const bool kok = k + s < K;
+                    const float x = kok ? x4[s] : 0.f;
+                    part[0][j] = __builtin_amdgcn_mfma_f32_16x16x4f32((nok[0] && kok) ? cur.w[j][0][s] : 0.f, x, part[0][j], 0, 0, 0);
+                    if (has1) part[1][j] = __builtin_amdgcn_mfma_f32_16x16x4f32((nok[1] && kok) ? cur.w[j][1][s] : 0.f, x, part[1][j], 0, 0, 0);
+                }
+            }
+            if (more) cur = nxt;
+        }
+#pragma unroll
+        for (int a = 0; a < 2; ++a) {
+            if (a == 1 && !has1) break;
+            const int n0 = 16 * tt[a] + 4 * kk;
+            float v[4];
+#pragma unroll
+            for (int r = 0; r < 4; ++r) {
+                float sum = part[a][0][r];
+                sum += part[a][1][r];
+                sum += part[a][2][r];
+                sum += part[a][3][r];
+                const float w = (bias && n_bias > 0) ? bias[min(n0 + r, n_bias - 1)] : 0.f;
+                v[r] = sum + (n0 + r < n_bias ? w : 0.f);
+            }
+            lm_act_n(v, act);
+            if (n0 < N) epi(tt[a], v);
+        }
+    }
+}
+
+__device__ __forceinline__ void tf_store4(float* p, const float (&v)[4]) { *reinterpret_cast<float4*>(p) = make_float4(v[0], v[1], v[2], v[3]); }
+
+__device__ __forceinline__ void tf_stage(float* dst, const int ld, const float* __restrict__ src, const int n4, const int m0, const int M) {
+    for (int e = threadIdx.x; e < TF_ROWS * n4; e += 256) {
+        const int r = e / n4, c = e - r * n4;
+        float4 v = make_float4(0.f, 0.f, 0.f, 0.f);
+        if (m0 + r < M) v = reinterpret_cast<const float4*>(src)[(size_t)(m0 + r) * n4 + c];
+        *reinterpret_cast<float4*>(dst + r * ld + 4 * c) = v;
+    }
+}
+
+__device__ __forceinline__ void tf_times_act_grad(float (&out)[4], const float (&v)[4], const float* __restrict__ Y, const int ldy,
+                                                  const int m, const int M, const int n, const int act) {
+    const LmActGrad ag = lm_act_grad(act);
+    float4 y = make_float4(0.f, 0.f, 0.f, 0.f);
+    if (m < M) y = *reinterpret_cast<const float4*>(Y + (size_t)m * ldy + n);
+    out[0] = lm_apply_grad(v[0], y.x, ag, false); out[1] = lm_apply_grad(v[1], y.y, ag, false);
+    out[2] = lm_apply_grad(v[2], y.z, ag, false); out[3] = lm_apply_grad(v[3], y.w, ag, false);
+}
+
+#define TF_IDS                                                                                                             \
+    const int tid = threadIdx.x, wave = __builtin_amdgcn_readfirstlane(tid >> 6), lane = tid & 63, i = lane & 15, kk = lane >> 4; \
+    const int m0 = blockIdx.x * TF_ROWS, m = m0 + i;                                                                       \
+    const bool mok = m < M;                                                                                                \
+    (void)kk
+
+__global__ __launch_bounds__(256) void eye_tail_pre_fwd_kernel(const int BT, const float* __restrict__ feats, const float* __restrict__ hl,
+                                                               const float* __restrict__ hr, const TfWeights w, float* __restrict__ c0,
+                                                               const int ldc0, float* __restrict__ a1, float* __restrict__ a2, float* __restrict__ gi) {
+    __shared__ __attribute__((aligned(16))) float xs[TF_ROWS][516];
+    __shared__ __attribute__((aligned(16))) float c0s[TF_ROWS][148];
+    __shared__ __attribute__((aligned(16))) float a1s[TF_ROWS][132];
+    __shared__ __attribute__((aligned(16))) float a2s[TF_ROWS][132];
+    const int M = 2 * BT;
+    TF_IDS;
+    tf_stage(&xs[0][0], 516, feats, 128, m0, M);
+    if (tid < TF_ROWS) {
+        float hp[4] = {0.f, 0.f, 0.f, 0.f};
+        const int mm = m0 + tid;
+        if (mm < M) {
+            const float* h = mm >= BT ? hr + 2 * (size_t)(mm - BT) : hl + 2 * (size_t)mm;
+            hp[0] = h[0]; hp[1] = h[1];
+            tf_store4(c0 + (size_t)mm * ldc0 + 128, hp);
+        }
+        tf_store4(&c0s[tid][128], hp);
+    }
+    __syncthreads();
+    tf_layer(&xs[0][0], 516, 512, w.fc_w, 128, w.fc_b, 128, EVE_ACT_NONE, wave, 4, lane, [&](const int t, const float (&v)[4]) {
+        tf_store4(&c0s[i][16 * t + 4 * kk], v);
+        if (mok) tf_store4(c0 + (size_t)m * ldc0 + 16 * t + 4 * kk, v);
+    });
+    __syncthreads();
+    tf_layer(&c0s[0][0], 148, 132, w.c0_w, 128, w.c0_b, 128, EVE_ACT_SELU, wave, 4, lane, [&](const int t, const float (&v)[4]) {
+        tf_store4(&a1s[i][16 * t + 4 * kk], v);
+        if (mok) tf_store4(a1 + (size_t)m * 128 + 16 * t + 4 * kk, v);
+    });
+    __syncthreads();
+    tf_layer(&a1s[0][0], 132, 128, w.c2_w, 128, w.c2_b, 128, EVE_ACT_NONE, wave, 4, lane, [&](const int t, const float (&v)[4]) {
+        tf_store4(&a2s[i][16 * t + 4 * kk], v);
+        if (mok) tf_store4(a2 + (size_t)m * 128 + 16 * t + 4 * kk, v);
+    });
+    __syncthreads();
+    tf_layer(&a2s[0][0], 132, 128, w.ih_w, 384, w.ih_b, 384, EVE_ACT_NONE, wave, 4, lane, [&](const int t, const float (&v)[4]) {
+        if (mok) tf_store4(gi + (size_t)m * 384 + 16 * t + 4 * kk, v);
+    });
+}
+
+__global__ __launch_bounds__(256) void eye_tail_heads_fwd_kernel(const int M, const float* __restrict__ hs, const TfWeights w,
+                                                                 float* __restrict__ g1, float* __restrict__ g2, float* __restrict__ p1,
+                                                                 float* __restrict__ p2, float* __restrict__ gaze, float* __restrict__ pupil,
+                                                                 float* __restrict__ zero5) {
+    __shared__ __attribute__((aligned(16))) float hss[TF_ROWS][132];
+    __shared__ __attribute__((aligned(16))) float g1s[TF_ROWS][132];
+    __shared__ __attribute__((aligned(16))) float p1s[TF_ROWS][132];
+    TF_IDS;
+    if (zero5 && blockIdx.x == 0 && tid < 5) zero5[tid] = 0.f;
+    tf_stage(&hss[0][0], 132, hs, 32, m0, M);
+    __syncthreads();
+    tf_layer(&hss[0][0], 132, 128, w.g0_w, 128, w.g0_b, 128, EVE_ACT_SELU, wave, 4, lane, [&](const int t, const float (&v)[4]) {
+        tf_store4(&g1s[i][16 * t + 4 * kk], v);
+        if (mok) tf_store4(g1 + (size_t)m * 128 + 16 * t + 4 * kk, v);
+    });
+    tf_layer(&hss[0][0], 132, 128, w.p0_w, 128, w.p0_b, 128, EVE_ACT_SELU, wave, 4, lane, [&](const int t, const float (&v)[4]) {
+        tf_store4(&p1s[i][16 * t + 4 * kk], v);
+        if (mok) tf_store4(p1 + (size_t)m * 128 + 16 * t + 4 * kk, v);
+    });
+    __syncthreads();
+    if (wave == 0) {
+        tf_layer(&g1s[0][0], 132, 128, w.g2_w, 4, nullptr, 0, EVE_ACT_TANH, 0, 1, lane, [&](const int, const float (&v)[4]) {
+            if (!mok) return;
+            tf_store4(g2 + (size_t)m * 4, v);
+            gaze[2 * m] = LM_HALF_PI * v[0];
+            gaze[2 * m + 1] = LM_HALF_PI * v[1];
+        });
+    } else if (wave == 1) {
+        tf_layer(&p1s[0][0], 132, 128, w.p2_w, 4, w.p2_b, 1, EVE_ACT_RELU, 0, 1, lane, [&](const int, const float (&v)[4]) {
+            if (!mok) return;
+            tf_store4(p2 + (size_t)m * 4, v);
+            pupil[m] = v[0];
+        });
+    }
+}
+
+__global__ __launch_bounds__(256) void eye_tail_heads_bwd_kernel(const int BT, const float* __restrict__ dg_l, const float* __restrict__ dg_r,
+                                                                 const float* __restrict__ dp_l, const float* __restrict__ dp_r,
+                                                                 const float* __restrict__ g_full, const float c_ang, const float c_l1,
+                                                                 const float* __restrict__ g1, const float* __restrict__ g2,
+                                                                 const float* __restrict__ p1, const float* __restrict__ p2, const TfWeights w,
+                                                                 float* __restrict__ d_g2, float* __restrict__ d_g1, float* __restrict__ d_p2,
+                                                                 float* __restrict__ d_p1, float* __restrict__ d_hs) {
+    __shared__ __attribute__((aligned(16))) float tg[TF_ROWS][20];
+    __shared__ __attribute__((aligned(16))) float tp[TF_ROWS][20];
+    __shared__ __attribute__((aligned(16))) float g1s[TF_ROWS][132];
+    __shared__ __attribute__((aligned(16))) float p1s[TF_ROWS][132];
+    __shared__ __attribute__((aligned(16))) float hsum[TF_ROWS][132];
+    const int M = 2 * BT;
+    TF_IDS;
+    if (tid < TF_ROWS) {
+        const int mm = m0 + tid;
+        float a[4] = {0.f, 0.f, 0.f, 0.f}, b[4] = {0.f, 0.f, 0.f, 0.f}, ta[4] = {0.f, 0.f, 0.f, 0.f}, tb[4] = {0.f, 0.f, 0.f, 0.f};
+        if (mm < M) {
+            const float up = g_full ? *g_full : 1.f;
+            const bool right = mm >= BT;
+            const int r = right ? mm - BT : mm;
+            const float* dg = right ? dg_r : dg_l;
+            const float* dp = right ? dp_r : dp_l;
+            const float sa = LM_HALF_PI * c_ang * up, sl = c_l1 * up;
+            a[0] = sa * dg[2 * r]; a[1] = sa * dg[2 * r + 1];
+            b[0] = sl * dp[r];
+            tf_store4(d_g2 + (size_t)mm * 4, a);
+            tf_store4(d_p2 + (size_t)mm * 4, b);
+            tf_times_act_grad(ta, a, g2, 4, mm, M, 0, EVE_ACT_TANH);
+            tf_times_act_grad(tb, b, p2, 4, mm, M, 0, EVE_ACT_RELU);
+        }
+        tf_store4(&tg[tid][0], ta);
+        tf_store4(&tp[tid][0], tb);
+    }
+    __syncthreads();
+    tf_layer(&tg[0][0], 20, 4, w.g2_w, 128, nullptr, 0, EVE_ACT_NONE, wave, 4, lane, [&](const int t, const float (&v)[4]) {
+        const int n = 16 * t + 4 * kk;
+        float g[4];
+        tf_times_act_grad(g, v, g1, 128, m, M, n, EVE_ACT_SELU);
+        tf_store4(&g1s[i][n], g);
+        if (mok) tf_store4(d_g1 + (size_t)m * 128 + n, v);
+    });
+    tf_layer(&tp[0][0], 20, 4, w.p2_w, 128, nullptr, 0, EVE_ACT_NONE, wave, 4, lane, [&](const int t, const float (&v)[4]) {
+        const int n = 16 * t + 4 * kk;
+        float g[4];
+        tf_times_act_grad(g, v, p1, 128, m, M, n, EVE_ACT_SELU);
+        tf_store4(&p1s[i][n], g);
+        if (mok) tf_store4(d_p1 + (size_t)m * 128 + n, v);
+    });
+    __syncthreads();
+    tf_layer(&g1s[0][0], 132, 128, w.g0_w, 128, nullptr, 0, EVE_ACT_NONE, wave, 4, lane, [&](const int t, const float (&v)[4]) {
+        tf_store4(&hsum[i][16 * t + 4 * kk], v);
+    });
+    tf_layer(&p1s[0][0], 132, 128, w.p0_w, 128, nullptr, 0, EVE_ACT_NONE, wave, 4, lane, [&](const int t, const float (&v)[4]) {
+        const int n = 16 * t + 4 * kk;
+        const float4 prev = *reinterpret_cast<const float4*>(&hsum[i][n]);
+        const float s[4] = {v[0] + prev.x, v[1] + prev.y, v[2] + prev.z, v[3] + prev.w};
+        if (mok) tf_store4(d_hs + (size_t)m * 128 + n, s);
+    });
+}
+
+__global__ __launch_bounds__(256) void eye_tail_pre_bwd_kernel(const int M, const float* __restrict__ dgi, const float* __restrict__ a1,
+                                                               const TfWeights w, float* __restrict__ d_a2, float* __restrict__ d_a1,
+                                                               float* __restrict__ d_c0, const int ldc0, float* __restrict__ d_feats) {
+    __shared__ __attribute__((aligned(16))) float gis[TF_ROWS][388];
+    __shared__ __attribute__((aligned(16))) float a2s[TF_ROWS][132];
+    __shared__ __attribute__((aligned(16))) float a1s[TF_ROWS][132];
+    __shared__ __attribute__((aligned(16))) float c0s[TF_ROWS][148];
+    TF_IDS;
+    tf_stage(&gis[0][0], 388, dgi, 96, m0, M);
+    __syncthreads();
+    tf_layer(&gis[0][0], 388, 384, w.ih_w, 128, nullptr, 0, EVE_ACT_NONE, wave, 4, lane, [&](const int t, const float (&v)[4]) {
+        tf_store4(&a2s[i][16 * t + 4 * kk], v);
+        if (mok) tf_store4(d_a2 + (size_t)m * 128 + 16 * t + 4 * kk, v);
+    });
+    __syncthreads();
+    tf_layer(&a2s[0][0], 132, 128, w.c2_w, 128, nullptr, 0, EVE_ACT_NONE, wave, 4, lane, [&](const int t, const float (&v)[4]) {
+        const int n = 16 * t + 4 * kk;
+        float g[4];
+        tf_times_act_grad(g, v, a1, 128, m, M, n, EVE_ACT_SELU);
+        tf_store4(&a1s[i][n], g);
+        if (mok) tf_store4(d_a1 + (size_t)m * 128 + n, v);
+    });
+    __syncthreads();
+    tf_layer(&a1s[0][0], 132, 128, w.c0_w, 132, nullptr, 0, EVE_ACT_NONE, wave, 4, lane, [&](const int t, const float (&v)[4]) {
+        tf_store4(&c0s[i][16 * t + 4 * kk], v);
+        if (mok) tf_store4(d_c0 + (size_t)m * ldc0 + 16 * t + 4 * kk, v);
+    });
+    if (!d_feats) return;
+    __syncthreads();
+    tf_layer(&c0s[0][0], 148, 128, w.fc_w, 512, nullptr, 0, EVE_ACT_NONE, wave, 4, lane, [&](const int t, const float (&v)[4]) {
+        if (mok) tf_store4(d_feats + (size_t)m * 512 + 16 * t + 4 * kk, v);
+    });
+}
+
+static inline bool tf_al16(const void* p) { return !((uintptr_t)p & 15); }
+static inline TfWeights tf_weights(const eve_eye_tail_weights* s) {
+    return {s->fc_w, s->fc_b, s->c0_w, s->c0_b, s->c2_w, s->c2_b, s->ih_w, s->ih_b, s->g0_w, s->g0_b, s->g2_w, s->p0_w, s->p0_b, s->p2_w, s->p2_b};
+}
+static inline int tf_tiles(int M) { return (M + TF_ROWS - 1) / TF_ROWS; }
+
+}
+
+using namespace eve;
+
+extern "C" int eve_eye_tail_pre_fwd(int BT, const float* feats, const float* h_left, const float* h_right,
+                                    const eve_eye_tail_weights* w_in_out, float* c0, int ldc0, float* a1, float* a2, float* gi,
+                                    eve_stream_t stream) {
+    if (BT <= 0 || BT > (1 << 24)) return set_error_msg("eye_tail_pre_fwd: bad row count");
+    if (ldc0 < 132 || (ldc0 & 3)) return set_error_msg("eye_tail_pre_fwd: the concatenation's row stride is a multiple of 4, at least 132");
+    if (!feats || !h_left || !h_right || !w_in_out || !c0 || !a1 || !a2 || !gi) return set_error_msg("eye_tail_pre_fwd: null pointer");
+    const eve_eye_tail_weights& s = *w_in_out;
+    if (!s.fc_w || !s.fc_b || !s.c0_w || !s.c0_b || !s.c2_w || !s.c2_b || !s.ih_w || !s.ih_b) return set_error_msg("eye_tail_pre_fwd: null weight pointer");
+    if (!tf_al16(feats) || !tf_al16(c0) || !tf_al16(a1) || !tf_al16(a2) || !tf_al16(gi)) return set_error_msg("eye_tail_pre_fwd: 16-byte alignment");
+    EVE_LAUNCH("eye_tail_pre_fwd_kernel", eye_tail_pre_fwd_kernel, dim3(tf_tiles(2 * BT)), dim3(256), 0, (hipStream_t)stream, BT, feats, h_left, h_right,
+               tf_weights(w_in_out), c0, ldc0, a1, a2, gi);
+    EVE_CHECK_LAUNCH();
+    return 0;
+}
+
+extern "C" int eve_eye_tail_heads_fwd(int M, const float* hs, const eve_eye_tail_weights* w_in_out, float* g1, float* g2, float* p1,
+                                      float* p2, float* gaze, float* pupil, float* zero_terms, eve_stream_t stream) {
+    if (M <= 0 || M > (1 << 25)) return set_error_msg("eye_tail_heads_fwd: bad row count");
+    if (!hs || !w_in_out || !g1 || !g2 || !p1 || !p2 || !gaze || !pupil) return set_error_msg("eye_tail_heads_fwd: null pointer");
+    const eve_eye_tail_weights& s = *w_in_out;
+    if (!s.g0_w || !s.g0_b || !s.g2_w || !s.p0_w || !s.p0_b || !s.p2_w || !s.p2_b) return set_error_msg("eye_tail_heads_fwd: null weight pointer");
+    if (!tf_al16(hs) || !tf_al16(g1) || !tf_al16(g2) || !tf_al16(p1) || !tf_al16(p2)) return set_error_msg("eye_tail_heads_fwd: 16-byte alignment");
+    EVE_LAUNCH("eye_tail_heads_fwd_kernel", eye_tail_heads_fwd_kernel, dim3(tf_tiles(M)), dim3(256), 0, (hipStream_t)stream, M, hs, tf_weights(w_in_out), g1, g2,
+               p1, p2, gaze, pupil, zero_terms);
+    EVE_CHECK_LAUNCH();
+    return 0;
+}
+
+extern "C" int eve_eye_tail_heads_bwd(int BT, const float* dg_l, const float* dg_r, const float* dp_l, const float* dp_r, const float* g_full,
+                                      float coeff_ang, float coeff_l1, const float* g1, const float* g2, const float* p1, const float* p2,
+                                      const eve_eye_tail_weights* w_out_in, float* d_g2, float* d_g1, float* d_p2, float* d_p1, float* d_hs,
+                                      eve_stream_t stream) {
+    if (BT <= 0 || BT > (1 << 24)) return set_error_msg("eye_tail_heads_bwd: bad row count");
+    if (!dg_l || !dg_r || !dp_l || !dp_r || !g1 || !g2 || !p1 || !p2 || !w_out_in || !d_g2 || !d_g1 || !d_p2 || !d_p1 || !d_hs)
+        return set_error_msg("eye_tail_heads_bwd: null pointer");
+    const eve_eye_tail_weights& s = *w_out_in;
+    if (!s.g0_w || !s.g2_w || !s.p0_w || !s.p2_w) return set_error_msg("eye_tail_heads_bwd: null weight pointer");
+    if (!tf_al16(g1) || !tf_al16(g2) || !tf_al16(p1) || !tf_al16(p2) || !tf_al16(d_g2) || !tf_al16(d_g1) || !tf_al16(d_p2) || !tf_al16(d_p1) || !tf_al16(d_hs))
+        return set_error_msg("eye_tail_heads_bwd: 16-byte alignment");
+    EVE_LAUNCH("eye_tail_heads_bwd_kernel", eye_tail_heads_bwd_kernel, dim3(tf_tiles(2 * BT)), dim3(256), 0, (hipStream_t)stream, BT, dg_l, dg_r, dp_l, dp_r,
+               g_full, coeff_ang, coeff_l1, g1, g2, p1, p2, tf_weights(w_out_in), d_g2, d_g1, d_p2, d_p1, d_hs);
+    EVE_CHECK_LAUNCH();
+    return 0;
+}
+
+extern "C" int eve_eye_tail_pre_bwd(int M, const float* dgi, const float* a1, const eve_eye_tail_weights* w_out_in, float* d_a2, float* d_a1,
+                                    float* d_c0, int ldc0, float* d_feats, eve_stream_t stream) {
+    if (M <= 0 || M > (1 << 25)) return set_error_msg("eye_tail_pre_bwd: bad row count");
+    if (ldc0 < 132 || (ldc0 & 3)) return set_error_msg("eye_tail_pre_bwd: the concatenation's row stride is a multiple of 4, at least 132");
+    if (!dgi || !a1 || !w_out_in || !d_a2 || !d_a1 || !d_c0) return set_error_msg("eye_tail_pre_bwd: null pointer");
+    const eve_eye_tail_weights& s = *w_out_in;
+    if (!s.ih_w || !s.c2_w || !s.c0_w || (d_feats && !s.fc_w)) return set_error_msg("eye_tail_pre_bwd: null weight pointer");
+    if (!tf_al16(dgi) || !tf_al16(a1) || !tf_al16(d_a2) || !tf_al16(d_a1) || !tf_al16(d_c0) || !tf_al16(d_feats)) return set_error_msg("eye_tail_pre_bwd: 16-byte alignment");
+    EVE_LAUNCH("eye_tail_pre_bwd_kernel", eye_tail_pre_bwd_kernel, dim3(tf_tiles(M)), dim3(256), 0, (hipStream_t)stream, M, dgi, a1, tf_weights(w_out_in), d_a2,
+               d_a1, d_c0, ldc0, d_feats);
+    EVE_CHECK_LAUNCH();
+    return 0;
+}
diff --git a/eve_amd/kernels.py b/eve_amd/kernels.py
--- a/eve_amd/kernels.py
+++ b/eve_amd/kernels.py
@@ -1481,7 +1481,7 @@
                                                self._p(dp), self._stream()))
         return dp
 
-    def eye_losses(self, g_pred, g_tgt, g_val, p_pred, p_tgt, p_val, coeff_ang, coeff_l1):
+    def eye_losses(self, g_pred, g_tgt, g_val, p_pred, p_tgt, p_val, coeff_ang, coeff_l1, terms=None):
         B, T = p_pred[0].shape
         dev = p_pred[0].device
 
@@ -1502,7 +1502,9 @@
             k_, a = pair(ts, dt, shp)
             keep.append(k_)
             ptrs.append(a)
-        terms = torch.zeros((5,), dtype=torch.float32, device=dev)
+        if terms is None:
+            terms = torch.zeros((5,), dtype=torch.float32, device=dev)
+        assert terms.dtype == torch.float32 and terms.numel() == 5 and terms.is_contiguous() and terms.is_cuda
         dg = [torch.empty((B, T, 2), dtype=torch.float32, device=dev) for _ in range(2)]
         dp = [torch.empty((B, T), dtype=torch.float32, device=dev) for _ in range(2)]
         dg_a = (ctypes.c_void_p * 2)(*[t.data_ptr() for t in dg])
@@ -1567,6 +1569,82 @@
         self._ck(self.lib.eve_tail_outputs_bwd(BT, self._p(dg[0]), self._p(dg[1]), self._p(dp[0]), self._p(dp[1]), self._p(g_full),
                                                float(coeff_ang), float(coeff_l1), self._p(d_g2), self._p(d_p2), self._stream()))
         return d_g2, d_p2
+
+    @staticmethod
+    def _tail_weights(**ptrs):
+        w = _lib.EyeTailWeights()
+        for n, t in ptrs.items():
+            assert t is None or (t.dtype == torch.float32 and t.is_contiguous() and t.is_cuda), n
+            setattr(w, n, None if t is None else t.data_ptr())
+        return w
+
+    def _rows_f32(self, M, *shapes_and_tensors):
+        for t, n in shapes_and_tensors:
+            assert t.dtype == torch.float32 and t.is_contiguous() and t.is_cuda and tuple(t.shape) == ((M, n) if n else (M,)), (t.shape, n)
+
+    def eye_tail_pre_fwd(self, feats, h_left, h_right, fc_w, fc_b, c0_w, c0_b, c2_w, c2_b, ih_w, ih_b):
+        M, dev = feats.shape[0], feats.device
+        self._rows_f32(M, (feats, 512))
+        assert M % 2 == 0 and h_left.numel() == M and h_right.numel() == M and tuple(c0_w.shape) == (132, 128)
+        assert tuple(fc_w.shape) == (512, 128) and tuple(c2_w.shape) == (128, 128) and tuple(ih_w.shape) == (128, 384)
+        assert fc_b.numel() == 128 and c0_b.numel() == 128 and c2_b.numel() == 128 and ih_b.numel() == 384
+        for t in (h_left, h_right):
+            assert t.dtype == torch.float32 and t.is_contiguous() and t.is_cuda
+        new = lambda n: torch.empty((M, n), dtype=torch.float32, device=dev)
+        c0, a1, a2, gi = new(132), new(128), new(128), new(384)
+        w = self._tail_weights(fc_w=fc_w, fc_b=fc_b, c0_w=c0_w, c0_b=c0_b, c2_w=c2_w, c2_b=c2_b, ih_w=ih_w, ih_b=ih_b)
+        self._ck(self.lib.eve_eye_tail_pre_fwd(M // 2, self._p(feats), self._p(h_left), self._p(h_right), ctypes.byref(w), self._p(c0), 132,
+                                               self._p(a1), self._p(a2), self._p(gi), self._stream()))
+        return c0, a1, a2, gi
+
+    def eye_tail_heads_fwd(self, hs2, g0_w, g0_b, g2_w, p0_w, p0_b, p2_w, p2_b, zero_terms=None):
+        M, dev = hs2.shape[0], hs2.device
+        self._rows_f32(M, (hs2, 128))
+        assert tuple(g0_w.shape) == (128, 128) and tuple(p0_w.shape) == (128, 128) and tuple(g2_w.shape) == (128, 4) and tuple(p2_w.shape) == (128, 4)
+        assert g0_b.numel() == 128 and p0_b.numel() == 128 and p2_b.numel() == 1
+        assert zero_terms is None or (zero_terms.dtype == torch.float32 and zero_terms.numel() == 5 and zero_terms.is_contiguous())
+        new = lambda *s: torch.empty(s, dtype=torch.float32, device=dev)
+        g1, g2, p1, p2, gaze, pupil = new(M, 128), new(M, 4), new(M, 128), new(M, 4), new(M, 2), new(M)
+        w = self._tail_weights(g0_w=g0_w, g0_b=g0_b, g2_w=g2_w, p0_w=p0_w, p0_b=p0_b, p2_w=p2_w, p2_b=p2_b)
+        self._ck(self.lib.eve_eye_tail_heads_fwd(M, self._p(hs2), ctypes.byref(w), self._p(g1), self._p(g2), self._p(p1), self._p(p2),
+                                                 self._p(gaze), self._p(pupil), self._p(zero_terms), self._stream()))
+        return g1, g2, p1, p2, gaze, pupil
+
+    def eye_tail_heads_bwd(self, dg, dp, g_full, coeff_ang, coeff_l1, g1, g2, p1, p2, g0_w, g2_w, p0_w, p2_w):
+        BT = dp[0].numel()
+        M, dev = 2 * BT, g1.device
+        for t in (dg[0], dg[1], dp[0], dp[1]):
+            assert t.dtype == torch.float32 and t.is_contiguous() and t.is_cuda
+        assert dg[0].numel() == 2 * BT and dg[1].numel() == 2 * BT and dp[1].numel() == BT
+        assert g_full is None or (g_full.dtype == torch.float32 and g_full.numel() == 1 and g_full.is_cuda)
+        self._rows_f32(M, (g1, 128), (g2, 4), (p1, 128), (p2, 4))
+        assert tuple(g0_w.shape) == (128, 128) and tuple(p0_w.shape) == (128, 128) and tuple(g2_w.shape) == (4, 128) and tuple(p2_w.shape) == (4, 128)
+        new = lambda n: torch.empty((M, n), dtype=torch.float32, device=dev)
+        d_g2, d_g1, d_p2, d_p1, d_hs = new(4), new(128), new(4), new(128), new(128)
+        w = self._tail_weights(g0_w=g0_w, g2_w=g2_w, p0_w=p0_w, p2_w=p2_w)
+        self._ck(self.lib.eve_eye_tail_heads_bwd(BT, self._p(dg[0]), self._p(dg[1]), self._p(dp[0]), self._p(dp[1]), self._p(g_full),
+                                                 float(coeff_ang), float(coeff_l1), self._p(g1), self._p(g2), self._p(p1), self._p(p2),
+                                                 ctypes.byref(w), self._p(d_g2), self._p(d_g1), self._p(d_p2), self._p(d_p1), self._p(d_hs),
+                                                 self._stream()))
+        return d_g2, d_g1, d_p2, d_p1, d_hs
+
+    def eye_tail_pre_bwd(self, dgi, a1, ih_w, c2_w, c0_w, fc_w, want_d_feats):
+        M, dev = dgi.shape[0], dgi.device
+        self._rows_f32(M, (dgi, 384), (a1, 128))
+        assert tuple(ih_w.shape) == (384, 128) and tuple(c2_w.shape) == (128, 128) and tuple(c0_w.shape) == (128, 132) and tuple(fc_w.shape) == (128, 512)
+        new = lambda n: torch.empty((M, n), dtype=torch.float32, device=dev)
+        d_a2, d_a1, d_c0 = new(128), new(128), new(132)
+        d_feats = new(512) if want_d_feats else None
+        w = self._tail_weights(ih_w=ih_w, c2_w=c2_w, c0_w=c0_w, fc_w=fc_w)
+        self._ck(self.lib.eve_eye_tail_pre_bwd(M, self._p(dgi), self._p(a1), ctypes.byref(w), self._p(d_a2), self._p(d_a1), self._p(d_c0), 132,
+                                               self._p(d_feats), self._stream()))
+        return d_a2, d_a1, d_c0, d_feats
+
+    def wgrad_slab_reduce(self, slabs, dw, wide=True):
+        splits, n = slabs.shape
+        assert slabs.dtype == torch.float32 and dw.dtype == torch.float32 and dw.numel() == n and slabs.is_contiguous() and dw.is_contiguous()
+        self._ck(self.lib.eve_wgrad_slab_reduce(self._p(slabs), self._p(dw), n, splits, int(bool(wide)), self._stream()))
+        return dw
 
     def linear_dgrad(self, dy, y, act, w_out_in):
         M, N = dy.shape
diff --git a/eve_amd/ops.py b/eve_amd/ops.py
--- a/eve_amd/ops.py
+++ b/eve_amd/ops.py
@@ -485,22 +485,37 @@
         new = lambda n: torch.empty((M, n), dtype=torch.float32, device=dev)
         feats = feats.contiguous()
         cin0 = p0.ohwi.shape[3]
-        c0 = new(cin0)
-        k.linear_fwd_ex(feats, 512, p_fc.ihwo.view(512, 128), f32(cnn.fc.bias), ACT_NONE, c0)
-        k.tail_head_pose(h_left.detach().float().contiguous(), h_right.detach().float().contiguous(), c0, 128)
-        a1 = k.linear_fwd(c0, p0.ihwo.view(cin0, 128), f32(net.fc_common[0].bias), ACT_SELU)
-        a2 = k.linear_fwd(a1, p2.ihwo.view(128, 128), f32(net.fc_common[2].bias), ACT_NONE)
-        gi = k.linear_fwd(a2, p_ih.ihwo.view(128, 384), f32(cell.bias_ih), ACT_NONE)
+        fused = EyeTailLossFn.fused_ok(k, packs)
+        hl, hr = h_left.detach().float().contiguous(), h_right.detach().float().contiguous()
+        if fused:
+            c0, a1, a2, gi = k.eye_tail_pre_fwd(feats, hl, hr, p_fc.ihwo.view(512, 128), f32(cnn.fc.bias), p0.ihwo.view(cin0, 128),
+                                                f32(net.fc_common[0].bias), p2.ihwo.view(128, 128), f32(net.fc_common[2].bias),
+                                                p_ih.ihwo.view(128, 384), f32(cell.bias_ih))
+        else:
+            c0 = new(cin0)
+            k.linear_fwd_ex(feats, 512, p_fc.ihwo.view(512, 128), f32(cnn.fc.bias), ACT_NONE, c0)
+            k.tail_head_pose(hl, hr, c0, 128)
+            a1 = k.linear_fwd(c0, p0.ihwo.view(cin0, 128), f32(net.fc_common[0].bias), ACT_SELU)
+            a2 = k.linear_fwd(a1, p2.ihwo.view(128, 128), f32(net.fc_common[2].bias), ACT_NONE)
+            gi = k.linear_fwd(a2, p_ih.ihwo.view(128, 384), f32(cell.bias_ih), ACT_NONE)
         hs, gates, hn_pre = k.gru_scan_fwd(gi.view(2 * B, T, 384), p_hh.ihwo.view(128, 384), f32(cell.bias_hh), None)
         hs2 = hs.view(M, 128)
-        g1 = k.linear_fwd(hs2, pg0.ihwo.view(128, 128), f32(net.fc_to_gaze[0].bias), ACT_SELU)
-        g2 = k.linear_fwd_ex(g1, 128, pg2.ihwo.view(128, 4), None, ACT_TANH, new(4))
-        p1 = k.linear_fwd(hs2, pp0.ihwo.view(128, 128), f32(net.fc_to_pupil[0].bias), ACT_SELU)
-        p2_ = k.linear_fwd_ex(p1, 128, pp2.ihwo.view(128, 4), f32(net.fc_to_pupil[2].bias), ACT_RELU, new(4))
-        gaze, pupil = k.tail_outputs_fwd(g2, p2_)
+        terms0 = None
+        if fused:
+            terms0 = torch.empty((5,), dtype=torch.float32, device=dev)
+            g1, g2, p1, p2_, gaze, pupil = k.eye_tail_heads_fwd(hs2, pg0.ihwo.view(128, 128), f32(net.fc_to_gaze[0].bias), pg2.ihwo.view(128, 4),
+                                                                pp0.ihwo.view(128, 128), f32(net.fc_to_pupil[0].bias), pp2.ihwo.view(128, 4),
+                                                                f32(net.fc_to_pupil[2].bias), zero_terms=terms0)
+        else:
+            g1 = k.linear_fwd(hs2, pg0.ihwo.view(128, 128), f32(net.fc_to_gaze[0].bias), ACT_SELU)
+            g2 = k.linear_fwd_ex(g1, 128, pg2.ihwo.view(128, 4), None, ACT_TANH, new(4))
+            p1 = k.linear_fwd(hs2, pp0.ihwo.view(128, 128), f32(net.fc_to_pupil[0].bias), ACT_SELU)
+            p2_ = k.linear_fwd_ex(p1, 128, pp2.ihwo.view(128, 4), f32(net.fc_to_pupil[2].bias), ACT_RELU, new(4))
+            gaze, pupil = k.tail_outputs_fwd(g2, p2_)
         tg_l, tg_r, vg_l, vg_r, tp_l, tp_r, vp_l, vp_r = targets
-        terms, dg, dp = k.eye_losses((gaze[:BT].view(B, T, 2), gaze[BT:].view(B, T, 2)), (tg_l, tg_r), (vg_l, vg_r),
-                                     (pupil[:BT].view(B, T), pupil[BT:].view(B, T)), (tp_l, tp_r), (vp_l, vp_r), c_ang, c_l1)
+        loss_args = ((gaze[:BT].view(B, T, 2), gaze[BT:].view(B, T, 2)), (tg_l, tg_r), (vg_l, vg_r),
+                     (pupil[:BT].view(B, T), pupil[BT:].view(B, T)), (tp_l, tp_r), (vp_l, vp_r), c_ang, c_l1)
+        terms, dg, dp = k.eye_losses(*loss_args, terms=terms0) if fused else k.eye_losses(*loss_args)
         ctx.net, ctx.packs, ctx.coeffs, ctx.BT = net, packs, (c_ang, c_l1), (B, T)
         ctx.params = EyeTailLossFn.tail_parameters(net)
         for p_ in ctx.params:
@@ -510,6 +525,17 @@
         ctx.mark_non_differentiable(gaze, pupil, hs)
         return tuple(terms.unbind(0)) + (gaze, pupil, hs)
 
+    capture = None
+
+    @staticmethod
+    def fused_ok(k, packs):
+        if not (hasattr(k, 'eye_tail_pre_fwd') and hasattr(k, 'eye_tail_heads_fwd') and hasattr(k, 'eye_tail_heads_bwd') and
+                hasattr(k, 'eye_tail_pre_bwd') and dispatch_flag(k, 'tail_fused', 0)):
+            return False
+        want = ((128, 512), (128, 132), (128, 128), (384, 128), (384, 128), (128, 128), (4, 128), (128, 128), (4, 128))
+        return all(p_.ihwo is not None and p_.ohwi.dtype == torch.float32 and
+                   (p_.ohwi.shape[0], p_.ohwi.shape[3]) == s and p_.ohwi.shape[1] == p_.ohwi.shape[2] == 1 for p_, s in zip(packs, want))
+
     @staticmethod
     def tail_parameters(net):
         cnn, cell = net.cnn_layers, net.rnn_cells[0]
@@ -533,20 +559,33 @@
         cin0 = p0.ohwi.shape[3]
         hs2 = hs.view(M, 128)
         g_full = g_full.detach().float().contiguous()
-        d_g2, d_p2 = k.tail_outputs_bwd((dg_l, dg_r), (dp_l, dp_r), g_full, ctx.coeffs[0], ctx.coeffs[1])
-        d_g1 = k.linear_dgrad(d_g2, g2, ACT_TANH, pg2.ohwi.view(4, 128))
-        d_hs = k.linear_dgrad(d_g1, g1, ACT_SELU, pg0.ohwi.view(128, 128))
-        d_p1 = k.linear_dgrad(d_p2, p2_, ACT_RELU, pp2.ohwi.view(4, 128))
-        k.linear_dgrad_ex(d_p1, 128, p1, ACT_SELU, pp0.ohwi.view(128, 128), d_hs, accumulate=True)
+        fused = EyeTailLossFn.fused_ok(k, ctx.packs)
+        if fused:
+            d_g2, d_g1, d_p2, d_p1, d_hs = k.eye_tail_heads_bwd((dg_l, dg_r), (dp_l, dp_r), g_full, ctx.coeffs[0], ctx.coeffs[1], g1, g2, p1, p2_,
+                                                                pg0.ohwi.view(128, 128), pg2.ohwi.view(4, 128), pp0.ohwi.view(128, 128),
+                                                                pp2.ohwi.view(4, 128))
+        else:
+            d_g2, d_p2 = k.tail_outputs_bwd((dg_l, dg_r), (dp_l, dp_r), g_full, ctx.coeffs[0], ctx.coeffs[1])
+            d_g1 = k.linear_dgrad(d_g2, g2, ACT_TANH, pg2.ohwi.view(4, 128))
+            d_hs = k.linear_dgrad(d_g1, g1, ACT_SELU, pg0.ohwi.view(128, 128))
+            d_p1 = k.linear_dgrad(d_p2, p2_, ACT_RELU, pp2.ohwi.view(4, 128))
+            k.linear_dgrad_ex(d_p1, 128, p1, ACT_SELU, pp0.ohwi.view(128, 128), d_hs, accumulate=True)
         dgi, dgh, _ = k.gru_scan_bwd(d_hs.view(2 * B, T, 128), p_hh.ohwi.view(384, 128), None, hs, gates, hn_pre, False)
         dgi2, dgh2 = dgi.view(M, 384), dgh.view(M, 384)
-        d_a2 = k.linear_dgrad(dgi2, None, ACT_NONE, p_ih.ohwi.view(384, 128))
-        d_a1 = k.linear_dgrad(d_a2, None, ACT_NONE, p2.ohwi.view(128, 128))
-        d_c0 = k.linear_dgrad(d_a1, a1, ACT_SELU, p0.ohwi.view(128, cin0))
-        d_feats = None
-        if ctx.needs_input_grad[0]:
-            d_feats = torch.empty((M, 512), dtype=torch.float32, device=dev)
-            k.linear_dgrad_ex(d_c0, 128, None, ACT_NONE, p_fc.ohwi.view(128, 512), d_feats)
+        if fused:
+            d_a2, d_a1, d_c0, d_feats = k.eye_tail_pre_bwd(dgi2, a1, p_ih.ohwi.view(384, 128), p2.ohwi.view(128, 128), p0.ohwi.view(128, cin0),
+                                                           p_fc.ohwi.view(128, 512), bool(ctx.needs_input_grad[0]))
+        else:
+            d_a2 = k.linear_dgrad(dgi2, None, ACT_NONE, p_ih.ohwi.view(384, 128))
+            d_a1 = k.linear_dgrad(d_a2, None, ACT_NONE, p2.ohwi.view(128, 128))
+            d_c0 = k.linear_dgrad(d_a1, a1, ACT_SELU, p0.ohwi.view(128, cin0))
+            d_feats = None
+            if ctx.needs_input_grad[0]:
+                d_feats = torch.empty((M, 512), dtype=torch.float32, device=dev)
+                k.linear_dgrad_ex(d_c0, 128, None, ACT_NONE, p_fc.ohwi.view(128, 512), d_feats)
+        if EyeTailLossFn.capture is not None:
+            EyeTailLossFn.capture.update(d_g2=d_g2, d_g1=d_g1, d_p2=d_p2, d_p1=d_p1, d_hs=d_hs, dgi=dgi2, dgh=dgh2, d_a2=d_a2, d_a1=d_a1,
+                                         d_c0=d_c0, d_feats=d_feats, fused=fused)
         gw = lambda p_: p_.grad.view(p_.shape[0], -1) if p_.dim() == 2 else p_.grad
         k.linear_wgrad_batch([
             dict(dY=d_c0, X=feats, dW=gw(w_fc), db=gw(b_fc)),
diff --git a/include/eve_hip.h b/include/eve_hip.h
--- a/include/eve_hip.h
+++ b/include/eve_hip.h
@@ -57,6 +57,7 @@
     int tail_loss_node;
     int bucket_elems;
     int gate_wait_polls;
+    int tail_fused;
     long long wgrad_halo_min_m;
 } eve_dispatch_config;
 int eve_get_dispatch_config(eve_dispatch_config* out);
@@ -83,6 +84,7 @@
 int eve_conv2d_wgrad(const eve_conv_desc* d, const void* x, const void* dy,
                      const float* in_scale_shift, int pro_act, float* dw_ohwi,
                      void* workspace, unsigned long long workspace_bytes, eve_stream_t stream);
+int eve_wgrad_slab_reduce(const float* slabs, float* dw, long long n, int splits, int wide, eve_stream_t stream);
 int eve_conv2d_wgrad_bias(const eve_conv_desc* d, const void* x, const void* dy, float* dw_ohwi, float* db,
                           void* workspace, unsigned long long workspace_bytes, eve_stream_t stream);
 int eve_stem_pack_input(int dtype , int N, int C, int IH, int IW, const float* src_nchw, void* x_padded,
@@ -332,6 +334,16 @@
 } eve_eye_tail_weights;
 int eve_eye_tail_stream_fwd(int S, int T, const float* feats, const float* head_pose, const eve_eye_tail_weights* weights,
                             float* h, const int* reset, float* gaze, float* pupil, float* hs, eve_stream_t stream);
+int eve_eye_tail_pre_fwd(int BT, const float* feats, const float* h_left, const float* h_right, const eve_eye_tail_weights* w_in_out,
+                         float* c0, int ldc0, float* a1, float* a2, float* gi, eve_stream_t stream);
+int eve_eye_tail_heads_fwd(int M, const float* hs, const eve_eye_tail_weights* w_in_out, float* g1, float* g2, float* p1, float* p2,
+                           float* gaze, float* pupil, float* zero_terms, eve_stream_t stream);
+int eve_eye_tail_heads_bwd(int BT, const float* dg_l, const float* dg_r, const float* dp_l, const float* dp_r, const float* g_full,
+                           float coeff_ang, float coeff_l1, const float* g1, const float* g2, const float* p1, const float* p2,
+                           const eve_eye_tail_weights* w_out_in, float* d_g2, float* d_g1, float* d_p2, float* d_p1, float* d_hs,
+                           eve_stream_t stream);
+int eve_eye_tail_pre_bwd(int M, const float* dgi, const float* a1, const eve_eye_tail_weights* w_out_in, float* d_a2, float* d_a1,
+                         float* d_c0, int ldc0, float* d_feats, eve_stream_t stream);
 int eve_stream_state_rows(int dtype, int S, long long row_elems, long long src_stride, long long dst_stride, const void* src,
                           void* dst, const int* reset, eve_stream_t stream);
 int eve_eye_tail_stream_fwd_len(int S, int T, const float* feats, const float* head_pose, const eve_eye_tail_weights* weights,
```

Result: no change. 90400 frames/s (median of 4 runs) (+0.3%).
